# andrewadare/SLAM.jl

Measured on AMD Instinct MI355X. Metric: EKF updates/sec @ 10k landmarks, higher is better.
Workload: dtype f32; 1 GPU; EKF-SLAM observation step (associate+update; no new features arise), N=10000 landmarks (n=20003), nz=64 obs/step, gates 4.0/25.0, cholesky form, state resident in HBM; landmarks=10000, form=cholesky, parallelism=single GPU

## Files before the change

### slam.jl_amd/csrc/common.h

```cpp
#pragma once

#include <hip/hip_runtime.h>
#include <stdint.h>
#include <stdio.h>
#include <string.h>
#include <vector>

#include "../../include/slamhip.h"
#include "../../include/slamhip_diag.h"

#define SLAM_PI 3.14159265358979323846

void slam_set_error(const char* fmt, ...);

#define HIP_TRY(expr)                                                                  \
    do {                                                                               \
        hipError_t _e = (expr);                                                        \
        if (_e != hipSuccess) {                                                        \
            slam_set_error("%s failed: %s (%s:%d)", #expr, hipGetErrorString(_e),     \
                           __FILE__, __LINE__);                                        \
            return (_e == hipErrorOutOfMemory) ? SLAM_E_NOMEM : SLAM_E_HIP;            \
        }                                                                              \
    } while (0)

#define ARG_CHECK(cond, msg)                                                           \
    do {                                                                               \
        if (!(cond)) {                                                                 \
            slam_set_error("bad argument: %s", msg);                                   \
            return SLAM_E_BADARG;                                                      \
        }                                                                              \
    } while (0)

void slam_roctx_push(const char* name);
void slam_roctx_pop(void);
struct SlamRange {
    explicit SlamRange(const char* name) { slam_roctx_push(name); }
    ~SlamRange() { slam_roctx_pop(); }
    SlamRange(const SlamRange&) = delete;
    SlamRange& operator=(const SlamRange&) = delete;
};
#define SLAM_RANGE() SlamRange slam_range_scope_(__func__)

#define SLAM_TILE 128
#define SLAM_KPAD 32

static inline int round_up(int a, int b) { return (a + b - 1) / b * b; }

#ifdef SLAMHIP_EXPERIMENTS
#include <stdlib.h>
static inline int slam_exp_env(const char* name, int dflt) {
    const char* v = getenv(name);
    return v ? atoi(v) : dflt;
}
constexpr int SLAM_XFLAGS_MASK = ~0;
#else
static inline int slam_exp_env(const char*, int dflt) { return dflt; }
constexpr int SLAM_XFLAGS_MASK = 4 | 8 | 16 | 32 | 64 | 128 | 512 | 65536;
#endif

struct TimingPair {
    hipEvent_t a, b;
    int kid;
};

struct slam_ekf {
    int dtype;
    int device;
    int num_cus;
    int maxN;
    int N;
    int ncap;
    int ld;
    int npad;
    size_t esz;
    void* x;
    void* P;
    void* Pside;
    hipStream_t stream;
    double* PHtS;
    hipEvent_t stage_ev;
    int stage_pending;

    int kcap;
    double* PHt;
    double* Kd;
    void* W1;
    void* W2;
    void* Wimg;
    double* Cmat;
    double* Smat;
    double* Mwork;
    double* gvec;
    double* obsbuf;
    int32_t* idfbuf;
    int ocap;
    double* h_obs;
    int32_t* h_idf;
    int32_t* h_assoc;
    int32_t* d_assoc;
    double* h_obs_dev;
    int32_t* h_assoc_dev;
    double* znbuf;
    int32_t* d_count;
    int32_t* h_flag;
    int32_t* h_flag_dev;
    int32_t obs_seq;

    int2* tiles;
    int tiles_T, tiles_len, tiles_cap;
    int tilesB_off, tilesB_len;
    int tilesH_off, tilesH_len;
    unsigned* dd_claim;
    int tiles_xlen[8];
    int diag_off, diag_len, diag_xlen[8];

    double* d_pmax;
    int pmax_valid;

    int gate_mode;
    int gate_last;
    void* grid_meta;
    int32_t* grid_cells;
    void* grid_items;
    int grid_force;
    int grid_upd;
    int grid_live;
    int grid_n_seen;

    double* gate_part;
    int gate_blocks_cap;

    double* d_small;
    double* h_small;
    int32_t* d_status;
    int32_t* h_status;

    int xflags;
    int debug_flags;
    void* dd_prof;
    int factor_blocked;
    int debug_stamps;
    int async_updates;
    int deferred;
    int pending_status;

    int timing;
    std::vector<TimingPair> pairs;
    std::vector<TimingPair> free_pairs;
    double t_ms[SLAM_K_COUNT];
    double t_sq[SLAM_K_COUNT];
    double t_min[SLAM_K_COUNT];
    int64_t t_n[SLAM_K_COUNT];
};

struct KTimer {
    slam_ekf* h;
    TimingPair p;
    bool on;
    hipStream_t s;
    KTimer(slam_ekf* h_, int kid, hipStream_t stream = nullptr);
    ~KTimer();
};

int launch_ellipses(slam_ekf* h, double* d_out);
int launch_block_gather(slam_ekf* h, int r0, int c0, int nr, int nc, int diag, void* d_out);
int launch_pack(slam_ekf* h, const void* d_src, int lds, int n, int cf, int ncols);
int launch_unpack(slam_ekf* h, void* d_dst, int ldd, int n, int cf, int ncols);
int launch_side_rebuild(slam_ekf* h);
int launch_compact(slam_ekf* h, const int32_t* keep_host, int n_new, int f0);
int launch_find_duplicates(slam_ekf* h, double gate, int32_t* pairs_out, int cap, int* count);
int launch_merge_update(slam_ekf* h, const int32_t* keep, const int32_t* gone, int cnt, const double Rc[4]);
int launch_copy_floor(slam_ekf* h, int reps, double out[2]);
int launch_predict(slam_ekf* h, double v, double g, double w, const double Q[4], double dt);
int launch_augment(slam_ekf* h, int nn, const double R[4], const double* zn_dev);
int launch_gate(slam_ekf* h, int nz, const double R[4], double gate1, double gate2, const double* z_host, bool compact);
constexpr int SLAM_GRID_SLOTS = 64;
int gate_kernels_init();
int gate_info(slam_ekf* h, int64_t out[8]);
unsigned long long* grid_drift_slot(slam_ekf* h);
int ensure_pmax(slam_ekf* h);
int launch_nis(slam_ekf* h, const double z1[2], int j, const double R[4]);
int launch_obs_model(slam_ekf* h, int j);
int launch_update(slam_ekf* h, int m, const double R[4], int form, bool device_count);
int ensure_update_workspace(slam_ekf* h, int m);
int ensure_obs_capacity(slam_ekf* h, int nobs);
```

### slam.jl_amd/csrc/ekf_api.hip

```cpp
#include <stdarg.h>
#include <stdio.h>
#include <stdlib.h>
#include <string.h>
#include <vector>

#include "common.h"

int update_kernels_init();

static thread_local char g_err[512] = "";

void slam_set_error(const char* fmt, ...) {
    va_list ap;
    va_start(ap, fmt);
    vsnprintf(g_err, sizeof(g_err), fmt, ap);
    va_end(ap);
}

extern "C" const char* slam_last_error(void) { return g_err; }

#include <dlfcn.h>
#include <mutex>
namespace {
typedef int (*roctx_push_fn)(const char*);
typedef int (*roctx_pop_fn)(void);
roctx_push_fn g_roctx_push = nullptr;
roctx_pop_fn g_roctx_pop = nullptr;
std::once_flag g_roctx_once;
void roctx_resolve() {
    const char* names[] = {"librocprofiler-sdk-roctx.so.1", "librocprofiler-sdk-roctx.so", "libroctx64.so.4", "libroctx64.so"};
    const char* env = getenv("SLAMHIP_ROCTX");
    const bool want = env && atoi(env) != 0;
    if (env && !want) return;
    void* lib = nullptr;
    for (const char* n : names)
        if ((lib = dlopen(n, RTLD_LAZY | RTLD_NOLOAD))) break;
    if (!lib && want)
        for (const char* n : names)
            if ((lib = dlopen(n, RTLD_LAZY | RTLD_GLOBAL))) break;
    if (!lib) return;
    g_roctx_push = (roctx_push_fn)dlsym(lib, "roctxRangePushA");
    g_roctx_pop = (roctx_pop_fn)dlsym(lib, "roctxRangePop");
    if (!g_roctx_push || !g_roctx_pop) g_roctx_push = nullptr, g_roctx_pop = nullptr;
}
}
void slam_roctx_push(const char* name) {
    std::call_once(g_roctx_once, roctx_resolve);
    if (g_roctx_push) (void)g_roctx_push(name);
}
void slam_roctx_pop(void) {
    if (g_roctx_pop) (void)g_roctx_pop();
}

extern "C" int slam_device_count(void) {
    int n = 0;
    if (hipGetDeviceCount(&n) != hipSuccess) {
        (void)hipGetLastError();
        return 0;
    }
    return n;
}

KTimer::KTimer(slam_ekf* h_, int kid, hipStream_t stream)
    : h(h_), on(h_->timing == 1 || ((h_->timing >> (kid + 1)) & 1)), s(stream ? stream : h_->stream) {
    if (!on) return;
    if (!h->free_pairs.empty()) {
        p = h->free_pairs.back();
        h->free_pairs.pop_back();
    } else {
        if (hipEventCreateWithFlags(&p.a, hipEventDisableSystemFence) != hipSuccess ||
            hipEventCreateWithFlags(&p.b, hipEventDisableSystemFence) != hipSuccess) {
            on = false;
            return;
        }
    }
    p.kid = kid;
    (void)hipEventRecord(p.a, s);
}

KTimer::~KTimer() {
    if (!on) return;
    (void)hipEventRecord(p.b, s);
    h->pairs.push_back(p);
}

static int fold_timing(slam_ekf* h) {
    HIP_TRY(hipStreamSynchronize(h->stream));
    for (auto& p : h->pairs) {
        float ms = 0.f;
        if (hipEventElapsedTime(&ms, p.a, p.b) == hipSuccess) {
            h->t_ms[p.kid] += ms;
            h->t_sq[p.kid] += (double)ms * (double)ms;
            if (h->t_min[p.kid] == 0.0 || ms < h->t_min[p.kid]) h->t_min[p.kid] = ms;
            h->t_n[p.kid] += 1;
        }
        h->free_pairs.push_back(p);
    }
    h->pairs.clear();
    return SLAM_OK;
}

template <typename P>
static int dev_alloc_zero(P** p, size_t bytes, hipStream_t s) {
    *p = nullptr;
    if (bytes == 0) bytes = 16;
    HIP_TRY(hipMalloc((void**)p, bytes));
    HIP_TRY(hipMemsetAsync(*p, 0, bytes, s));
    return SLAM_OK;
}

static void dev_free(void* p) {
    if (p) (void)hipFree(p);
}

int ensure_obs_capacity(slam_ekf* h, int nobs) {
    if (nobs <= h->ocap) return SLAM_OK;
    int cap = h->ocap ? h->ocap : 256;
    while (cap < nobs) cap *= 2;
    HIP_TRY(hipStreamSynchronize(h->stream));
    dev_free(h->obsbuf); dev_free(h->idfbuf); dev_free(h->d_assoc); dev_free(h->gate_part); dev_free(h->znbuf);
    if (h->h_obs) (void)hipHostFree(h->h_obs);
    if (h->h_idf) (void)hipHostFree(h->h_idf);
    if (h->h_assoc) (void)hipHostFree(h->h_assoc);
    h->obsbuf = nullptr; h->idfbuf = nullptr; h->d_assoc = nullptr; h->gate_part = nullptr; h->znbuf = nullptr;
    h->h_obs = nullptr; h->h_idf = nullptr; h->h_assoc = nullptr;
    h->ocap = 0;
    int rc;
    if ((rc = dev_alloc_zero(&h->obsbuf, sizeof(double) * 2 * cap, h->stream))) return rc;
    if ((rc = dev_alloc_zero(&h->idfbuf, sizeof(int32_t) * cap, h->stream))) return rc;
    if ((rc = dev_alloc_zero(&h->d_assoc, sizeof(int32_t) * cap, h->stream))) return rc;
    if ((rc = dev_alloc_zero(&h->znbuf, sizeof(double) * 2 * cap, h->stream))) return rc;
    h->gate_blocks_cap = (h->maxN + 63) / 64 + 1;
    if ((rc = dev_alloc_zero(&h->gate_part, sizeof(double) * 3 * 256 * (size_t)h->gate_blocks_cap, h->stream))) return rc;
    HIP_TRY(hipHostMalloc((void**)&h->h_obs, sizeof(double) * 2 * cap, hipHostMallocDefault));
    HIP_TRY(hipHostMalloc((void**)&h->h_idf, sizeof(int32_t) * cap, hipHostMallocDefault));
    HIP_TRY(hipHostMalloc((void**)&h->h_assoc, sizeof(int32_t) * cap, hipHostMallocDefault));
    HIP_TRY(hipHostGetDevicePointer((void**)&h->h_obs_dev, h->h_obs, 0));
    HIP_TRY(hipHostGetDevicePointer((void**)&h->h_assoc_dev, h->h_assoc, 0));
    h->ocap = cap;
    return SLAM_OK;
}

static void free_update_workspace(slam_ekf* h) {
    dev_free(h->PHt); dev_free(h->PHtS); dev_free(h->Kd); dev_free(h->W1); dev_free(h->W2); dev_free(h->Cmat); dev_free(h->Wimg);
    dev_free(h->Smat); dev_free(h->Mwork); dev_free(h->gvec);
    h->W1 = h->W2 = h->Wimg = nullptr;
    h->PHt = h->PHtS = h->Kd = h->Cmat = h->Smat = h->Mwork = h->gvec = nullptr;
    h->kcap = 0;
}

static int zero_panels(slam_ekf* h) {
    if (!h->kcap) return SLAM_OK;
    HIP_TRY(hipMemsetAsync(h->PHt, 0, sizeof(double) * (size_t)h->npad * h->kcap, h->stream));
    HIP_TRY(hipMemsetAsync(h->Kd, 0, sizeof(double) * (size_t)h->npad * h->kcap, h->stream));
    HIP_TRY(hipMemsetAsync(h->W1, 0, h->esz * (size_t)h->npad * 2 * h->kcap, h->stream));
    HIP_TRY(hipMemsetAsync(h->W2, 0, h->esz * (size_t)h->npad * 2 * h->kcap, h->stream));
    return SLAM_OK;
}

int ensure_update_workspace(slam_ekf* h, int m) {
    const int kp = round_up(2 * m, SLAM_KPAD);
    if (kp <= h->kcap) return SLAM_OK;
    int cap = h->kcap ? h->kcap : 32;
    while (cap < kp) cap *= 2;
    HIP_TRY(hipStreamSynchronize(h->stream));
    free_update_workspace(h);
    int rc;
    if ((rc = dev_alloc_zero(&h->PHt, sizeof(double) * (size_t)h->npad * cap, h->stream))) return rc;
    if ((rc = dev_alloc_zero(&h->PHtS, sizeof(double) * (size_t)(3 + cap) * cap, h->stream))) return rc;
    if ((rc = dev_alloc_zero(&h->Kd, sizeof(double) * (size_t)h->npad * cap, h->stream))) return rc;
    if ((rc = dev_alloc_zero(&h->W1, h->esz * (size_t)h->npad * 2 * cap, h->stream))) return rc;
    if ((rc = dev_alloc_zero(&h->W2, h->esz * (size_t)h->npad * 2 * cap, h->stream))) return rc;
    if (h->dtype == SLAM_F32 && (rc = dev_alloc_zero(&h->Wimg, (size_t)(h->npad / 128) * (cap / 16) * 3 * 4096, h->stream))) return rc;
    if ((rc = dev_alloc_zero(&h->Cmat, sizeof(double) * (size_t)cap * cap, h->stream))) return rc;
    if ((rc = dev_alloc_zero(&h->Smat, sizeof(double) * (size_t)cap * cap, h->stream))) return rc;
    if ((rc = dev_alloc_zero(&h->Mwork, sizeof(double) * (size_t)cap * (cap + 1), h->stream))) return rc;
    if ((rc = dev_alloc_zero(&h->gvec, sizeof(double) * (size_t)cap, h->stream))) return rc;
    h->kcap = cap;
    return SLAM_OK;
}

extern "C" int slam_ekf_destroy(slam_ekf_t h) {
    if (!h) return SLAM_OK;
    (void)hipSetDevice(h->device);
    if (h->stream) (void)hipStreamSynchronize(h->stream);
#ifdef SLAMHIP_EXPERIMENTS
    if (h->dd_prof && slam_exp_env("SLAMHIP_STAMPS", 0)) {
        const size_t cnt = (size_t)4096 * 16;
        std::vector<unsigned long long> v(cnt);
        if (hipMemcpy(v.data(), h->dd_prof, cnt * 8, hipMemcpyDeviceToHost) == hipSuccess) {
            double s[16] = {0};
            size_t waves = 0;
            for (size_t w = 0; w < 4096; ++w) {
                if (!v[16 * w]) continue;
                ++waves;
                for (int i = 0; i < 16; ++i) s[i] += (double)v[16 * w + i];
            }
            if (waves) {
                fprintf(stderr, "[slamhip] dma down-date, mean per wave of %zu waves: steps %.1f  clk per step: reads %.0f  mfma-issue %.0f  barrier %.0f  dma-issue %.0f  stores(per tile) %.0f  chunk-wait by step:",
                        waves, s[0] / waves, s[1] / s[0], s[2] / s[0], s[3] / s[0], s[4] / s[0], s[5] / s[0] * 8);
                for (int i = 0; i < 8; ++i) fprintf(stderr, " %.0f", s[6 + i] / s[0] * 8);
                fprintf(stderr, "  | stream: %.0f shader clocks in %.2f us per wave = %.3f GHz in-kernel clock\n", s[14] / waves, s[15] / waves / 100.0,
                        s[15] > 0 ? s[14] / s[15] * 0.1 : 0.0);
            }
        }
        dev_free(h->dd_prof);
        h->dd_prof = nullptr;
    }
#endif
    if (h->dd_prof) {
        const size_t cnt = (size_t)4096 * 4 * 4;
        std::vector<unsigned long long> v(cnt);
        if (hipMemcpy(v.data(), h->dd_prof, cnt * 8, hipMemcpyDeviceToHost) == hipSuccess) {
            double s[4] = {0, 0, 0, 0}, mx = 0;
            size_t waves = 0;
            for (size_t w = 0; w < cnt / 4; ++w) {
                if (!v[4 * w + 3]) continue;
                ++waves;
                for (int i = 0; i < 4; ++i) s[i] += (double)v[4 * w + i];
                if ((double)v[4 * w + 3] > mx) mx = (double)v[4 * w + 3];
            }
            if (waves)
                fprintf(stderr, "[slamhip] down-date per-wave (mean of %zu waves): panel-wait %.0f clk  lifetime %.0f x 10 ns  epilogue %.0f clk  lifetime %.0f clk (max %.0f)\n",
                        waves, s[0] / waves, s[1] / waves, s[2] / waves, s[3] / waves, mx);
        }
        dev_free(h->dd_prof);
    }
    for (auto& p : h->pairs) { (void)hipEventDestroy(p.a); (void)hipEventDestroy(p.b); }
    for (auto& p : h->free_pairs) { (void)hipEventDestroy(p.a); (void)hipEventDestroy(p.b); }
    free_update_workspace(h);
    dev_free(h->x); dev_free(h->P); dev_free(h->Pside); dev_free(h->tiles);
    dev_free(h->obsbuf); dev_free(h->idfbuf); dev_free(h->d_assoc); dev_free(h->gate_part); dev_free(h->znbuf);
    dev_free(h->d_small); dev_free(h->d_status); dev_free(h->d_count); dev_free(h->d_pmax); dev_free(h->dd_claim);
    dev_free(h->grid_meta); dev_free(h->grid_cells); dev_free(h->grid_items);
    if (h->h_flag) (void)hipHostFree(h->h_flag);
    if (h->h_obs) (void)hipHostFree(h->h_obs);
    if (h->h_idf) (void)hipHostFree(h->h_idf);
    if (h->h_assoc) (void)hipHostFree(h->h_assoc);
    if (h->h_small) (void)hipHostFree(h->h_small);
    if (h->h_status) (void)hipHostFree(h->h_status);
    if (h->stage_ev) (void)hipEventDestroy(h->stage_ev);
    if (h->stream) (void)hipStreamDestroy(h->stream);
    delete h;
    return SLAM_OK;
}

static int create_impl(slam_ekf* h) {
    HIP_TRY(hipSetDevice(h->device));
    hipDeviceProp_t prop;
    HIP_TRY(hipGetDeviceProperties(&prop, h->device));
    h->num_cus = prop.multiProcessorCount > 0 ? prop.multiProcessorCount : 256;
    HIP_TRY(hipStreamCreateWithFlags(&h->stream, hipStreamNonBlocking));
    HIP_TRY(hipEventCreateWithFlags(&h->stage_ev, hipEventDisableTiming | hipEventDisableSystemFence));
    int rc;
    if ((rc = update_kernels_init())) return rc;
    if ((rc = gate_kernels_init())) return rc;
    if ((rc = dev_alloc_zero(&h->x, h->esz * (size_t)h->ncap, h->stream))) return rc;
    {
        const int E = h->dtype == SLAM_F32 ? 128 : 64;
        const size_t T = (size_t)h->npad / E;
        if ((rc = dev_alloc_zero(&h->P, h->esz * (T * (T + 1) / 2) * E * E, h->stream))) return rc;
        if ((rc = dev_alloc_zero(&h->Pside, h->esz * 3 * (size_t)(h->npad / 2), h->stream))) return rc;
    }
    if ((rc = dev_alloc_zero(&h->d_small, sizeof(double) * 64, h->stream))) return rc;
    if ((rc = dev_alloc_zero(&h->d_count, sizeof(int32_t) * 4, h->stream))) return rc;
    if ((rc = dev_alloc_zero(&h->d_pmax, sizeof(double), h->stream))) return rc;
    if ((rc = dev_alloc_zero(&h->dd_claim, 8 * 64, h->stream))) return rc;
    HIP_TRY(hipHostMalloc((void**)&h->h_flag, sizeof(int32_t) * 16, hipHostMallocDefault));
    h->h_flag[0] = 0;
    HIP_TRY(hipHostGetDevicePointer((void**)&h->h_flag_dev, h->h_flag, 0));
    if ((h->debug_flags & 8) && (rc = dev_alloc_zero(&h->dd_prof, (size_t)4096 * 4 * 4 * 8, h->stream))) return rc;
#ifdef SLAMHIP_EXPERIMENTS
    if (!h->dd_prof && slam_exp_env("SLAMHIP_STAMPS", 0) && (rc = dev_alloc_zero(&h->dd_prof, (size_t)4096 * 16 * 8, h->stream))) return rc;
#endif
    if ((rc = dev_alloc_zero(&h->d_status, sizeof(int32_t) * 4, h->stream))) return rc;
    HIP_TRY(hipHostMalloc((void**)&h->h_small, sizeof(double) * 64, hipHostMallocDefault));
    HIP_TRY(hipHostMalloc((void**)&h->h_status, sizeof(int32_t) * 4, hipHostMallocDefault));
    if ((rc = ensure_obs_capacity(h, 256))) return rc;
    HIP_TRY(hipStreamSynchronize(h->stream));
    return SLAM_OK;
}

extern "C" int slam_ekf_create(slam_ekf_t* out, int dtype, int max_landmarks, int device) {
    ARG_CHECK(out != nullptr, "handle pointer is null");
    *out = nullptr;
    ARG_CHECK(dtype == SLAM_F32 || dtype == SLAM_F64, "dtype must be SLAM_F32 or SLAM_F64");
    ARG_CHECK(max_landmarks >= 0 && max_landmarks <= 500000, "max_landmarks out of range");
    const int ndev = slam_device_count();
    if (ndev <= 0) {
        slam_set_error("no HIP device available: libslamhip has no CPU fallback");
        return SLAM_E_HIP;
    }
    ARG_CHECK(device >= 0 && device < ndev, "device index out of range");
    slam_ekf* h = new slam_ekf();
    h->dtype = dtype;
    h->device = device;
    h->maxN = max_landmarks;
    h->N = 0;
    h->ncap = 3 + 2 * max_landmarks;
    h->npad = round_up(h->ncap, SLAM_TILE);
    h->ld = h->npad;
    h->esz = dtype == SLAM_F32 ? 4 : 8;
    h->x = h->P = h->Pside = nullptr;
    h->stream = nullptr;
    h->stage_ev = nullptr; h->stage_pending = 0;
    h->PHtS = nullptr;
    h->kcap = 0;
    h->W1 = h->W2 = h->Wimg = nullptr;
    h->PHt = h->PHtS = h->Kd = h->Cmat = h->Smat = h->Mwork = h->gvec = nullptr;
    h->tiles = nullptr; h->tiles_T = h->tiles_len = h->tiles_cap = 0; h->tilesB_off = h->tilesB_len = 0;
    h->obsbuf = nullptr; h->idfbuf = nullptr; h->ocap = 0;
    h->h_obs = nullptr; h->h_idf = nullptr; h->h_assoc = nullptr; h->d_assoc = nullptr;
    h->gate_part = nullptr; h->gate_blocks_cap = 0;
    h->d_small = h->h_small = nullptr;
    h->d_pmax = nullptr; h->pmax_valid = 0; h->dd_claim = nullptr;
    h->gate_mode = SLAM_GATE_AUTO; h->gate_last = 0; h->grid_meta = nullptr; h->grid_cells = nullptr; h->grid_items = nullptr;
    h->grid_force = 1; h->grid_upd = 0; h->grid_live = 0; h->grid_n_seen = 0;
    h->znbuf = nullptr; h->d_count = nullptr; h->h_flag = nullptr; h->h_flag_dev = nullptr; h->obs_seq = 0;
    h->d_status = h->h_status = nullptr;
    h->async_updates = 0; h->deferred = 0; h->pending_status = 0; h->debug_stamps = 0;
    h->debug_flags = 0;
#ifdef SLAMHIP_EXPERIMENTS
    h->debug_flags = getenv("SLAMHIP_DEBUG") ? atoi(getenv("SLAMHIP_DEBUG")) : 0;
#endif
    h->dd_prof = nullptr;
    h->xflags = (getenv("SLAMHIP_X") ? atoi(getenv("SLAMHIP_X")) : 0) & SLAM_XFLAGS_MASK;
    h->factor_blocked = 1;
#ifdef SLAMHIP_EXPERIMENTS
    h->factor_blocked = !(getenv("SLAMHIP_FACTOR") && !strcmp(getenv("SLAMHIP_FACTOR"), "scalar"));
    if (getenv("SLAMHIP_FACTOR") && !strcmp(getenv("SLAMHIP_FACTOR"), "pivot1")) h->factor_blocked = 2;
#endif
    h->timing = 0;
    for (int i = 0; i < SLAM_K_COUNT; ++i) { h->t_ms[i] = 0; h->t_sq[i] = 0; h->t_n[i] = 0; h->t_min[i] = 0; }
    const int rc = create_impl(h);
    if (rc != SLAM_OK) {
        slam_ekf_destroy(h);
        return rc;
    }
    *out = h;
    return SLAM_OK;
}

static int state_band_columns(const slam_ekf* h, int n) {
    const size_t budget = (size_t)256 << 20;
    size_t w = budget / (h->esz * (size_t)n) / SLAM_TILE * SLAM_TILE;
    if (w < SLAM_TILE) w = SLAM_TILE;
    if (w > (size_t)h->npad) w = (size_t)h->npad;
    return (int)w;
}

static int set_state_impl(slam_ekf* h, const void* x, const void* P, int n, int ldP, hipMemcpyKind kind) {
    ARG_CHECK(h != nullptr, "null handle");
    ARG_CHECK(x != nullptr && P != nullptr, "x / P is null");
    ARG_CHECK(n >= 3 && ((n - 3) % 2) == 0, "n must be 3 + 2*N");
    ARG_CHECK(ldP >= n, "ldP < n");
    const int N = (n - 3) / 2;
    if (N > h->maxN) {
        slam_set_error("state has %d landmarks, capacity is %d", N, h->maxN);
        return SLAM_E_CAPACITY;
    }
    HIP_TRY(hipSetDevice(h->device));
    if (N < h->N) {
        const int rc = zero_panels(h);
        if (rc) return rc;
    }
    HIP_TRY(hipMemcpyAsync(h->x, x, h->esz * (size_t)n, kind, h->stream));
    int rc = SLAM_OK;
    hipError_t es = hipSuccess;
    if (kind == hipMemcpyHostToDevice) {
        const int W = state_band_columns(h, n);
        void* d_tmp = nullptr;
        HIP_TRY(hipMalloc(&d_tmp, h->esz * (size_t)n * W));
        for (int c = 0; c < h->npad && rc == SLAM_OK && es == hipSuccess; c += W) {
            const int w = c + W <= h->npad ? W : h->npad - c;
            const int wn = n - c < 0 ? 0 : (n - c < w ? n - c : w);
            if (wn > 0)
                es = hipMemcpy2DAsync(d_tmp, h->esz * (size_t)n, (const char*)P + h->esz * (size_t)c * ldP, h->esz * (size_t)ldP,
                                      h->esz * (size_t)n, (size_t)wn, kind, h->stream);
            if (es == hipSuccess) rc = launch_pack(h, d_tmp, n, n, c, w);
            if (es == hipSuccess && rc == SLAM_OK) es = hipStreamSynchronize(h->stream);
        }
        (void)hipFree(d_tmp);
    } else {
        rc = launch_pack(h, P, ldP, n, 0, h->npad);
        es = hipStreamSynchronize(h->stream);
    }
    if (rc) return rc;
    if (es != hipSuccess) {
        slam_set_error("upload of the state failed: %s", hipGetErrorString(es));
        return SLAM_E_HIP;
    }
    h->N = N;
    h->pmax_valid = 0;
    h->grid_force = 1;
    return SLAM_OK;
}

extern "C" int slam_ekf_set_state(slam_ekf_t h, const void* x, const void* P, int n, int ldP) {
    SLAM_RANGE();
    return set_state_impl(h, x, P, n, ldP, hipMemcpyHostToDevice);
}

extern "C" int slam_ekf_set_state_device(slam_ekf_t h, const void* d_x, const void* d_P, int n, int ldP) {
    SLAM_RANGE();
    return set_state_impl(h, d_x, d_P, n, ldP, hipMemcpyDeviceToDevice);
}

extern "C" int slam_ekf_get_state(slam_ekf_t h, void* x, void* P, int n, int ldP) {
    SLAM_RANGE();
    ARG_CHECK(h != nullptr, "null handle");
    ARG_CHECK(n == 3 + 2 * h->N, "n does not match the state (3 + 2*N)");
    ARG_CHECK(P == nullptr || ldP >= n, "ldP < n");
    HIP_TRY(hipSetDevice(h->device));
    if (x) HIP_TRY(hipMemcpyAsync(x, h->x, h->esz * (size_t)n, hipMemcpyDeviceToHost, h->stream));
    int rc = SLAM_OK;
    hipError_t es = hipSuccess;
    if (P) {
        const int W = state_band_columns(h, n);
        void* d_tmp = nullptr;
        HIP_TRY(hipMalloc(&d_tmp, h->esz * (size_t)n * W));
        for (int c = 0; c < n && rc == SLAM_OK && es == hipSuccess; c += W) {
            const int w = c + W <= n ? W : n - c;
            rc = launch_unpack(h, d_tmp, n, n, c, w);
            if (rc == SLAM_OK)
                es = hipMemcpy2DAsync((char*)P + h->esz * (size_t)c * ldP, h->esz * (size_t)ldP, d_tmp, h->esz * (size_t)n,
                                      h->esz * (size_t)n, (size_t)w, hipMemcpyDeviceToHost, h->stream);
            if (rc == SLAM_OK && es == hipSuccess) es = hipStreamSynchronize(h->stream);
        }
        (void)hipFree(d_tmp);
    }
    if (es == hipSuccess) es = hipStreamSynchronize(h->stream);
    if (rc) return rc;
    if (es != hipSuccess) {
        slam_set_error("download of the state failed: %s", hipGetErrorString(es));
        return SLAM_E_HIP;
    }
    return SLAM_OK;
}

static int get_gathered(slam_ekf* h, int r0, int c0, int nr, int nc, int diag, void* out, int ld_out) {
    HIP_TRY(hipSetDevice(h->device));
    void* d_tmp = nullptr;
    HIP_TRY(hipMalloc(&d_tmp, h->esz * (size_t)nr * nc));
    int rc = launch_block_gather(h, r0, c0, nr, nc, diag, d_tmp);
    if (rc == SLAM_OK) {
        hipError_t e = hipMemcpy2DAsync(out, h->esz * (size_t)ld_out, d_tmp, h->esz * (size_t)nr, h->esz * (size_t)nr, (size_t)nc,
                                        hipMemcpyDeviceToHost, h->stream);
        if (e == hipSuccess) e = hipStreamSynchronize(h->stream);
        if (e != hipSuccess) {
            slam_set_error("HIP error while reading a covariance block: %s", hipGetErrorString(e));
            rc = SLAM_E_HIP;
        }
    }
    (void)hipFree(d_tmp);
    return rc;
}

extern "C" int slam_ekf_get_block(slam_ekf_t h, int r0, int c0, int nr, int nc, void* out, int ld_out) {
    SLAM_RANGE();
    ARG_CHECK(h != nullptr, "null handle");
    const int n = 3 + 2 * h->N;
    ARG_CHECK(nr >= 0 && nc >= 0, "negative block size");
    if (nr == 0 || nc == 0) return SLAM_OK;
    ARG_CHECK(out != nullptr, "out is null");
    ARG_CHECK(r0 >= 0 && c0 >= 0 && r0 + nr <= n && c0 + nc <= n, "block outside the n x n covariance (Julia: BoundsError)");
    ARG_CHECK(ld_out >= nr, "ld_out < nr");
    ARG_CHECK((size_t)nr * nc <= ((size_t)1 << 28), "block larger than 2^28 elements: read it in pieces");
    return get_gathered(h, r0, c0, nr, nc, 0, out, ld_out);
}

extern "C" int slam_ekf_get_diag(slam_ekf_t h, void* out) {
    ARG_CHECK(h != nullptr && out != nullptr, "null argument");
    const int n = 3 + 2 * h->N;
    return get_gathered(h, 0, 0, n, 1, 1, out, n);
}

extern "C" int slam_ekf_get_landmark_blocks(slam_ekf_t h, void* out) {
    ARG_CHECK(h != nullptr && out != nullptr, "null argument");
    if (h->N == 0) return SLAM_OK;
    HIP_TRY(hipSetDevice(h->device));
    HIP_TRY(hipMemcpy2DAsync(out, h->esz * (size_t)h->N, h->Pside, h->esz * (size_t)(h->npad / 2), h->esz * (size_t)h->N, 3,
                             hipMemcpyDeviceToHost, h->stream));
    HIP_TRY(hipStreamSynchronize(h->stream));
    return SLAM_OK;
}

extern "C" int slam_ekf_get_pose(slam_ekf_t h, double pose[3]) {
    ARG_CHECK(h != nullptr && pose != nullptr, "null argument");
    HIP_TRY(hipSetDevice(h->device));
    HIP_TRY(hipMemcpyAsync(h->h_small, h->x, h->esz * 3, hipMemcpyDeviceToHost, h->stream));
    HIP_TRY(hipStreamSynchronize(h->stream));
    for (int i = 0; i < 3; ++i)
        pose[i] = h->dtype == SLAM_F32 ? (double)((float*)h->h_small)[i] : h->h_small[i];
    return SLAM_OK;
}

extern "C" int slam_ekf_ellipses(slam_ekf_t h, double* features, double vehicle[6]) {
    SLAM_RANGE();
    ARG_CHECK(h != nullptr, "null handle");
    HIP_TRY(hipSetDevice(h->device));
    const size_t cnt = (size_t)h->N + 1;
    double* d_out = nullptr;
    HIP_TRY(hipMalloc((void**)&d_out, sizeof(double) * 5 * cnt));
    std::vector<double> host(5 * cnt);
    int rc = launch_ellipses(h, d_out);
    if (rc == SLAM_OK) {
        const hipError_t e1 = hipMemcpyAsync(host.data(), d_out, sizeof(double) * 5 * cnt, hipMemcpyDeviceToHost, h->stream);
        const hipError_t e2 = e1 == hipSuccess ? hipStreamSynchronize(h->stream) : e1;
        if (e2 != hipSuccess) {
            slam_set_error("HIP error in slam_ekf_ellipses: %s", hipGetErrorString(e2));
            rc = SLAM_E_HIP;
        }
    }
    (void)hipFree(d_out);
    if (rc) return rc;
    if (features)
        for (size_t i = 0; i < 5 * (cnt - 1); ++i) features[i] = host[5 + i];
    if (vehicle) {
        double pose[3];
        if ((rc = slam_ekf_get_pose(h, pose))) return rc;
        vehicle[0] = pose[0]; vehicle[1] = pose[1]; vehicle[2] = pose[2];
        vehicle[3] = host[2]; vehicle[4] = host[3]; vehicle[5] = host[4];
    }
    return SLAM_OK;
}

extern "C" int slam_ekf_num_landmarks(slam_ekf_t h, int* N) {
    ARG_CHECK(h != nullptr && N != nullptr, "null argument");
    *N = h->N;
    return SLAM_OK;
}

extern "C" int slam_ekf_dtype(slam_ekf_t h, int* dtype) {
    ARG_CHECK(h != nullptr && dtype != nullptr, "null argument");
    *dtype = h->dtype;
    return SLAM_OK;
}

extern "C" int slam_ekf_device_ptrs(slam_ekf_t h, void** d_x, void** d_P, int* ld, void** stream) {
    ARG_CHECK(h != nullptr, "null handle");
    if (d_x) *d_x = h->x;
    if (d_P) *d_P = h->P;
    if (ld) *ld = h->ld;
    if (stream) *stream = (void*)h->stream;
    return SLAM_OK;
}

extern "C" int slam_ekf_state_written(slam_ekf_t h) {
    SLAM_RANGE();
    ARG_CHECK(h != nullptr, "null handle");
    HIP_TRY(hipSetDevice(h->device));
    h->pmax_valid = 0;
    h->grid_force = 1;
    return launch_side_rebuild(h);
}

static int remove_marked(slam_ekf* h, const std::vector<char>& gone, int cnt, int32_t* new_index) {
    const int N = h->N;
    const int n_new = 3 + 2 * (N - cnt);
    std::vector<int32_t> keep((size_t)n_new);
    keep[0] = 0; keep[1] = 1; keep[2] = 2;
    int first = 0, next = 0;
    for (int j = 1; j <= N; ++j) {
        if (gone[j]) {
            if (!first) first = j;
            continue;
        }
        keep[3 + 2 * next] = 3 + 2 * (j - 1);
        keep[4 + 2 * next] = 4 + 2 * (j - 1);
        ++next;
    }
    HIP_TRY(hipSetDevice(h->device));
    int rc;
    if ((rc = launch_compact(h, keep.data(), n_new, 3 + 2 * (first - 1)))) return rc;
    h->N = N - cnt;
    if ((rc = zero_panels(h))) return rc;
    h->pmax_valid = 0;
    h->grid_force = 1;
    h->grid_n_seen = h->N;
    if ((rc = launch_side_rebuild(h))) return rc;
    if (new_index)
        for (int j = 1, k = 0; j <= N; ++j) new_index[j - 1] = gone[j] ? 0 : ++k;
    return SLAM_OK;
}

extern "C" int slam_ekf_remove_landmarks(slam_ekf_t h, const int32_t* ids, int cnt, int32_t* new_index) {
    SLAM_RANGE();
    ARG_CHECK(h != nullptr, "null handle");
    ARG_CHECK(cnt >= 0, "cnt < 0");
    ARG_CHECK(cnt == 0 || ids != nullptr, "ids is null");
    const int N = h->N;
    std::vector<char> gone((size_t)N + 1, 0);
    for (int i = 0; i < cnt; ++i) {
        ARG_CHECK(ids[i] >= 1 && ids[i] <= N, "landmark id out of range");
        ARG_CHECK(!gone[ids[i]], "duplicate landmark id");
        gone[ids[i]] = 1;
    }
    if (cnt == 0) {
        if (new_index)
            for (int j = 1; j <= N; ++j) new_index[j - 1] = j;
        return SLAM_OK;
    }
    return remove_marked(h, gone, cnt, new_index);
}

extern "C" int slam_ekf_find_duplicates(slam_ekf_t h, double gate, int32_t* pairs, int cap, int* count) {
    SLAM_RANGE();
    ARG_CHECK(h != nullptr, "null handle");
    ARG_CHECK(count != nullptr, "count is null");
    ARG_CHECK(cap >= 0, "cap < 0");
    ARG_CHECK(cap == 0 || pairs != nullptr, "pairs is null");
    ARG_CHECK(gate > 0.0 && gate <= 1.79769313486231570815e308, "gate must be finite and positive");
    HIP_TRY(hipSetDevice(h->device));
    return launch_find_duplicates(h, gate, pairs, cap, count);
}

extern "C" int slam_ekf_merge_landmarks(slam_ekf_t h, const int32_t* pairs, int cnt, const double Rc[4], int32_t* new_index) {
    SLAM_RANGE();
    ARG_CHECK(h != nullptr, "null handle");
    ARG_CHECK(cnt >= 0 && cnt <= SLAM_MERGE_MAX, "cnt outside 0 .. SLAM_MERGE_MAX");
    ARG_CHECK(cnt == 0 || pairs != nullptr, "pairs is null");
    const int N = h->N;
    std::vector<char> used((size_t)N + 1, 0), gone((size_t)N + 1, 0);
    int32_t keep_id[SLAM_MERGE_MAX], gone_id[SLAM_MERGE_MAX];
    for (int p = 0; p < cnt; ++p) {
        const int32_t a = pairs[2 * p], b = pairs[2 * p + 1];
        ARG_CHECK(a >= 1 && a <= N && b >= 1 && b <= N, "landmark id out of range");
        ARG_CHECK(a != b, "a pair names one landmark twice");
        ARG_CHECK(!used[a] && !used[b], "a landmark appears in more than one pair (merge a chain with one call per link)");
        used[a] = used[b] = 1;
        gone[b] = 1;
        keep_id[p] = a;
        gone_id[p] = b;
    }
    if (Rc) {
        ARG_CHECK(Rc[1] == Rc[2], "Rc is not symmetric");
        ARG_CHECK(Rc[0] >= 0.0 && Rc[3] >= 0.0, "Rc has a negative diagonal");
    }
    if (cnt == 0) {
        if (new_index)
            for (int j = 1; j <= N; ++j) new_index[j - 1] = j;
        return SLAM_OK;
    }
    HIP_TRY(hipSetDevice(h->device));
    int rc;
    if ((rc = ensure_update_workspace(h, SLAM_MERGE_MAX))) return rc;
    if ((rc = launch_merge_update(h, keep_id, gone_id, cnt, Rc))) return rc;
    HIP_TRY(hipMemcpyAsync(h->h_status, h->d_status, sizeof(int32_t) * 4, hipMemcpyDeviceToHost, h->stream));
    HIP_TRY(hipStreamSynchronize(h->stream));
    if (h->h_status[0]) {
        slam_set_error("merge: S is not positive definite (state left unchanged, nothing removed)");
        return SLAM_E_NOTPD;
    }
    if ((rc = remove_marked(h, gone, cnt, new_index))) return rc;
    if (new_index)
        for (int p = 0; p < cnt; ++p) new_index[gone_id[p] - 1] = new_index[keep_id[p] - 1];
    return SLAM_OK;
}

extern "C" int slam_ekf_copy_floor(slam_ekf_t h, int reps, double out[2]) {
    SLAM_RANGE();
    ARG_CHECK(h != nullptr && out != nullptr, "null argument");
    ARG_CHECK(reps >= 1 && reps <= 1000, "reps out of range");
    HIP_TRY(hipSetDevice(h->device));
    return launch_copy_floor(h, reps, out);
}

static int check_R(const double* R) {
    ARG_CHECK(R != nullptr, "R is null");
    return SLAM_OK;
}

static int stage_obs(slam_ekf* h, const double* z, const int32_t* idf, int nobs) {
    int rc = ensure_obs_capacity(h, nobs);
    if (rc) return rc;
    if (h->stage_pending) {
        HIP_TRY(hipEventSynchronize(h->stage_ev));
        h->stage_pending = 0;
    }
    memcpy(h->h_obs, z, sizeof(double) * 2 * (size_t)nobs);
    HIP_TRY(hipMemcpyAsync(h->obsbuf, h->h_obs, sizeof(double) * 2 * (size_t)nobs, hipMemcpyHostToDevice, h->stream));
    if (idf) {
        memcpy(h->h_idf, idf, sizeof(int32_t) * (size_t)nobs);
        HIP_TRY(hipMemcpyAsync(h->idfbuf, h->h_idf, sizeof(int32_t) * (size_t)nobs, hipMemcpyHostToDevice, h->stream));
    }
    HIP_TRY(hipEventRecord(h->stage_ev, h->stream));
    h->stage_pending = 1;
    return SLAM_OK;
}

extern "C" int slam_ekf_predict(slam_ekf_t h, double v, double g, double wheelbase, const double Q[4], double dt) {
    SLAM_RANGE();
    ARG_CHECK(h != nullptr && Q != nullptr, "null argument");
    HIP_TRY(hipSetDevice(h->device));
    return launch_predict(h, v, g, wheelbase, Q, dt);
}

extern "C" int slam_ekf_associate(slam_ekf_t h, const double* z, int nz, const double R[4], double gate1, double gate2,
                                  int32_t* assoc) {
    SLAM_RANGE();
    ARG_CHECK(h != nullptr, "null handle");
    ARG_CHECK(nz >= 0, "nz < 0");
    if (nz == 0) return SLAM_OK;
    ARG_CHECK(z != nullptr && assoc != nullptr, "z / assoc is null");
    int rc = check_R(R);
    if (rc) return rc;
    if (h->N == 0) {
        for (int i = 0; i < nz; ++i) assoc[i] = -1;
        return SLAM_OK;
    }
    HIP_TRY(hipSetDevice(h->device));
    if ((rc = ensure_obs_capacity(h, nz))) return rc;
    if ((rc = launch_gate(h, nz, R, gate1, gate2, z, false))) return rc;
    HIP_TRY(hipMemcpyAsync(h->h_assoc, h->d_assoc, sizeof(int32_t) * (size_t)nz, hipMemcpyDeviceToHost, h->stream));
    HIP_TRY(hipStreamSynchronize(h->stream));
    memcpy(assoc, h->h_assoc, sizeof(int32_t) * (size_t)nz);
    return SLAM_OK;
}

extern "C" int slam_ekf_set_gate_mode(slam_ekf_t h, int mode) {
    ARG_CHECK(h != nullptr, "null handle");
    ARG_CHECK(mode == SLAM_GATE_AUTO || mode == SLAM_GATE_SWEEP || mode == SLAM_GATE_GRID, "unknown gate mode");
    h->gate_mode = mode;
    h->grid_force = 1;
    return SLAM_OK;
}

extern "C" int slam_ekf_gate_info(slam_ekf_t h, int64_t out[8]) {
    ARG_CHECK(h != nullptr && out != nullptr, "null argument");
    HIP_TRY(hipSetDevice(h->device));
    return gate_info(h, out);
}

extern "C" int slam_ekf_nis(slam_ekf_t h, const double z1[2], int j, const double R[4], double out[2]) {
    ARG_CHECK(h != nullptr && z1 != nullptr && out != nullptr, "null argument");
    int rc = check_R(R);
    if (rc) return rc;
    ARG_CHECK(j >= 1 && j <= h->N, "landmark index out of range");
    HIP_TRY(hipSetDevice(h->device));
    if ((rc = launch_nis(h, z1, j, R))) return rc;
    HIP_TRY(hipMemcpyAsync(h->h_small, h->d_small, sizeof(double) * 2, hipMemcpyDeviceToHost, h->stream));
    HIP_TRY(hipStreamSynchronize(h->stream));
    out[0] = h->h_small[0];
    out[1] = h->h_small[1];
    return SLAM_OK;
}

extern "C" int slam_ekf_predict_observation(slam_ekf_t h, int j, double zp[2], double Hv[6], double Hf[4]) {
    ARG_CHECK(h != nullptr && zp != nullptr && Hv != nullptr && Hf != nullptr, "null argument");
    ARG_CHECK(j >= 1 && j <= h->N, "landmark index out of range");
    HIP_TRY(hipSetDevice(h->device));
    int rc;
    if ((rc = launch_obs_model(h, j))) return rc;
    HIP_TRY(hipMemcpyAsync(h->h_small, h->d_small, sizeof(double) * 12, hipMemcpyDeviceToHost, h->stream));
    HIP_TRY(hipStreamSynchronize(h->stream));
    zp[0] = h->h_small[0]; zp[1] = h->h_small[1];
    for (int i = 0; i < 6; ++i) Hv[i] = h->h_small[2 + i];
    for (int i = 0; i < 4; ++i) Hf[i] = h->h_small[8 + i];
    return SLAM_OK;
}

static int read_status(slam_ekf* h, int sticky) {
    HIP_TRY(hipMemcpyAsync(h->h_status, h->d_status, sizeof(int32_t) * 4, hipMemcpyDeviceToHost, h->stream));
    HIP_TRY(hipStreamSynchronize(h->stream));
    const int bad = sticky ? h->h_status[1] : h->h_status[0];
    if (h->h_status[1]) HIP_TRY(hipMemsetAsync(h->d_status + 1, 0, sizeof(int32_t), h->stream));
    h->pending_status = 0;
    if (bad == 2) {
        slam_set_error("update: the factorisation did not publish within 2 s; covariance unchanged, the mean may be partly updated");
        return SLAM_E_HIP;
    }
    if (bad) {
        slam_set_error("innovation covariance S is not positive definite (state left unchanged)");
        return SLAM_E_NOTPD;
    }
    return SLAM_OK;
}

extern "C" int slam_ekf_update(slam_ekf_t h, const double* zf, const int32_t* idf, int m, const double R[4], int form) {
    SLAM_RANGE();
    ARG_CHECK(h != nullptr, "null handle");
    ARG_CHECK(m >= 0, "m < 0");
    ARG_CHECK(form == SLAM_FORM_CHOLESKY || form == SLAM_FORM_JOSEPH, "unknown update form");
    if (m == 0) return SLAM_OK;
    ARG_CHECK(zf != nullptr && idf != nullptr, "zf / idf is null");
    int rc = check_R(R);
    if (rc) return rc;
    for (int i = 0; i < m; ++i) ARG_CHECK(idf[i] >= 1 && idf[i] <= h->N, "idf entry out of range (Julia: BoundsError)");
    HIP_TRY(hipSetDevice(h->device));
    if ((rc = ensure_update_workspace(h, m))) return rc;
    if ((rc = stage_obs(h, zf, idf, m))) return rc;
    if ((rc = launch_update(h, m, R, form, false))) return rc;
    if (h->async_updates) {
        h->pending_status = 1;
        return SLAM_OK;
    }
    return read_status(h, 0);
}

extern "C" int slam_ekf_augment(slam_ekf_t h, const double* zn, int nn, const double R[4]) {
    SLAM_RANGE();
    ARG_CHECK(h != nullptr, "null handle");
    ARG_CHECK(nn >= 0, "nn < 0");
    if (nn == 0) return SLAM_OK;
    ARG_CHECK(zn != nullptr, "zn is null");
    int rc = check_R(R);
    if (rc) return rc;
    if (h->N + nn > h->maxN) {
        slam_set_error("augment: %d + %d landmarks exceed capacity %d", h->N, nn, h->maxN);
        return SLAM_E_CAPACITY;
    }
    HIP_TRY(hipSetDevice(h->device));
    if ((rc = stage_obs(h, zn, nullptr, nn))) return rc;
    if ((rc = launch_augment(h, nn, R, h->obsbuf))) return rc;
    h->N += nn;
    return SLAM_OK;
}

extern "C" int slam_ekf_observe(slam_ekf_t h, const double* z, int nz, const double R[4], double gate1, double gate2, int form,
                                int32_t* assoc) {
    SLAM_RANGE();
    ARG_CHECK(h != nullptr, "null handle");
    ARG_CHECK(nz >= 0, "nz < 0");
    ARG_CHECK(form == SLAM_FORM_CHOLESKY || form == SLAM_FORM_JOSEPH, "unknown update form");
    if (nz == 0) return SLAM_OK;
    ARG_CHECK(z != nullptr && assoc != nullptr, "z / assoc is null");
    int rc = check_R(R);
    if (rc) return rc;
    HIP_TRY(hipSetDevice(h->device));
    if (h->N == 0) {
        for (int i = 0; i < nz; ++i) assoc[i] = -1;
        return slam_ekf_augment(h, z, nz, R);
    }
    if ((rc = ensure_update_workspace(h, nz))) return rc;
    if ((rc = ensure_obs_capacity(h, nz))) return rc;
    h->obs_seq = h->obs_seq == 0x7fffffff ? 1 : h->obs_seq + 1;
    if ((rc = launch_gate(h, nz, R, gate1, gate2, z, true))) return rc;
    if ((rc = launch_update(h, nz, R, form, true))) return rc;
    {
        volatile int32_t* flag = h->h_flag;
        unsigned long long spins = 0;
        while (*flag != h->obs_seq) {
            __builtin_ia32_pause();
            if ((++spins & 0xfffffull) == 0) {
                const hipError_t q = hipStreamQuery(h->stream);
                if (q != hipErrorNotReady && *flag != h->obs_seq) {
                    if (q == hipSuccess) slam_set_error("observe: the gating finished without publishing its decisions");
                    else slam_set_error("HIP error while waiting for the gating: %s", hipGetErrorString(q));
                    return SLAM_E_HIP;
                }
            }
        }
        __atomic_thread_fence(__ATOMIC_ACQUIRE);
    }
    int nn = 0;
    for (int i = 0; i < nz; ++i) {
        assoc[i] = h->h_assoc[i];
        nn += assoc[i] < 0;
    }
    int cap_rc = SLAM_OK;
    if (nn) {
        if (h->N + nn > h->maxN) cap_rc = SLAM_E_CAPACITY;
        else {
            if ((rc = launch_augment(h, nn, R, h->znbuf))) return rc;
            h->N += nn;
        }
    }
    if (h->async_updates) h->pending_status = 1;
    else if ((rc = read_status(h, 0))) return rc;
    if (cap_rc) {
        slam_set_error("observe: %d + %d landmarks exceed capacity %d (the update was applied, no feature added)", h->N, nn,
                       h->maxN);
        return cap_rc;
    }
    return SLAM_OK;
}

#ifdef SLAMHIP_EXPERIMENTS
extern "C" int slam_exp_observe_enqueue(slam_ekf_t h, const double* z, int nz, const double R[4], double gate1, double gate2) {
    ARG_CHECK(h != nullptr && z != nullptr && nz > 0 && h->N > 0, "bad argument");
    int rc = check_R(R);
    if (rc) return rc;
    HIP_TRY(hipSetDevice(h->device));
    if ((rc = ensure_update_workspace(h, nz))) return rc;
    if ((rc = ensure_obs_capacity(h, nz))) return rc;
    h->obs_seq = h->obs_seq == 0x7fffffff ? 1 : h->obs_seq + 1;
    if ((rc = launch_gate(h, nz, R, gate1, gate2, z, true))) return rc;
    return launch_update(h, nz, R, SLAM_FORM_CHOLESKY, true);
}

extern "C" int slam_exp_workspace(slam_ekf_t h, int what, void* out, size_t bytes, size_t* size) {
    ARG_CHECK(h != nullptr && h->kcap > 0, "no workspace yet");
    HIP_TRY(hipSetDevice(h->device));
    const void* src = nullptr;
    size_t sz = 0;
    if (what == 0) { src = h->W1; sz = h->esz * (size_t)h->npad * 2 * h->kcap; }
    else if (what == 1) { src = h->Wimg; sz = h->Wimg ? (size_t)(h->npad / 128) * (h->kcap / 16) * 3 * 4096 : 0; }
    else if (what == 2) { src = h->Cmat; sz = sizeof(double) * (size_t)h->kcap * h->kcap; }
    else if (what == 3) { src = h->gvec; sz = sizeof(double) * (size_t)h->kcap; }
    ARG_CHECK(src != nullptr, "no such buffer");
    if (size) *size = sz;
    if (out && bytes) {
        HIP_TRY(hipStreamSynchronize(h->stream));
        HIP_TRY(hipMemcpy(out, src, bytes < sz ? bytes : sz, hipMemcpyDeviceToHost));
    }
    return SLAM_OK;
}
#endif

extern "C" int slam_ekf_set_async(slam_ekf_t h, int async_updates) {
    ARG_CHECK(h != nullptr, "null handle");
    h->async_updates = async_updates ? 1 : 0;
    return SLAM_OK;
}

extern "C" int slam_ekf_sync(slam_ekf_t h) {
    SLAM_RANGE();
    ARG_CHECK(h != nullptr, "null handle");
    HIP_TRY(hipSetDevice(h->device));
    if (h->pending_status) return read_status(h, 1);
    HIP_TRY(hipStreamSynchronize(h->stream));
    return SLAM_OK;
}

extern "C" int slam_ekf_debug_stamps(slam_ekf_t h, int enable, uint64_t* out16) {
    ARG_CHECK(h != nullptr, "null handle");
    h->debug_stamps = enable ? 1 : 0;
    if (out16) {
        HIP_TRY(hipSetDevice(h->device));
        HIP_TRY(hipMemcpyAsync(h->h_small, h->d_small + 40, sizeof(uint64_t) * 16, hipMemcpyDeviceToHost, h->stream));
        HIP_TRY(hipStreamSynchronize(h->stream));
        memcpy(out16, h->h_small, sizeof(uint64_t) * 16);
    }
    return SLAM_OK;
}

extern "C" int slam_ekf_timing(slam_ekf_t h, int enable) {
    ARG_CHECK(h != nullptr, "null handle");
    h->timing = enable < 0 ? 0 : enable;
    return SLAM_OK;
}

extern "C" int slam_ekf_timing_read(slam_ekf_t h, int kid, double* total_ms, int64_t* launches) {
    ARG_CHECK(h != nullptr, "null handle");
    ARG_CHECK(kid >= 0 && kid < SLAM_K_COUNT, "kernel id out of range");
    HIP_TRY(hipSetDevice(h->device));
    const int rc = fold_timing(h);
    if (rc) return rc;
    if (total_ms) *total_ms = h->t_ms[kid];
    if (launches) *launches = h->t_n[kid];
    return SLAM_OK;
}

extern "C" int slam_ekf_timing_min(slam_ekf_t h, int kid, double* min_ms) {
    ARG_CHECK(h != nullptr && min_ms != nullptr, "null argument");
    ARG_CHECK(kid >= 0 && kid < SLAM_K_COUNT, "kernel id out of range");
    HIP_TRY(hipSetDevice(h->device));
    const int rc = fold_timing(h);
    if (rc) return rc;
    *min_ms = h->t_min[kid];
    return SLAM_OK;
}

extern "C" int slam_ekf_timing_stats(slam_ekf_t h, int kid, double out[4]) {
    ARG_CHECK(h != nullptr && out != nullptr, "null argument");
    ARG_CHECK(kid >= 0 && kid < SLAM_K_COUNT, "kernel id out of range");
    HIP_TRY(hipSetDevice(h->device));
    const int rc = fold_timing(h);
    if (rc) return rc;
    const double nn = (double)h->t_n[kid];
    const double mean = nn > 0 ? h->t_ms[kid] / nn : 0.0;
    const double var = nn > 1 ? (h->t_sq[kid] - nn * mean * mean) / (nn - 1.0) : 0.0;
    out[0] = nn; out[1] = mean; out[2] = var > 0 ? sqrt(var) : 0.0; out[3] = h->t_min[kid];
    return SLAM_OK;
}

extern "C" int slam_ekf_timing_reset(slam_ekf_t h) {
    ARG_CHECK(h != nullptr, "null handle");
    HIP_TRY(hipSetDevice(h->device));
    const int rc = fold_timing(h);
    if (rc) return rc;
    for (int i = 0; i < SLAM_K_COUNT; ++i) { h->t_ms[i] = 0; h->t_sq[i] = 0; h->t_n[i] = 0; h->t_min[i] = 0; }
    return SLAM_OK;
}
```

### slam.jl_amd/csrc/ekf_gate.hip

```cpp
#include "common.h"
#include "device_math.h"

namespace {

constexpr int GATE_BLOCK = 64;
constexpr int GATE_WAVES = 1;
constexpr int OBS_WAVES = 8;

struct PairConst {
    double zp0, zp1;
    double s00, s01, s10, s11;
    double det, logdet;
    double qa, qb, qc;
};

__device__ inline PairConst pair_const(const ObsModel& om, const double* pvv, const double pfv[2][3],
                                       const double pff[4], const double R[4]) {
    PairConst pc;
    pc.zp0 = om.zp[0];
    pc.zp1 = om.zp[1];
    double A[2][3];
    double B[2][2];
    double Cc[2][3];
    double D[2][2];
#pragma unroll
    for (int r = 0; r < 2; ++r) {
#pragma unroll
        for (int c = 0; c < 3; ++c) {
            A[r][c] = om.Hv[r * 3 + 0] * pvv[0 * 3 + c] + om.Hv[r * 3 + 1] * pvv[1 * 3 + c] +
                      om.Hv[r * 3 + 2] * pvv[2 * 3 + c];
            Cc[r][c] = om.Hf[r * 2 + 0] * pfv[0][c] + om.Hf[r * 2 + 1] * pfv[1][c];
        }
#pragma unroll
        for (int a = 0; a < 2; ++a) {
            B[r][a] = om.Hv[r * 3 + 0] * pfv[a][0] + om.Hv[r * 3 + 1] * pfv[a][1] + om.Hv[r * 3 + 2] * pfv[a][2];
            D[r][a] = om.Hf[r * 2 + 0] * pff[0 * 2 + a] + om.Hf[r * 2 + 1] * pff[1 * 2 + a];
        }
    }
    double S[2][2];
#pragma unroll
    for (int r = 0; r < 2; ++r)
#pragma unroll
        for (int q = 0; q < 2; ++q) {
            double s = A[r][0] * om.Hv[q * 3 + 0] + A[r][1] * om.Hv[q * 3 + 1] + A[r][2] * om.Hv[q * 3 + 2];
            s += B[r][0] * om.Hf[q * 2 + 0] + B[r][1] * om.Hf[q * 2 + 1];
            s += Cc[r][0] * om.Hv[q * 3 + 0] + Cc[r][1] * om.Hv[q * 3 + 1] + Cc[r][2] * om.Hv[q * 3 + 2];
            s += D[r][0] * om.Hf[q * 2 + 0] + D[r][1] * om.Hf[q * 2 + 1];
            S[r][q] = s + R[q * 2 + r];
        }
    pc.s00 = S[0][0]; pc.s01 = S[0][1]; pc.s10 = S[1][0]; pc.s11 = S[1][1];
    pc.det = pc.s00 * pc.s11 - pc.s01 * pc.s10;
    pc.logdet = log(pc.det);
    const double rdet = 1.0 / pc.det;
    pc.qa = pc.s11 * rdet;
    pc.qb = -(pc.s01 + pc.s10) * rdet;
    pc.qc = pc.s00 * rdet;
    return pc;
}

__device__ inline void pair_eval(const PairConst& pc, double z0, double z1, double& nis, double& nd) {
    const double v0 = z0 - pc.zp0;
    const double v1 = mpi_to_pi_d(z1 - pc.zp1);
    nis = pc.qa * v0 * v0 + pc.qb * v0 * v1 + pc.qc * v1 * v1;
    nd = nis + pc.logdet;
}

template <typename T>
__device__ inline PairConst landmark_const(const T* __restrict__ x, const T* __restrict__ P, int ld, int tlog, int j0,
                                           const double pose[3], const double* pvv, const double R[4],
                                           const T* __restrict__ side = nullptr, int side_n = 0) {
    const int f = 3 + 2 * j0;
    const double lx = (double)x[f], ly = (double)x[f + 1];
    const ObsModel om = obs_model(pose[0], pose[1], pose[2], lx, ly);
    double pfv[2][3];
#pragma unroll
    for (int c = 0; c < 3; ++c) {
        pfv[0][c] = (double)P[p_off(ld, tlog, f, c)];
        pfv[1][c] = (double)P[p_off(ld, tlog, f + 1, c)];
    }
    double pff[4];
    if (side) {
        pff[0] = (double)side[j0];
        pff[2] = (double)side[(size_t)side_n + j0];
        pff[3] = (double)side[(size_t)2 * side_n + j0];
    } else {
        pff[0] = (double)P[p_off(ld, tlog, f, f)];
        pff[2] = (double)P[p_off(ld, tlog, f + 1, f)];
        pff[3] = (double)P[p_off(ld, tlog, f + 1, f + 1)];
    }
    pff[1] = pff[2];
    return pair_const(om, pvv, pfv, pff, R);
}

struct PreGate {
    double b0, b1;
};

__device__ inline PreGate pre_gate(double dx, double dy, const double* pvv, double pmax, const double R[4], double gate2) {
    PreGate g;
    const double d2 = dx * dx + dy * dy, d = sqrt(d2);
    const double sx = sqrt(pvv[0]), sy = sqrt(pvv[4]), sp = sqrt(pvv[8]), sm = sqrt(pmax);
    const double ax = fabs(dx), ay = fabs(dy);
    const double a0 = (ax * sx + ay * sy + (ax + ay) * sm) / d;
    const double a1 = (ay * sx + ax * sy + (ax + ay) * sm) / d2 + sp;
    const double slack = 1.0 + 1e-6;
    g.b0 = gate2 * (a0 * a0 + R[0]) * slack;
    g.b1 = gate2 * (a1 * a1 + R[3]) * slack;
    if (!(g.b0 > 0.0) || !(g.b0 < __builtin_inf())) g.b0 = __builtin_inf();
    if (!(g.b1 > 0.0) || !(g.b1 < __builtin_inf())) g.b1 = __builtin_inf();
    return g;
}

template <bool ZAGENT = false>
__device__ __forceinline__ void compact_wave(const int32_t* assoc, int nz, const double* zsrc,
                                             double* zbuf, int32_t* __restrict__ idf,
                                             double* __restrict__ zn, int32_t* __restrict__ count,
                                             int32_t* __restrict__ assoc_host, int lane, int32_t* __restrict__ flag_host,
                                             int32_t seq) {
    int m = 0, nn = 0;
    for (int base = 0; base < nz; base += 64) {
        const int i = base + lane;
        const int a = i < nz ? __hip_atomic_load(assoc + i, __ATOMIC_RELAXED, __HIP_MEMORY_SCOPE_AGENT) : 0;
        double z0 = 0.0, z1 = 0.0;
        if (i < nz) {
            if (ZAGENT) {
                z0 = __hip_atomic_load(zsrc + 2 * i, __ATOMIC_RELAXED, __HIP_MEMORY_SCOPE_AGENT);
                z1 = __hip_atomic_load(zsrc + 2 * i + 1, __ATOMIC_RELAXED, __HIP_MEMORY_SCOPE_AGENT);
            } else {
                z0 = zsrc[2 * i];
                z1 = zsrc[2 * i + 1];
            }
        }
        if (i < nz) __hip_atomic_store(assoc_host + i, a, __ATOMIC_RELAXED, __HIP_MEMORY_SCOPE_SYSTEM);
        const unsigned long long mm = __ballot(a > 0), mn = __ballot(a < 0);
        const unsigned long long below = (1ull << lane) - 1ull;
        __builtin_amdgcn_s_waitcnt(0);
        __builtin_amdgcn_wave_barrier();
        if (a > 0) {
            const int pos = m + __popcll(mm & below);
            idf[pos] = a;
            zbuf[2 * pos] = z0;
            zbuf[2 * pos + 1] = z1;
        } else if (a < 0) {
            const int pos = nn + __popcll(mn & below);
            zn[2 * pos] = z0;
            zn[2 * pos + 1] = z1;
        }
        m += __popcll(mm);
        nn += __popcll(mn);
    }
    if (lane == 0) {
        count[0] = m;
        count[1] = nn;
    }
    asm volatile("s_waitcnt vmcnt(0)" ::: "memory");
    __builtin_amdgcn_wave_barrier();
    if (lane == 0) __hip_atomic_store(flag_host, seq, __ATOMIC_RELAXED, __HIP_MEMORY_SCOPE_SYSTEM);
}

constexpr int GATE_CHUNK = 128;
__device__ __forceinline__ const double* zdev_base(const double*, const double* zbuf) { return zbuf; }
struct GateObs {
    double z[2 * GATE_CHUNK];
};

template <typename T>
__global__ __launch_bounds__(GATE_BLOCK * OBS_WAVES) void gate_kernel(GateObs zarg, const T* __restrict__ x, const T* __restrict__ P,
                                                           int ld, int N, double* __restrict__ zdev, int nz, double R0,
                                                           double R1, double R2, double R3, double gate1, double gate2,
                                                           double* __restrict__ part, const double* __restrict__ pmax_ptr,
                                                           int pregate, int tlog, const T* __restrict__ side, int side_n,
                                                           int part_cap, int32_t* assoc, int32_t* assoc_all, int compact_total,
                                                           double* zbuf, int32_t* __restrict__ idf, double* __restrict__ zn,
                                                           int32_t* __restrict__ count, int32_t* __restrict__ assoc_host, int32_t* arrive,
                                                           int32_t* __restrict__ flag_host, int32_t seq) {
    extern __shared__ double smem[];
    double* zs = smem;
    double* red = smem + 2 * nz;
    const int tid = threadIdx.x;
    const int lane = tid & 63;
    const int wave = tid >> 6;
    constexpr int NT = GATE_BLOCK * OBS_WAVES;
    typedef const __attribute__((address_space(4))) GateObs* KargPtr;
    const KargPtr ka = (KargPtr)__builtin_amdgcn_kernarg_segment_ptr();
    for (int i = tid; i < 2 * nz; i += NT) {
        const double v = ka->z[i];
        zs[i] = v;
        if (blockIdx.x == 0) __hip_atomic_store(zdev + i, v, __ATOMIC_RELAXED, __HIP_MEMORY_SCOPE_AGENT);
    }
    double* const list = part;
    int32_t* const cnt = reinterpret_cast<int32_t*>(part + (size_t)2 * GATE_CHUNK * part_cap);
    int32_t* const nearw = cnt + GATE_CHUNK;

    const double R[4] = {R0, R1, R2, R3};
    double pose[3] = {(double)x[0], (double)x[1], (double)x[2]};
    double pvv[9];
#pragma unroll
    for (int r = 0; r < 3; ++r)
#pragma unroll
        for (int c = 0; c < 3; ++c) pvv[r * 3 + c] = (double)P[p_off(ld, tlog, r, c)];

    const int j0 = blockIdx.x * GATE_BLOCK + lane;
    bool valid = j0 < N;
    const double INF = __builtin_inf();
    if (pregate) {
        __syncthreads();
        bool need = false;
        if (valid) {
            const int f = 3 + 2 * j0;
            const double dx = (double)x[f] - pose[0], dy = (double)x[f + 1] - pose[1];
            const PreGate g = pre_gate(dx, dy, pvv, *pmax_ptr, R, gate2);
            const double zp0 = sqrt(dx * dx + dy * dy), zp1 = atan2(dy, dx) - pose[2];
            for (int i = wave; i < nz; i += OBS_WAVES) {
                const double v0 = zs[2 * i] - zp0, v1 = mpi_to_pi_d(zs[2 * i + 1] - zp1);
                if (!(v0 * v0 > g.b0) && !(v1 * v1 > g.b1)) need = true;
            }
        }
        valid = need;
    }
    PairConst pc;
    if (valid) pc = landmark_const(x, P, ld, tlog, j0, pose, pvv, R, side, side_n);
    __syncthreads();

    for (int i = wave; i < nz; i += OBS_WAVES) {
        double nis = INF, nd = INF;
        if (valid) pair_eval(pc, zs[2 * i], zs[2 * i + 1], nis, nd);
        const bool cand = valid && (nis < gate1) && (nd < INF);
        const bool near = valid && (nis <= gate2);
        const unsigned long long cand_mask = __ballot(cand);
        const unsigned long long near_mask = __ballot(near);
        if ((cand_mask | near_mask) != 0ull) {
            double nd_c = INF;
            int j_c = 0x7fffffff;
            if (cand_mask != 0ull) {
                if (cand) { nd_c = nd; j_c = j0 + 1; }
#pragma unroll
                for (int off = 32; off >= 1; off >>= 1) {
                    const double o_nd = __shfl_xor(nd_c, off);
                    const int o_j = __shfl_xor(j_c, off);
                    if (o_nd < nd_c || (o_nd == nd_c && o_j < j_c)) { nd_c = o_nd; j_c = o_j; }
                }
            }
            if (lane == 0) {
                (void)__hip_atomic_fetch_or(nearw + i, 1, __ATOMIC_RELAXED, __HIP_MEMORY_SCOPE_AGENT);
                if (cand_mask != 0ull) {
                    const int e = __hip_atomic_fetch_add(cnt + i, 1, __ATOMIC_RELAXED, __HIP_MEMORY_SCOPE_AGENT);
                    double* o = list + ((size_t)i * part_cap + e) * 2;
                    __hip_atomic_store(o, nd_c, __ATOMIC_RELAXED, __HIP_MEMORY_SCOPE_AGENT);
                    __hip_atomic_store(o + 1, (double)j_c, __ATOMIC_RELAXED, __HIP_MEMORY_SCOPE_AGENT);
                }
            }
        }
    }
    asm volatile("s_waitcnt vmcnt(0)" ::: "memory");
    __syncthreads();
    int* const s_last = reinterpret_cast<int*>(red);
    if (tid == 0) *s_last = __hip_atomic_fetch_add(arrive, 1, __ATOMIC_RELAXED, __HIP_MEMORY_SCOPE_AGENT) == (int)gridDim.x - 1 ? 1 : 0;
    __syncthreads();
    if (!*s_last) return;
    for (int i = tid; i < nz; i += NT) {
        const int c = __hip_atomic_load(cnt + i, __ATOMIC_RELAXED, __HIP_MEMORY_SCOPE_AGENT);
        const int nr = __hip_atomic_load(nearw + i, __ATOMIC_RELAXED, __HIP_MEMORY_SCOPE_AGENT);
        double nd_c = INF, j_c = (double)0x7fffffff;
        for (int e = 0; e < c; ++e) {
            const double* o = list + ((size_t)i * part_cap + e) * 2;
            const double r0 = __hip_atomic_load(o, __ATOMIC_RELAXED, __HIP_MEMORY_SCOPE_AGENT);
            const double r1 = __hip_atomic_load(o + 1, __ATOMIC_RELAXED, __HIP_MEMORY_SCOPE_AGENT);
            if (r0 < nd_c || (r0 == nd_c && r1 < j_c)) { nd_c = r0; j_c = r1; }
        }
        int32_t a;
        if (nd_c < INF) a = (int32_t)j_c;
        else if (!nr) a = -1;
        else a = 0;
        __hip_atomic_store(assoc + i, a, __ATOMIC_RELAXED, __HIP_MEMORY_SCOPE_AGENT);
        __hip_atomic_store(cnt + i, 0, __ATOMIC_RELAXED, __HIP_MEMORY_SCOPE_AGENT);
        __hip_atomic_store(nearw + i, 0, __ATOMIC_RELAXED, __HIP_MEMORY_SCOPE_AGENT);
    }
    if (tid == 0) __hip_atomic_store(arrive, 0, __ATOMIC_RELAXED, __HIP_MEMORY_SCOPE_AGENT);
    if (compact_total > 0) {
        asm volatile("s_waitcnt vmcnt(0)" ::: "memory");
        __syncthreads();
        if (wave == 0) compact_wave<true>(assoc_all, compact_total, zdev_base(zdev, zbuf), zbuf, idf, zn, count, assoc_host, lane, flag_host, seq);
    }
}

constexpr int GRID_MAX_G = 128;
constexpr int GRID_SLOTS = SLAM_GRID_SLOTS;
constexpr int GRID_SUBS = 16;
constexpr int GRID_FOLD_UPDATES = 16;
constexpr int GRID_TAIL_MAX = 512;
constexpr int GRID_AUTO_N = 16384;
constexpr int GRID_BUILD_THREADS = 1024;
constexpr int GRID_QUERY_THREADS = 256;

struct GridItem {
    double bx, by;
    int j0, pad;
};

struct GridMeta {
    double x0, y0, invx, invy;
    double cellmin;
    double drift;
    int G, n_built, valid, pad;
    unsigned long long rebuilds, queries, boxed, evals;
    unsigned long long slot[GRID_SUBS][GRID_SLOTS];
};

__device__ __forceinline__ int grid_coord(double p, double p0, double inv, int G) {
    const double t = floor((p - p0) * inv);
    if (t >= (double)(G - 1)) return G - 1;
    return t > 0.0 ? (int)t : 0;
}

template <typename T>
__global__ __launch_bounds__(GRID_BUILD_THREADS) void grid_prepare_kernel(const T* __restrict__ x, int N, GridMeta* __restrict__ meta,
                                                                          int32_t* __restrict__ cell_start,
                                                                          GridItem* __restrict__ items, int nslots, int force) {
    extern __shared__ int g_hist[];
    __shared__ double s_red[4][GRID_BUILD_THREADS / 64];
    __shared__ int s_scan[GRID_BUILD_THREADS / 64];
    __shared__ int s_do;
    const int tid = threadIdx.x, lane = tid & 63, wave = tid >> 6;
    constexpr int NW = GRID_BUILD_THREADS / 64;
    const double INF = __builtin_inf();
    if (wave == 0) {
        double d = 0.0;
        if (lane < nslots) {
            unsigned long long m = 0ull;
            for (int sub = 0; sub < GRID_SUBS; ++sub) {
                const unsigned long long v = meta->slot[sub][lane];
                m = v > m ? v : m;
                meta->slot[sub][lane] = 0ull;
            }
            d = __longlong_as_double((long long)m);
        }
#pragma unroll
        for (int off = 32; off >= 1; off >>= 1) d += __shfl_xor(d, off);
        if (lane == 0) {
            d = (meta->drift + d) * (1.0 + 1e-12);
            const int tail_max = min(GRID_TAIL_MAX, 32 + meta->n_built / 4);
            const bool rebuild = force || !meta->valid || !(d <= 0.25 * meta->cellmin) || N < meta->n_built ||
                                 N - meta->n_built >= tail_max;
            meta->drift = d;
            s_do = rebuild ? 1 : 0;
        }
    }
    __syncthreads();
    if (!s_do) return;

    double xmin = INF, xmax = -INF, ymin = INF, ymax = -INF;
    for (int j = tid; j < N; j += GRID_BUILD_THREADS) {
        const double lx = (double)x[3 + 2 * j], ly = (double)x[4 + 2 * j];
        if (lx < xmin) xmin = lx;
        if (lx > xmax) xmax = lx;
        if (ly < ymin) ymin = ly;
        if (ly > ymax) ymax = ly;
    }
#pragma unroll
    for (int off = 32; off >= 1; off >>= 1) {
        xmin = fmin(xmin, __shfl_xor(xmin, off));
        xmax = fmax(xmax, __shfl_xor(xmax, off));
        ymin = fmin(ymin, __shfl_xor(ymin, off));
        ymax = fmax(ymax, __shfl_xor(ymax, off));
    }
    if (lane == 0) { s_red[0][wave] = xmin; s_red[1][wave] = xmax; s_red[2][wave] = ymin; s_red[3][wave] = ymax; }
    __syncthreads();
    xmin = s_red[0][0]; xmax = s_red[1][0]; ymin = s_red[2][0]; ymax = s_red[3][0];
    for (int w = 1; w < NW; ++w) {
        xmin = fmin(xmin, s_red[0][w]); xmax = fmax(xmax, s_red[1][w]);
        ymin = fmin(ymin, s_red[2][w]); ymax = fmax(ymax, s_red[3][w]);
    }
    if (!(xmin <= xmax) || !(xmax < INF) || !(xmin > -INF)) { xmin = 0.0; xmax = 0.0; }
    if (!(ymin <= ymax) || !(ymax < INF) || !(ymin > -INF)) { ymin = 0.0; ymax = 0.0; }
    int G = (int)sqrt((double)N / 4.0);
    G = G < 4 ? 4 : (G > GRID_MAX_G ? GRID_MAX_G : G);
    const double scale = fmax(fmax(fabs(xmin), fabs(xmax)), fmax(fabs(ymin), fabs(ymax)));
    const double tiny = fmax(1e-9, 1e-12 * scale);
    double cwx = (xmax - xmin) / G, cwy = (ymax - ymin) / G;
    if (!(cwx > tiny)) cwx = fmax(1.0, tiny);
    if (!(cwy > tiny)) cwy = fmax(1.0, tiny);
    const double invx = 1.0 / cwx, invy = 1.0 / cwy;
    const int cells = G * G;
    for (int c = tid; c < cells; c += GRID_BUILD_THREADS) g_hist[c] = 0;
    __syncthreads();
    for (int j = tid; j < N; j += GRID_BUILD_THREADS) {
        const int cx = grid_coord((double)x[3 + 2 * j], xmin, invx, G), cy = grid_coord((double)x[4 + 2 * j], ymin, invy, G);
        atomicAdd(&g_hist[cy * G + cx], 1);
    }
    __syncthreads();
    const int per = (cells + GRID_BUILD_THREADS - 1) / GRID_BUILD_THREADS;
    const int c0 = tid * per;
    int sum = 0;
    for (int u = 0; u < per; ++u)
        if (c0 + u < cells) sum += g_hist[c0 + u];
    int incl = sum;
#pragma unroll
    for (int off = 1; off < 64; off <<= 1) {
        const int o = __shfl_up(incl, off);
        if (lane >= off) incl += o;
    }
    if (lane == 63) s_scan[wave] = incl;
    __syncthreads();
    int base = 0;
    for (int w = 0; w < wave; ++w) base += s_scan[w];
    int run = base + incl - sum;
    for (int u = 0; u < per; ++u)
        if (c0 + u < cells) {
            const int cnt = g_hist[c0 + u];
            cell_start[c0 + u] = run;
            g_hist[c0 + u] = run;
            run += cnt;
        }
    if (tid == 0) cell_start[cells] = N;
    __syncthreads();
    for (int j = tid; j < N; j += GRID_BUILD_THREADS) {
        const double lx = (double)x[3 + 2 * j], ly = (double)x[4 + 2 * j];
        const int cx = grid_coord(lx, xmin, invx, G), cy = grid_coord(ly, ymin, invy, G);
        GridItem it;
        it.bx = lx; it.by = ly; it.j0 = j; it.pad = 0;
        items[atomicAdd(&g_hist[cy * G + cx], 1)] = it;
    }
    if (tid == 0) {
        meta->x0 = xmin; meta->y0 = ymin; meta->invx = invx; meta->invy = invy;
        meta->cellmin = fmin(cwx, cwy);
        meta->drift = 0.0;
        meta->G = G; meta->n_built = N; meta->valid = 1;
        meta->rebuilds += 1ull;
    }
}

__device__ __forceinline__ bool arc_has(double a, double b, double t) {
    const double k = ceil((a - t) / (2.0 * SLAM_PI_D));
    return t + 2.0 * SLAM_PI_D * k <= b;
}

template <typename T>
__global__ __launch_bounds__(GRID_QUERY_THREADS) void gate_grid_kernel(
    GateObs zarg, const T* __restrict__ x, const T* __restrict__ P, int ld, int N, double* zdev, int nz, double R0, double R1, double R2,
    double R3, double gate1, double gate2, const double* __restrict__ pmax_ptr, int tlog, const T* __restrict__ side, int side_n,
    GridMeta* meta, int nslots, const int32_t* __restrict__ cell_start, const GridItem* __restrict__ items,
    int32_t* assoc, int32_t* assoc_all, int compact_total, double* zall, int32_t* __restrict__ idf, double* __restrict__ zn,
    int32_t* __restrict__ count, int32_t* __restrict__ assoc_host, int32_t* arrive, int32_t* __restrict__ flag_host, int32_t seq) {
    __shared__ double s_nd[GRID_QUERY_THREADS / 64];
    __shared__ int s_j[GRID_QUERY_THREADS / 64], s_near[GRID_QUERY_THREADS / 64];
    __shared__ unsigned s_cnt[2][GRID_QUERY_THREADS / 64];
    const int tid = threadIdx.x, lane = tid & 63, wave = tid >> 6;
    constexpr int NW = GRID_QUERY_THREADS / 64;
    const int i = blockIdx.x;
    typedef const __attribute__((address_space(4))) GateObs* KargPtr;
    const KargPtr ka = (KargPtr)__builtin_amdgcn_kernarg_segment_ptr();
    const double z0 = ka->z[2 * i], z1 = ka->z[2 * i + 1];
    unsigned long long dm[4];
#pragma unroll
    for (int it = 0; it < 4; ++it) {
        const int sl = 4 * it + (lane >> 4);
        dm[it] = sl < nslots ? meta->slot[lane & 15][sl] : 0ull;
    }
    const double R[4] = {R0, R1, R2, R3};
    const double pose[3] = {(double)x[0], (double)x[1], (double)x[2]};
    double pvv[9];
#pragma unroll
    for (int r = 0; r < 3; ++r)
#pragma unroll
        for (int c = 0; c < 3; ++c) pvv[r * 3 + c] = (double)P[p_off(ld, tlog, r, c)];
    const double pmax = *pmax_ptr;
    const int G = meta->G, n_built = meta->n_built < N ? meta->n_built : N;
    const double gx0 = meta->x0, gy0 = meta->y0, invx = meta->invx, invy = meta->invy, drift0 = meta->drift;
    if (tid == 0) {
        __hip_atomic_store(zdev + 2 * i, z0, __ATOMIC_RELAXED, __HIP_MEMORY_SCOPE_AGENT);
        __hip_atomic_store(zdev + 2 * i + 1, z1, __ATOMIC_RELAXED, __HIP_MEMORY_SCOPE_AGENT);
    }
    double dsum = 0.0;
#pragma unroll
    for (int it = 0; it < 4; ++it) {
#pragma unroll
        for (int off = 1; off <= 8; off <<= 1) {
            const unsigned long long o = __shfl_xor(dm[it], off);
            dm[it] = o > dm[it] ? o : dm[it];
        }
        dsum += __longlong_as_double((long long)dm[it]);
    }
    dsum += __shfl_xor(dsum, 16);
    dsum += __shfl_xor(dsum, 32);
    const double drift = (drift0 + dsum) * (1.0 + 1e-12);
    const double INF = __builtin_inf();

    int cx0 = 0, cx1 = G - 1, cy0 = 0, cy1 = G - 1;
    double d_lo = -INF, d_hi = INF;
    {
        const double A0 = sqrt(fmax(pvv[0], 0.0) + fmax(pvv[4], 0.0)) + sqrt(2.0 * fmax(pmax, 0.0));
        const double sp = sqrt(fmax(pvv[8], 0.0));
        const double rho = sqrt(gate2 * (A0 * A0 + R0)) * (1.0 + 1e-6) + 1e-9;
        const double dmax = z0 + rho;
        double dmin = z0 - rho;
        if (dmin < 0.0) dmin = 0.0;
        if (dmax < INF && dmax == dmax && drift == drift && drift < INF) {
            if (dmax < 0.0) { cx0 = 1; cx1 = 0; d_hi = -INF; }
            else {
                double cmin = -1.0, cmax = 1.0, smin = -1.0, smax = 1.0;
                if (dmin > 0.0) {
                    const double a1 = A0 / dmin + sp;
                    const double beta = sqrt(gate2 * (a1 * a1 + R3)) * (1.0 + 1e-6) + 1e-9;
                    const double th = z1 + pose[2];
                    if (beta < SLAM_PI_D && th == th && fabs(th) < 1e6) {
                        const double a = th - beta, b = th + beta;
                        const double ca = cos(a), cb = cos(b), sa = sin(a), sb = sin(b);
                        cmax = arc_has(a, b, 0.0) ? 1.0 : fmax(ca, cb);
                        cmin = arc_has(a, b, SLAM_PI_D) ? -1.0 : fmin(ca, cb);
                        smax = arc_has(a, b, 0.5 * SLAM_PI_D) ? 1.0 : fmax(sa, sb);
                        smin = arc_has(a, b, -0.5 * SLAM_PI_D) ? -1.0 : fmin(sa, sb);
                    }
                }
                const double eps = 1e-9 * (dmax + fabs(pose[0]) + fabs(pose[1]) + 1.0);
                const double pad = drift + eps;
                const double xlo = fmin(cmin * dmax, cmin * dmin), xhi = fmax(cmax * dmax, cmax * dmin);
                const double ylo = fmin(smin * dmax, smin * dmin), yhi = fmax(smax * dmax, smax * dmin);
                cx0 = grid_coord(pose[0] + xlo - pad, gx0, invx, G);
                cx1 = grid_coord(pose[0] + xhi + pad, gx0, invx, G);
                cy0 = grid_coord(pose[1] + ylo - pad, gy0, invy, G);
                cy1 = grid_coord(pose[1] + yhi + pad, gy0, invy, G);
                d_lo = dmin - 1.4142135623730951 * drift - eps;
                d_hi = dmax + 1.4142135623730951 * drift + eps;
            }
        }
    }

    double best_nd = INF;
    int best_j = 0x7fffffff;
    bool near_any = false;
    unsigned n_box = 0, n_eval = 0;
    auto evaluate = [&](int j0) {
        ++n_eval;
        const PairConst pc = landmark_const(x, P, ld, tlog, j0, pose, pvv, R, side, side_n);
        double nis, nd;
        pair_eval(pc, z0, z1, nis, nd);
        if (nis <= gate2) near_any = true;
        if (nis < gate1 && nd < INF && (nd < best_nd || (nd == best_nd && j0 + 1 < best_j))) {
            best_nd = nd;
            best_j = j0 + 1;
        }
    };
    if (cx0 <= cx1)
        for (int cy = cy0 + wave; cy <= cy1; cy += NW) {
            const int k0 = cell_start[cy * G + cx0], k1 = cell_start[cy * G + cx1 + 1];
            for (int k = k0 + lane; k < k1; k += 64) {
                const GridItem it = items[k];
                ++n_box;
                const double dx = it.bx - pose[0], dy = it.by - pose[1];
                const double db = sqrt(dx * dx + dy * dy);
                if (db < d_lo || db > d_hi) continue;
                if (it.j0 < N) evaluate(it.j0);
            }
        }
    for (int j0 = n_built + tid; j0 < N; j0 += GRID_QUERY_THREADS) {
        ++n_box;
        evaluate(j0);
    }

#pragma unroll
    for (int off = 32; off >= 1; off >>= 1) {
        const double o_nd = __shfl_xor(best_nd, off);
        const int o_j = __shfl_xor(best_j, off);
        if (o_nd < best_nd || (o_nd == best_nd && o_j < best_j)) { best_nd = o_nd; best_j = o_j; }
        n_box += __shfl_xor(n_box, off);
        n_eval += __shfl_xor(n_eval, off);
    }
    const bool wave_near = __ballot(near_any) != 0ull;
    if (lane == 0) { s_nd[wave] = best_nd; s_j[wave] = best_j; s_near[wave] = wave_near ? 1 : 0; s_cnt[0][wave] = n_box; s_cnt[1][wave] = n_eval; }
    __syncthreads();
    if (wave != 0) return;
    int last = 0;
    if (lane == 0) {
        bool near = false;
        unsigned long long nb = 0, ne = 0;
        for (int w = 0; w < NW; ++w) {
            if (s_nd[w] < best_nd || (s_nd[w] == best_nd && s_j[w] < best_j)) { best_nd = s_nd[w]; best_j = s_j[w]; }
            near = near || s_near[w] != 0;
            nb += s_cnt[0][w]; ne += s_cnt[1][w];
        }
        int32_t a;
        if (best_nd < INF) a = best_j;
        else if (!near) a = -1;
        else a = 0;
        __hip_atomic_store(assoc + i, a, __ATOMIC_RELAXED, __HIP_MEMORY_SCOPE_AGENT);
        if (compact_total > 0) {
            asm volatile("s_waitcnt vmcnt(0)" ::: "memory");
            last = __hip_atomic_fetch_add(arrive, 1, __ATOMIC_RELAXED, __HIP_MEMORY_SCOPE_AGENT) == (int)gridDim.x - 1;
        }
        atomicAdd(&meta->boxed, nb);
        atomicAdd(&meta->evals, ne);
        if (i == 0) atomicAdd(&meta->queries, 1ull);
    }
    if (compact_total > 0 && __shfl(last, 0)) {
        compact_wave<true>(assoc_all, compact_total, zall, zall, idf, zn, count, assoc_host, lane, flag_host, seq);
        if (lane == 0) __hip_atomic_store(arrive, 0, __ATOMIC_RELAXED, __HIP_MEMORY_SCOPE_AGENT);
    }
}

template <typename T>
__global__ void single_pair_kernel(const T* __restrict__ x, const T* __restrict__ P, int ld, int j0, double z0, double z1,
                                   double R0, double R1, double R2, double R3, int mode, double* __restrict__ out, int tlog) {
    if (threadIdx.x != 0 || blockIdx.x != 0) return;
    const double R[4] = {R0, R1, R2, R3};
    double pose[3] = {(double)x[0], (double)x[1], (double)x[2]};
    if (mode == 1) {
        const int f = 3 + 2 * j0;
        const ObsModel om = obs_model(pose[0], pose[1], pose[2], (double)x[f], (double)x[f + 1]);
        out[0] = om.zp[0]; out[1] = om.zp[1];
        for (int c = 0; c < 3; ++c) { out[2 + 2 * c] = om.Hv[c]; out[2 + 2 * c + 1] = om.Hv[3 + c]; }
        for (int c = 0; c < 2; ++c) { out[8 + 2 * c] = om.Hf[c]; out[8 + 2 * c + 1] = om.Hf[2 + c]; }
        return;
    }
    double pvv[9];
    for (int r = 0; r < 3; ++r)
        for (int c = 0; c < 3; ++c) pvv[r * 3 + c] = (double)P[p_off(ld, tlog, r, c)];
    const PairConst pc = landmark_const(x, P, ld, tlog, j0, pose, pvv, R);
    double nis, nd;
    pair_eval(pc, z0, z1, nis, nd);
    out[0] = nis;
    out[1] = nd;
}

}

template <typename T>
__global__ __launch_bounds__(256) void diag_max_kernel(const T* __restrict__ P, int ld, int n, unsigned long long* __restrict__ pmax, int tlog) {
    const int i = 3 + blockIdx.x * blockDim.x + threadIdx.x;
    double v = 0.0;
    if (i < n) {
        v = (double)P[p_off(ld, tlog, i, i)];
        if (!(v >= 0.0)) v = __builtin_inf();
    }
#pragma unroll
    for (int off = 32; off >= 1; off >>= 1) v = fmax(v, __shfl_xor(v, off));
    if ((threadIdx.x & 63) == 0 && v > 0.0) atomicMax(pmax, (unsigned long long)__double_as_longlong(v));
}

int ensure_pmax(slam_ekf* h) {
    if (h->pmax_valid) return SLAM_OK;
    const int n = 3 + 2 * h->N;
    HIP_TRY(hipMemsetAsync(h->d_pmax, 0, sizeof(double), h->stream));
    if (h->N > 0) {
        const int blocks = (2 * h->N + 255) / 256;
        if (h->dtype == SLAM_F32)
            hipLaunchKernelGGL(diag_max_kernel<float>, dim3(blocks), dim3(256), 0, h->stream, (const float*)h->P, h->ld, n,
                               (unsigned long long*)h->d_pmax, 7);
        else
            hipLaunchKernelGGL(diag_max_kernel<double>, dim3(blocks), dim3(256), 0, h->stream, (const double*)h->P, h->ld, n,
                               (unsigned long long*)h->d_pmax, 6);
        HIP_TRY(hipGetLastError());
    }
    h->pmax_valid = 1;
    return SLAM_OK;
}

static int grid_alloc_zero(void** p, size_t bytes, hipStream_t s) {
    *p = nullptr;
    HIP_TRY(hipMalloc(p, bytes));
    HIP_TRY(hipMemsetAsync(*p, 0, bytes, s));
    return SLAM_OK;
}

static int ensure_grid(slam_ekf* h) {
    if (h->grid_meta) return SLAM_OK;
    int rc;
    if ((rc = grid_alloc_zero(&h->grid_meta, sizeof(GridMeta), h->stream))) return rc;
    if ((rc = grid_alloc_zero((void**)&h->grid_cells, sizeof(int32_t) * (GRID_MAX_G * GRID_MAX_G + 1), h->stream))) return rc;
    if ((rc = grid_alloc_zero(&h->grid_items, sizeof(GridItem) * (size_t)(h->maxN > 0 ? h->maxN : 1), h->stream))) return rc;
    h->grid_force = 1;
    h->grid_upd = 0;
    return SLAM_OK;
}

unsigned long long* grid_drift_slot(slam_ekf* h) {
    if (!h->grid_live) return nullptr;
    if (h->grid_upd >= GRID_SLOTS) {
        h->grid_force = 1;
        return nullptr;
    }
    return &((GridMeta*)h->grid_meta)->slot[0][h->grid_upd++];
}

static int launch_gate_grid(slam_ekf* h, int nz, const double R[4], double gate1, double gate2, const double* z_host, bool compact) {
    int rc;
    if ((rc = ensure_pmax(h))) return rc;
    if ((rc = ensure_grid(h))) return rc;
    GridMeta* meta = (GridMeta*)h->grid_meta;
    GridItem* items = (GridItem*)h->grid_items;
    const int tlog = h->dtype == SLAM_F32 ? 7 : 6;
    KTimer t(h, SLAM_K_GATE);
    const int tail_max = GRID_TAIL_MAX < 32 + h->grid_n_seen / 4 ? GRID_TAIL_MAX : 32 + h->grid_n_seen / 4;
    if (h->grid_force || !h->grid_live || h->grid_upd >= GRID_FOLD_UPDATES || h->N - h->grid_n_seen >= tail_max || h->N < h->grid_n_seen) {
        const size_t lds = sizeof(int) * GRID_MAX_G * GRID_MAX_G;
        if (h->dtype == SLAM_F32)
            hipLaunchKernelGGL(grid_prepare_kernel<float>, dim3(1), dim3(GRID_BUILD_THREADS), lds, h->stream, (const float*)h->x, h->N,
                               meta, h->grid_cells, items, h->grid_upd, h->grid_force);
        else
            hipLaunchKernelGGL(grid_prepare_kernel<double>, dim3(1), dim3(GRID_BUILD_THREADS), lds, h->stream, (const double*)h->x, h->N,
                               meta, h->grid_cells, items, h->grid_upd, h->grid_force);
        HIP_TRY(hipGetLastError());
        h->grid_upd = 0;
        h->grid_force = 0;
        h->grid_live = 1;
        h->grid_n_seen = h->N;
    }
    constexpr int CHUNK = GATE_CHUNK;
    for (int o = 0; o < nz; o += CHUNK) {
        const int cz = nz - o < CHUNK ? nz - o : CHUNK;
        GateObs zarg;
        memcpy(zarg.z, z_host + 2 * (size_t)o, sizeof(double) * 2 * (size_t)cz);
        double* zc = h->obsbuf + 2 * (size_t)o;
        const bool last = o + CHUNK >= nz;
        const int ctot = (compact && last) ? nz : 0;
        if (h->dtype == SLAM_F32)
            hipLaunchKernelGGL(gate_grid_kernel<float>, dim3(cz), dim3(GRID_QUERY_THREADS), 0, h->stream, zarg, (const float*)h->x,
                               (const float*)h->P, h->ld, h->N, zc, cz, R[0], R[1], R[2], R[3], gate1, gate2, (const double*)h->d_pmax,
                               tlog, (const float*)h->Pside, h->npad / 2, meta, h->grid_upd, (const int32_t*)h->grid_cells,
                               (const GridItem*)items, h->d_assoc + o, h->d_assoc, ctot, h->obsbuf, h->idfbuf, h->znbuf, h->d_count,
                               h->h_assoc_dev, h->d_count + 2, h->h_flag_dev, h->obs_seq);
        else
            hipLaunchKernelGGL(gate_grid_kernel<double>, dim3(cz), dim3(GRID_QUERY_THREADS), 0, h->stream, zarg, (const double*)h->x,
                               (const double*)h->P, h->ld, h->N, zc, cz, R[0], R[1], R[2], R[3], gate1, gate2, (const double*)h->d_pmax,
                               tlog, (const double*)h->Pside, h->npad / 2, meta, h->grid_upd, (const int32_t*)h->grid_cells,
                               (const GridItem*)items, h->d_assoc + o, h->d_assoc, ctot, h->obsbuf, h->idfbuf, h->znbuf, h->d_count,
                               h->h_assoc_dev, h->d_count + 2, h->h_flag_dev, h->obs_seq);
        HIP_TRY(hipGetLastError());
    }
    h->gate_last = SLAM_GATE_GRID;
    return SLAM_OK;
}

int gate_kernels_init() {
    const int lds = (int)sizeof(int) * GRID_MAX_G * GRID_MAX_G + 4096;
    HIP_TRY(hipFuncSetAttribute(reinterpret_cast<const void*>(&grid_prepare_kernel<float>), hipFuncAttributeMaxDynamicSharedMemorySize, lds));
    HIP_TRY(hipFuncSetAttribute(reinterpret_cast<const void*>(&grid_prepare_kernel<double>), hipFuncAttributeMaxDynamicSharedMemorySize, lds));
    return SLAM_OK;
}

int gate_info(slam_ekf* h, int64_t out[8]) {
    for (int i = 0; i < 8; ++i) out[i] = 0;
    out[0] = h->gate_last;
    if (!h->grid_meta) return SLAM_OK;
    GridMeta m;
    HIP_TRY(hipMemcpyAsync(&m, h->grid_meta, sizeof(GridMeta), hipMemcpyDeviceToHost, h->stream));
    HIP_TRY(hipStreamSynchronize(h->stream));
    out[1] = m.G;
    out[2] = m.n_built;
    out[3] = h->N - m.n_built;
    out[4] = (int64_t)m.rebuilds;
    out[5] = (int64_t)m.queries;
    out[6] = (int64_t)m.boxed;
    out[7] = (int64_t)m.evals;
    return SLAM_OK;
}

int launch_gate(slam_ekf* h, int nz, const double R[4], double gate1, double gate2, const double* z_host, bool compact) {
    const int nblocks = (h->N + GATE_BLOCK - 1) / GATE_BLOCK;
    if (nblocks > h->gate_blocks_cap) {
        slam_set_error("internal: gate partial buffer too small");
        return SLAM_E_HIP;
    }
    const bool r_pd = R[0] > 0.0 && R[3] > 0.0 && R[0] * R[3] - 0.25 * (R[1] + R[2]) * (R[1] + R[2]) > 0.0 && R[1] == R[2];
    const bool big = h->N >= 32768 || (h->xflags & 64);
    const int pregate = (big && r_pd && gate2 >= gate1 && gate2 < __builtin_inf() && !(h->xflags & 32)) ? 1 : 0;
    if (pregate) {
        const int rcp = ensure_pmax(h);
        if (rcp) return rcp;
    }
    const bool grid_ok = r_pd && gate2 >= gate1 && gate2 < __builtin_inf();
    if (grid_ok && (h->gate_mode == SLAM_GATE_GRID || (h->gate_mode == SLAM_GATE_AUTO && h->N >= GRID_AUTO_N)))
        return launch_gate_grid(h, nz, R, gate1, gate2, z_host, compact);
    h->gate_last = SLAM_GATE_SWEEP;
    if (h->grid_live) {
        h->grid_live = 0;
        h->grid_force = 1;
    }
    constexpr int CHUNK = GATE_CHUNK;
    for (int o = 0; o < nz; o += CHUNK) {
        const int cz = nz - o < CHUNK ? nz - o : CHUNK;
        const size_t shmem = (size_t)(2 * cz + 3 * GATE_WAVES * cz) * sizeof(double);
        GateObs zarg;
        memcpy(zarg.z, z_host + 2 * (size_t)o, sizeof(double) * 2 * (size_t)cz);
        double* zc = h->obsbuf + 2 * (size_t)o;
        {
            KTimer t(h, SLAM_K_GATE);
            const bool last = o + CHUNK >= nz;
            const int ctot = (compact && last) ? nz : 0;
            if (h->dtype == SLAM_F32)
                hipLaunchKernelGGL(gate_kernel<float>, dim3(nblocks), dim3(GATE_BLOCK * OBS_WAVES), shmem, h->stream, zarg,
                                   (const float*)h->x, (const float*)h->P, h->ld, h->N, zc, cz, R[0], R[1], R[2], R[3],
                                   gate1, gate2, h->gate_part, (const double*)h->d_pmax, pregate, 7, (const float*)h->Pside, h->npad / 2,
                                   h->gate_blocks_cap, h->d_assoc + o, h->d_assoc, ctot, h->obsbuf, h->idfbuf, h->znbuf, h->d_count,
                                   h->h_assoc_dev, h->d_count + 2, h->h_flag_dev, h->obs_seq);
            else
                hipLaunchKernelGGL(gate_kernel<double>, dim3(nblocks), dim3(GATE_BLOCK * OBS_WAVES), shmem, h->stream, zarg,
                                   (const double*)h->x, (const double*)h->P, h->ld, h->N, zc, cz, R[0], R[1], R[2], R[3],
                                   gate1, gate2, h->gate_part, (const double*)h->d_pmax, pregate, 6, (const double*)h->Pside, h->npad / 2,
                                   h->gate_blocks_cap, h->d_assoc + o, h->d_assoc, ctot, h->obsbuf, h->idfbuf, h->znbuf, h->d_count,
                                   h->h_assoc_dev, h->d_count + 2, h->h_flag_dev, h->obs_seq);
        }
        HIP_TRY(hipGetLastError());
    }
    return SLAM_OK;
}

static int launch_single(slam_ekf* h, int j0, double z0, double z1, const double R[4], int mode) {
    if (h->dtype == SLAM_F32)
        hipLaunchKernelGGL(single_pair_kernel<float>, dim3(1), dim3(64), 0, h->stream, (const float*)h->x,
                           (const float*)h->P, h->ld, j0, z0, z1, R[0], R[1], R[2], R[3], mode, h->d_small, 7);
    else
        hipLaunchKernelGGL(single_pair_kernel<double>, dim3(1), dim3(64), 0, h->stream, (const double*)h->x,
                           (const double*)h->P, h->ld, j0, z0, z1, R[0], R[1], R[2], R[3], mode, h->d_small, 6);
    HIP_TRY(hipGetLastError());
    return SLAM_OK;
}

int launch_nis(slam_ekf* h, const double z1[2], int j, const double R[4]) {
    return launch_single(h, j - 1, z1[0], z1[1], R, 0);
}

int launch_obs_model(slam_ekf* h, int j) {
    const double R[4] = {0, 0, 0, 0};
    return launch_single(h, j - 1, 0.0, 0.0, R, 1);
}
```

### slam.jl_amd/csrc/ekf_update.hip

```cpp
#include "common.h"
#include "device_math.h"

int launch_downdate(slam_ekf* h, int kp_total, const void* X, const void* Y, int pitch, const int32_t* dcount, int joseph, int k16,
                    const void* img);

namespace {

#define SLAM_DEVICE_COUNT(dcount, m, k, kp)          \
    if (dcount) {                                    \
        m = dcount[0];                               \
        k = 2 * m;                                   \
        kp = (k + SLAM_KPAD - 1) / SLAM_KPAD * SLAM_KPAD; \
    }

constexpr int PHT_OBS = 16;
__device__ __forceinline__ double pht_entry(double h0, double h1, double h2, double h3, double h4, double p0, double p1, double p2,
                                            double q0, double q1) {
    return __builtin_fma(h4, q1, __builtin_fma(h3, q0, __builtin_fma(h2, p2, __builtin_fma(h1, p1, h0 * p0))));
}
constexpr int HB_STRIDE = 10, HB_MAXOBS = 64;

template <typename T>
__device__ __forceinline__ void pht_body(const T* __restrict__ x, const T* __restrict__ P, int ld, int n,
                                         const int32_t* __restrict__ idf, int m, int k, int kp, double* __restrict__ PHt,
                                         int pitch, int tile_log2, const int32_t* __restrict__ dcount, int row0, int by,
                                         const double* __restrict__ hblk = nullptr) {
    __shared__ double sh[PHT_OBS][10];
    __shared__ int sf[PHT_OBS];
    SLAM_DEVICE_COUNT(dcount, m, k, kp)
    const int tid = threadIdx.x;
    const int i0 = by * PHT_OBS;
    if (2 * i0 >= kp) return;
    const int mc = (m - i0 < PHT_OBS) ? m - i0 : PHT_OBS;
    if (tid < mc && hblk) {
#pragma unroll
        for (int q = 0; q < 10; ++q) sh[tid][q] = hblk[HB_STRIDE * (i0 + tid) + q];
        sf[tid] = reinterpret_cast<const int*>(hblk + HB_STRIDE * HB_MAXOBS)[i0 + tid];
    } else if (tid < mc) {
        const double xv = (double)x[0], yv = (double)x[1], phi = (double)x[2];
        const int f = 3 + 2 * (idf[i0 + tid] - 1);
        const ObsModel om = obs_model(xv, yv, phi, (double)x[f], (double)x[f + 1]);
#pragma unroll
        for (int q = 0; q < 6; ++q) sh[tid][q] = om.Hv[q];
#pragma unroll
        for (int q = 0; q < 4; ++q) sh[tid][6 + q] = om.Hf[q];
        sf[tid] = f;
    }
    __syncthreads();
    const int r = row0 + tid;
    if (r >= n) return;
    double* out = PHt + (size_t)r * pitch + 2 * i0;
    if (mc > 0) {
        const double p0 = (double)P[p_off(ld, tile_log2, r, 0)];
        const double p1 = (double)P[p_off(ld, tile_log2, r, 1)];
        const double p2 = (double)P[p_off(ld, tile_log2, r, 2)];
        T q0[PHT_OBS], q1[PHT_OBS];
#pragma unroll
        for (int i = 0; i < PHT_OBS; ++i) {
            const int f = sf[i < mc ? i : 0];
            q0[i] = sym_at(P, ld, tile_log2, r, f);
            q1[i] = sym_at(P, ld, tile_log2, r, f + 1);
        }
#pragma unroll
        for (int i = 0; i < PHT_OBS; ++i) {
            if (i < mc) {
                const double* hb = sh[i];
                out[2 * i] = pht_entry(hb[0], hb[1], hb[2], hb[6], hb[7], p0, p1, p2, (double)q0[i], (double)q1[i]);
                out[2 * i + 1] = pht_entry(hb[3], hb[4], hb[5], hb[8], hb[9], p0, p1, p2, (double)q0[i], (double)q1[i]);
            }
        }
    }
    const int c_begin = (2 * i0 > k) ? 2 * i0 : k;
    const int c_end = (2 * (i0 + PHT_OBS) < kp) ? 2 * (i0 + PHT_OBS) : kp;
    for (int c = c_begin; c < c_end; ++c) PHt[(size_t)r * pitch + c] = 0.0;
}

template <typename T>
__global__ __launch_bounds__(128) void pht_compact_kernel(const T* __restrict__ x, const T* __restrict__ P, int ld, int n,
                                                           const int32_t* __restrict__ idf, int m, int k, int kp,
                                                           double* __restrict__ PHtS, int pitch, int tile_log2,
                                                           const int32_t* __restrict__ dcount) {
    SLAM_DEVICE_COUNT(dcount, m, k, kp)
    const int slot = blockIdx.x;
    if (slot >= 3 + 2 * m) return;
    const int r = slot < 3 ? slot : 3 + 2 * (idf[(slot - 3) >> 1] - 1) + ((slot - 3) & 1);
    const double xv = (double)x[0], yv = (double)x[1], phi = (double)x[2];
    const double p0 = (double)sym_at(P, ld, tile_log2, r, 0), p1 = (double)sym_at(P, ld, tile_log2, r, 1),
                 p2 = (double)sym_at(P, ld, tile_log2, r, 2);
    double* out = PHtS + (size_t)slot * pitch;
    for (int i = threadIdx.x; i < m; i += blockDim.x) {
        const int f = 3 + 2 * (idf[i] - 1);
        const double q0 = (double)sym_at(P, ld, tile_log2, r, f), q1 = (double)sym_at(P, ld, tile_log2, r, f + 1);
        const ObsModel om = obs_model(xv, yv, phi, (double)x[f], (double)x[f + 1]);
        out[2 * i] = pht_entry(om.Hv[0], om.Hv[1], om.Hv[2], om.Hf[0], om.Hf[1], p0, p1, p2, q0, q1);
        out[2 * i + 1] = pht_entry(om.Hv[3], om.Hv[4], om.Hv[5], om.Hf[2], om.Hf[3], p0, p1, p2, q0, q1);
    }
    for (int c = k + threadIdx.x; c < kp; c += blockDim.x) out[c] = 0.0;
}

template <typename T>
__global__ __launch_bounds__(128) void s_build_kernel(const T* __restrict__ x, const T* __restrict__ P, int ld,
                                                       const int32_t* __restrict__ idf, int m, int k, int kp,
                                                       double* __restrict__ Sg, int pitch, int tile_log2,
                                                       const int32_t* __restrict__ dcount, double R0, double R1, double R2, double R3,
                                                       double* __restrict__ hblk, unsigned* __restrict__ ready) {
    if (ready && blockIdx.x == 0 && threadIdx.x == 0) ready[0] = 0u;
    SLAM_DEVICE_COUNT(dcount, m, k, kp)
    const int i = blockIdx.x;
    if (2 * i >= kp) return;
    double* row0 = Sg + (size_t)(2 * i) * pitch;
    double* row1 = row0 + pitch;
    if (i >= m) {
        for (int b = threadIdx.x; b < kp; b += blockDim.x) {
            row0[b] = (b == 2 * i) ? 1.0 : 0.0;
            row1[b] = (b == 2 * i + 1) ? 1.0 : 0.0;
        }
        return;
    }
    const double xv = (double)x[0], yv = (double)x[1], phi = (double)x[2];
    const int fi = 3 + 2 * (idf[i] - 1);
    const ObsModel oi = obs_model(xv, yv, phi, (double)x[fi], (double)x[fi + 1]);
    if (hblk && threadIdx.x == 0) {
#pragma unroll
        for (int q = 0; q < 6; ++q) hblk[HB_STRIDE * i + q] = oi.Hv[q];
#pragma unroll
        for (int q = 0; q < 4; ++q) hblk[HB_STRIDE * i + 6 + q] = oi.Hf[q];
        reinterpret_cast<int*>(hblk + HB_STRIDE * HB_MAXOBS)[i] = fi;
    }
    const int rows[5] = {0, 1, 2, fi, fi + 1};
    for (int b = threadIdx.x; b < kp; b += blockDim.x) {
        if (b >= k) {
            row0[b] = 0.0;
            row1[b] = 0.0;
            continue;
        }
        const int j = b >> 1, bb = b & 1;
        const int fj = 3 + 2 * (idf[j] - 1);
        const ObsModel oj = obs_model(xv, yv, phi, (double)x[fj], (double)x[fj + 1]);
        double pr[5][5];
#pragma unroll
        for (int t = 0; t < 5; ++t) {
            pr[t][0] = (double)sym_at(P, ld, tile_log2, rows[t], 0);
            pr[t][1] = (double)sym_at(P, ld, tile_log2, rows[t], 1);
            pr[t][2] = (double)sym_at(P, ld, tile_log2, rows[t], 2);
            pr[t][3] = (double)sym_at(P, ld, tile_log2, rows[t], fj);
            pr[t][4] = (double)sym_at(P, ld, tile_log2, rows[t], fj + 1);
        }
        double ph[5];
#pragma unroll
        for (int t = 0; t < 5; ++t)
            ph[t] = bb == 0 ? pht_entry(oj.Hv[0], oj.Hv[1], oj.Hv[2], oj.Hf[0], oj.Hf[1], pr[t][0], pr[t][1], pr[t][2], pr[t][3], pr[t][4])
                            : pht_entry(oj.Hv[3], oj.Hv[4], oj.Hv[5], oj.Hf[2], oj.Hf[3], pr[t][0], pr[t][1], pr[t][2], pr[t][3], pr[t][4]);
#pragma unroll
        for (int ra = 0; ra < 2; ++ra) {
            double sv = pht_entry(oi.Hv[3 * ra + 0], oi.Hv[3 * ra + 1], oi.Hv[3 * ra + 2], oi.Hf[2 * ra + 0], oi.Hf[2 * ra + 1], ph[0], ph[1], ph[2],
                                  ph[3], ph[4]);
            if (j == i) sv += ra ? (bb ? R3 : R1) : (bb ? R2 : R0);
            double pt[5];
#pragma unroll
            for (int t = 0; t < 5; ++t)
                pt[t] = pht_entry(oi.Hv[3 * ra + 0], oi.Hv[3 * ra + 1], oi.Hv[3 * ra + 2], oi.Hf[2 * ra + 0], oi.Hf[2 * ra + 1], pr[0][t], pr[1][t],
                                  pr[2][t], pr[3][t], pr[4][t]);
            double st = pht_entry(bb ? oj.Hv[3] : oj.Hv[0], bb ? oj.Hv[4] : oj.Hv[1], bb ? oj.Hv[5] : oj.Hv[2], bb ? oj.Hf[2] : oj.Hf[0],
                                  bb ? oj.Hf[3] : oj.Hf[1], pt[0], pt[1], pt[2], pt[3], pt[4]);
            if (j == i) st += bb ? (ra ? R3 : R1) : (ra ? R2 : R0);
            (ra ? row1 : row0)[b] = (b == 2 * i + ra) ? sv : (sv + st) * 0.5;
        }
    }
}

constexpr int FACTOR_THREADS = 512;

template <int NB>
__device__ __forceinline__ bool eliminate_in_registers(double* M, int mp, int k, int kp, double* rowbuf, double* colbuf) {
    const int tid = threadIdx.x;
    const bool worker = tid < 256;
    const int tx = tid & 15, ty = (tid >> 4) & 15;
    double a[NB][NB];
    if (worker) {
#pragma unroll
        for (int u = 0; u < NB; ++u)
#pragma unroll
            for (int v = 0; v < NB; ++v) {
                const int i = ty + 16 * u, c = tx + 16 * v;
                a[u][v] = (M[(size_t)i * mp + c] + M[(size_t)c * mp + i]) * 0.5;
            }
    }
    bool bad = false;
#pragma unroll
    for (int ub = 0; ub < NB; ++ub) {
        for (int jj = 0; jj < 16; ++jj) {
            const int j = 16 * ub + jj;
            if (j >= k || bad) break;
            double* rb = rowbuf + (j & 1) * kp;
            double* cb = colbuf + (j & 1) * kp;
            if (worker && ty == jj) {
#pragma unroll
                for (int v = 0; v < NB; ++v) rb[tx + 16 * v] = a[ub][v];
            }
            if (worker && tx == jj) {
#pragma unroll
                for (int u = 0; u < NB; ++u) cb[ty + 16 * u] = a[u][ub];
            }
            __syncthreads();
            const double piv = rb[j];
            if (!(piv > 0.0) || piv == __builtin_inf()) { bad = true; break; }
            if (worker) {
                double rp = __builtin_amdgcn_rcp(piv);
                rp = __builtin_fma(rp, __builtin_fma(-piv, rp, 1.0), rp);
                rp = __builtin_fma(rp, __builtin_fma(-piv, rp, 1.0), rp);
                double rowv[NB], colv[NB];
#pragma unroll
                for (int v = 0; v < NB; ++v) rowv[v] = rb[tx + 16 * v];
#pragma unroll
                for (int u = 0; u < NB; ++u) colv[u] = cb[ty + 16 * u];
                const bool fix = tx == jj;
#pragma unroll
                for (int u = ub; u < NB; ++u) {
                    const bool act = (u > ub) || (ty > jj);
                    const double mu = act ? colv[u] * rp : 0.0;
#pragma unroll
                    for (int v = 0; v < NB; ++v) a[u][v] = __builtin_fma(-mu, rowv[v], a[u][v]);
                    a[u][ub] = (act && fix) ? -mu : a[u][ub];
                }
            }
        }
    }
    __syncthreads();
    if (worker) {
#pragma unroll
        for (int u = 0; u < NB; ++u)
#pragma unroll
            for (int v = 0; v < NB; ++v) M[(size_t)(ty + 16 * u) * mp + tx + 16 * v] = a[u][v];
    }
    __syncthreads();
    return !bad;
}

typedef double f64x4 __attribute__((ext_vector_type(4)));

__device__ __forceinline__ double pivot_rcp(double piv) {
    double rp = __builtin_amdgcn_rcp(piv);
    rp = __builtin_fma(rp, __builtin_fma(-piv, rp, 1.0), rp);
    rp = __builtin_fma(rp, __builtin_fma(-piv, rp, 1.0), rp);
    return rp;
}

__device__ __forceinline__ double readlane_f64(double v, int srclane) {
    const long long b = __builtin_bit_cast(long long, v);
    const int lo = __builtin_amdgcn_readlane((int)(b & 0xffffffffll), srclane);
    const int hi = __builtin_amdgcn_readlane((int)(b >> 32), srclane);
    return __builtin_bit_cast(double, ((long long)hi << 32) | (unsigned int)lo);
}

__device__ __forceinline__ double bpermute_f64(double v, int srclane) {
    const long long b = __builtin_bit_cast(long long, v);
    const int lo = __builtin_amdgcn_ds_bpermute(4 * srclane, (int)(b & 0xffffffffll));
    const int hi = __builtin_amdgcn_ds_bpermute(4 * srclane, (int)(b >> 32));
    return __builtin_bit_cast(double, ((long long)hi << 32) | (unsigned int)lo);
}

__device__ __forceinline__ bool factor_diag_block4(double* M, int mp, int J, double* dvec, double* dinv) {
    const int lane = threadIdx.x & 63;
    const int c = lane & 15, q = lane >> 4;
    double* blk = M + (16 * J) * mp + 16 * J;
    f64x4 acc;
#pragma unroll
    for (int r = 0; r < 4; ++r) acc[r] = blk[(4 * r + q) * mp + c];
    bool bad = false;
#pragma unroll
    for (int s = 0; s < 4; ++s) {
        const int j0 = 4 * s;
        double rp[4];
#pragma unroll
        for (int t = 0; t < 4; ++t) {
            const int j = j0 + t;
            const double piv = readlane_f64(acc[s], j + 16 * t);
            bad = bad || !(piv > 0.0) || piv == __builtin_inf();
            rp[t] = pivot_rcp(piv);
            if (t < 3) {
                const double rowv = bpermute_f64(acc[s], c + 16 * t);
                const double muv = bpermute_f64(acc[s], (j0 + q) + 16 * t);
                const double mu = muv * rp[t];
                if (q > t) acc[s] = (c == j) ? -mu : acc[s] - mu * rowv;
            }
        }
        if (s < 3) {
            const double rpq = q == 0 ? rp[0] : (q == 1 ? rp[1] : (q == 2 ? rp[2] : rp[3]));
            const double aval = (c > j0 + 3) ? -(acc[s] * rpq) : 0.0;
            const double bval = (c == j0 + q) ? 1.0 : ((c > j0 + q && c <= j0 + 3) ? 0.0 : acc[s]);
#pragma unroll
            for (int r = 0; r < 4; ++r)
                if (r > s) acc[r] = (c >= j0 && c <= j0 + 3) ? 0.0 : acc[r];
            acc = __builtin_amdgcn_mfma_f64_16x16x4f64(aval, bval, acc, 0, 0, 0);
        }
    }
#pragma unroll
    for (int r = 0; r < 4; ++r) {
        const int row = 4 * r + q;
        blk[row * mp + c] = (c < row) ? acc[r] : (c == row ? 1.0 : 0.0);
        if (c == row) {
            dvec[16 * J + row] = acc[r];
            dinv[16 * J + row] = pivot_rcp(acc[r]);
        }
    }
    return !bad;
}

__device__ __forceinline__ bool factor_diag_block(double* M, int mp, int J, double* dvec, double* dinv) {
    const int lane = threadIdx.x & 63;
    const int c = lane & 15, q = lane >> 4;
    double* blk = M + (16 * J) * mp + 16 * J;
    f64x4 acc;
#pragma unroll
    for (int r = 0; r < 4; ++r) acc[r] = blk[(4 * r + q) * mp + c];
    bool bad = false;
#pragma unroll
    for (int j = 0; j < 16; ++j) {
        const int rj = j >> 2, qj = j & 3;
        const double rowv = bpermute_f64(acc[rj], c + 16 * qj);
        const double piv = readlane_f64(acc[rj], j + 16 * qj);
        bad = bad || !(piv > 0.0) || piv == __builtin_inf();
        const double rp = pivot_rcp(piv);
        const double aval = (q == 0 && c > j) ? -(rowv * rp) : 0.0;
        const double bval = (q == 0) ? (c == j ? 1.0 : rowv) : 0.0;
#pragma unroll
        for (int r = 0; r < 4; ++r)
            if (4 * r + 3 > j) acc[r] = (c == j && 4 * r + q > j) ? 0.0 : acc[r];
        acc = __builtin_amdgcn_mfma_f64_16x16x4f64(aval, bval, acc, 0, 0, 0);
    }
#pragma unroll
    for (int r = 0; r < 4; ++r) {
        const int row = 4 * r + q;
        blk[row * mp + c] = (c < row) ? acc[r] : (c == row ? 1.0 : 0.0);
        if (c == row) {
            dvec[16 * J + row] = acc[r];
            dinv[16 * J + row] = pivot_rcp(acc[r]);
        }
    }
    return !bad;
}

struct ProgC {
    double* C;
    int pitch, k;
    unsigned* ready;
    int mode;
    unsigned long long* stamps;
};
constexpr unsigned PC_DONE = 15u, PC_FAIL = 31u;
constexpr unsigned long long FW1_TIMEOUT = 200000000ull;
typedef unsigned pc_u32x4 __attribute__((ext_vector_type(4)));
typedef unsigned u32x2_pc __attribute__((ext_vector_type(2)));
__device__ __forceinline__ void emit_c_part(const double* M, int mp, int Jc, const double* dvec, const ProgC& pc, int wave, int lane,
                                            int nwaves) {
    const int blk = wave - 1;
    const bool diag = blk == Jc || (wave == 0 && Jc + 1 >= nwaves);
    if (!diag && !(blk >= 0 && blk < Jc)) return;
    const auto rsc = __builtin_amdgcn_make_buffer_rsrc(pc.C, (short)0, 0x7fffffff, 0x00020000);
    const int b0 = 16 * Jc + 2 * (lane & 7);
    const double m0 = b0 < pc.k ? 1.0 / sqrt(dvec[b0]) : 0.0, m1 = b0 + 1 < pc.k ? 1.0 / sqrt(dvec[b0 + 1]) : 0.0;
    const int rblk = diag ? Jc : blk;
    double v[2][2];
#pragma unroll
    for (int u = 0; u < 2; ++u) {
        const int a = 16 * rblk + (lane >> 3) + 8 * u;
        if (!diag) {
            v[u][0] = M[a * mp + b0];
            v[u][1] = M[a * mp + b0 + 1];
        } else {
            v[u][0] = a < b0 ? M[b0 * mp + a] : (a == b0 ? 1.0 : 0.0);
            v[u][1] = a < b0 + 1 ? M[(b0 + 1) * mp + a] : (a == b0 + 1 ? 1.0 : 0.0);
        }
    }
#pragma unroll
    for (int u = 0; u < 2; ++u) {
        const int a = 16 * rblk + (lane >> 3) + 8 * u;
        double c0, c1;
        if (!diag) {
            c0 = v[u][0] * m0;
            c1 = v[u][1] * m1;
        } else {
            c0 = a == b0 ? m0 : v[u][0] * m0;
            c1 = a == b0 + 1 ? m1 : v[u][1] * m1;
        }
        if (a >= pc.k || b0 >= pc.k) c0 = 0.0;
        if (a >= pc.k || b0 + 1 >= pc.k) c1 = 0.0;
        pc_u32x4 w4;
        const unsigned long long u0 = (unsigned long long)__double_as_longlong(c0), u1 = (unsigned long long)__double_as_longlong(c1);
        w4.x = (unsigned)u0; w4.y = (unsigned)(u0 >> 32); w4.z = (unsigned)u1; w4.w = (unsigned)(u1 >> 32);
        __builtin_amdgcn_raw_buffer_store_b128(w4, rsc, (unsigned)(((size_t)a * pc.pitch + b0) * 8), 0u, 16);
    }
}

__device__ __forceinline__ bool eliminate_blocked(double* M, int mp, int k, int kp, double* dvec, double* dinv, double* flag,
                                                  bool four = true, const ProgC pc = ProgC{nullptr, 0, 0, nullptr, 0, nullptr}) {
    const int tid = threadIdx.x, nt = blockDim.x;
    const int lane = tid & 63, wave = tid >> 6, nwaves = nt >> 6;
    const int li = lane & 15, kk = lane >> 4;
    const int nbk = (k + 15) >> 4;
    const int tc = tid & 31, tr = tid >> 5, trs = nt >> 5;
    for (int j = tid; j < kp; j += nt) { dvec[j] = 1.0; dinv[j] = 1.0; }
    if (tid == 0) flag[0] = 0.0;
    __syncthreads();
    auto trailing = [&](int Jp, int e0, int stride, int e_end) {
        for (int first = e0; first < e_end; first += 4 * stride) {
            f64x4 acc[4];
            double av[4][4], bv[4][4];
            int bi[4], bk[4];
#pragma unroll
            for (int q = 0; q < 4; ++q) {
                const int e = first + q * stride;
                int I = 0;
                while ((I + 1) * (I + 2) / 2 <= e) ++I;
                const int K = e - I * (I + 1) / 2;
                bi[q] = e < e_end ? Jp + 1 + I : -1;
                bk[q] = Jp + 1 + K;
                if (bi[q] < 0) continue;
#pragma unroll
                for (int r = 0; r < 4; ++r) acc[q][r] = M[(16 * bi[q] + 4 * r + kk) * mp + 16 * bk[q] + li];
#pragma unroll
                for (int s = 0; s < 4; ++s) {
                    const int kx = 4 * s + kk;
                    av[q][s] = -M[(16 * bi[q] + li) * mp + 16 * Jp + kx] * dvec[16 * Jp + kx];
                    bv[q][s] = M[(16 * bk[q] + li) * mp + 16 * Jp + kx];
                }
            }
#pragma unroll
            for (int q = 0; q < 4; ++q) {
                if (bi[q] < 0) continue;
#pragma unroll
                for (int s = 0; s < 4; ++s) acc[q] = __builtin_amdgcn_mfma_f64_16x16x4f64(av[q][s], bv[q][s], acc[q], 0, 0, 0);
#pragma unroll
                for (int r = 0; r < 4; ++r) M[(16 * bi[q] + 4 * r + kk) * mp + 16 * bk[q] + li] = acc[q][r];
            }
        }
    };
#define ESTAMP(i)                                                                                             \
    do {                                                                                                      \
        if ((pc.mode & 16) && pc.stamps && J == 3 && tid == 0) pc.stamps[8 + (i)] = wall_clock64();           \
    } while (0)
    if ((pc.mode & 16) && pc.stamps && tid == 0) pc.stamps[14] = wall_clock64();
    for (int J = 0; J < nbk; ++J) {
        ESTAMP(0);
        if (pc.ready && J > 0 && !(pc.mode & 2)) {
            if (!(pc.mode & 1)) asm volatile("s_waitcnt vmcnt(0)" ::: "memory");
            if (wave > 0) emit_c_part(M, mp, J - 1, dvec, pc, wave, lane, nwaves);
        }
        f64x4 T = {0.0, 0.0, 0.0, 0.0};
        const int C = wave - 1;
        const int tp = nbk - J;
        if (wave == 0) {
            if (J > 0) trailing(J - 1, 0, 1, 1);
            ESTAMP(1);
            const bool okb = four ? factor_diag_block4(M, mp, J, dvec, dinv) : factor_diag_block(M, mp, J, dvec, dinv);
            if (!okb && lane == 0) flag[0] = 1.0;
            ESTAMP(2);
        } else {
            if (J > 0) trailing(J - 1, wave, nwaves - 1, tp * (tp + 1) / 2);
            if (C < J) {
                for (int K = C; K < J; ++K) {
#pragma unroll
                    for (int s = 0; s < 4; ++s) {
                        const int kx = 4 * s + kk;
                        const double av = M[(16 * J + li) * mp + 16 * K + kx];
                        const double bv = (K == C) ? M[(16 * C + kx) * mp + 16 * C + li]
                                                   : M[(16 * C + li) * mp + 16 * K + kx];
                        T = __builtin_amdgcn_mfma_f64_16x16x4f64(av, bv, T, 0, 0, 0);
                    }
                }
            }
        }
        __syncthreads();
        ESTAMP(3);
        if (pc.ready && !(pc.mode & 3) && J >= 2 && tid == nt - 1 && flag[0] == 0.0) __hip_atomic_store(pc.ready, (unsigned)(J - 1), __ATOMIC_RELAXED, __HIP_MEMORY_SCOPE_AGENT);
        if (wave >= 1 && C < J) {
            f64x4 acc = {0.0, 0.0, 0.0, 0.0};
#pragma unroll
            for (int s = 0; s < 4; ++s)
                acc = __builtin_amdgcn_mfma_f64_16x16x4f64(M[(16 * J + li) * mp + 16 * J + 4 * s + kk], T[s], acc, 0, 0, 0);
#pragma unroll
            for (int r = 0; r < 4; ++r) M[(16 * C + li) * mp + 16 * J + 4 * r + kk] = -acc[r];
        } else if (wave > J && wave < nbk) {
            const int I = wave;
            f64x4 acc = {0.0, 0.0, 0.0, 0.0};
#pragma unroll
            for (int s = 0; s < 4; ++s) {
                const int kx = 4 * s + kk;
                acc = __builtin_amdgcn_mfma_f64_16x16x4f64(M[(16 * I + li) * mp + 16 * J + kx],
                                                           M[(16 * J + li) * mp + 16 * J + kx], acc, 0, 0, 0);
            }
            const double di = dinv[16 * J + li];
#pragma unroll
            for (int r = 0; r < 4; ++r) M[(16 * I + 4 * r + kk) * mp + 16 * J + li] = acc[r] * di;
        }
        ESTAMP(4);
        __syncthreads();
        ESTAMP(5);
    }
#undef ESTAMP
    if ((pc.mode & 16) && pc.stamps && tid == 0) pc.stamps[15] = wall_clock64();
    if (pc.ready) {
        if (flag[0] == 0.0) {
            if (pc.mode & 2)
                for (int Jc = 0; Jc < nbk - 1; ++Jc) emit_c_part(M, mp, Jc, dvec, pc, wave, lane, nwaves);
            emit_c_part(M, mp, nbk - 1, dvec, pc, wave, lane, nwaves);
        }
        for (int j = tid; j < kp; j += nt) M[(size_t)j * mp + j] = dvec[j];
        asm volatile("s_waitcnt vmcnt(0)" ::: "memory");
        __syncthreads();
        const bool good = flag[0] == 0.0;
        if (good && tid == 0) __hip_atomic_store(pc.ready, (unsigned)nbk, __ATOMIC_RELAXED, __HIP_MEMORY_SCOPE_AGENT);
        return good;
    }
    for (int b = tr; b < kp; b += trs) {
        double v[4];
#pragma unroll
        for (int u = 0; u < 4; ++u) {
            const int a = tc + 32 * u;
            const bool low = a < kp && (b >> 4) > (a >> 4);
            v[u] = (low && (b >> 4) < nbk) ? M[(size_t)a * mp + b] : 0.0;
        }
#pragma unroll
        for (int u = 0; u < 4; ++u) {
            const int a = tc + 32 * u;
            if (a < kp && (b >> 4) > (a >> 4)) M[(size_t)b * mp + a] = v[u];
        }
    }
    for (int j = tid; j < kp; j += nt) M[(size_t)j * mp + j] = dvec[j];
    __syncthreads();
    return flag[0] == 0.0;
}

__device__ inline bool eliminate_in_memory(double* M, int mp, int k, double* mvec) {
    const int tid = threadIdx.x, nt = blockDim.x;
    for (int j = 0; j < k; ++j) {
        const double piv = M[(size_t)j * mp + j];
        if (!(piv > 0.0) || piv == __builtin_inf()) return false;
        const double rp = 1.0 / piv;
        for (int i = j + 1 + tid; i < k; i += nt) mvec[i] = M[(size_t)i * mp + j] * rp;
        __syncthreads();
        const int rows = k - j - 1;
        for (int idx = tid; idx < rows * k; idx += nt) {
            const int ii = idx / k;
            const int c = idx - ii * k;
            const int i = j + 1 + ii;
            const double mi = mvec[i];
            if (c == j) M[(size_t)i * mp + j] = -mi;
            else M[(size_t)i * mp + c] -= mi * M[(size_t)j * mp + c];
        }
        __syncthreads();
    }
    return true;
}

template <typename T, bool INLDS>
__device__ __forceinline__ void factor_body(
    const T* __restrict__ x, const double* __restrict__ PHt, int pht_pitch, const double* __restrict__ z,
    const int32_t* __restrict__ idf, int m, int k, int kp, double R0, double R1, double R2, double R3,
    double* __restrict__ Cout, int c_pitch, double* __restrict__ gvec, double* __restrict__ Sout, int want_sinv,
    double* __restrict__ Mglobal, int32_t* __restrict__ status, unsigned long long* __restrict__ stamps,
    const int32_t* __restrict__ dcount, int blocked, unsigned* __restrict__ ready = nullptr, int mode = 0) {
#define STAMP(i)                                                  \
    do {                                                          \
        if (stamps && threadIdx.x == 0) stamps[i] = wall_clock64(); \
    } while (0)
    extern __shared__ double lds[];
    STAMP(0);
    SLAM_DEVICE_COUNT(dcount, m, k, kp)
    if (m == 0) {
        if (threadIdx.x == 0) status[0] = 0;
        return;
    }
    const int tid = threadIdx.x;
    const int nt = blockDim.x;
    const int mp = kp + 1;
    double* M;
    double* aux;
    if constexpr (INLDS) {
        M = lds;
        aux = lds + (size_t)kp * mp;
    } else {
        M = Mglobal;
        aux = lds;
    }
    double* mvec = aux;
    double* vvec = aux + kp;
    double* yvec = aux + 2 * kp;
    double* rowbuf = aux + 3 * kp;
    double* colbuf = aux + 5 * kp;
    double* hb = aux + 7 * kp;
    int* sf = reinterpret_cast<int*>(hb + (size_t)10 * m);

    if (tid == 0) status[0] = 0;
    const double xv = (double)x[0], yv = (double)x[1], phi = (double)x[2];
    for (int i = tid; i < m; i += nt) {
        const int f = 3 + 2 * (idf[i] - 1);
        const ObsModel om = obs_model(xv, yv, phi, (double)x[f], (double)x[f + 1]);
        for (int q = 0; q < 6; ++q) hb[10 * i + q] = om.Hv[q];
        for (int q = 0; q < 4; ++q) hb[10 * i + 6 + q] = om.Hf[q];
        sf[i] = f;
        vvec[2 * i] = z[2 * i] - om.zp[0];
        vvec[2 * i + 1] = mpi_to_pi_d(z[2 * i + 1] - om.zp[1]);
    }
    for (int a = k + tid; a < kp; a += nt) vvec[a] = 0.0;
    __syncthreads();
    STAMP(1);

    if constexpr (INLDS) {
        const int a0 = tid >> 5, bcol = tid & 31;
        for (int u0 = 0; u0 < kp; u0 += 8 * (nt >> 5)) {
            double v[8][4];
#pragma unroll
            for (int u = 0; u < 8; ++u)
#pragma unroll
                for (int w = 0; w < 4; ++w) {
                    const int a = u0 + a0 + u * (nt >> 5), b = bcol + 32 * w;
                    v[u][w] = (a < kp && b < kp) ? PHt[(size_t)a * pht_pitch + b] : 0.0;
                }
#pragma unroll
            for (int u = 0; u < 8; ++u)
#pragma unroll
                for (int w = 0; w < 4; ++w) {
                    const int a = u0 + a0 + u * (nt >> 5), b = bcol + 32 * w;
                    if (a < kp && b < kp) M[(size_t)a * mp + b] = v[u][w];
                }
        }
    } else {
    for (int a = tid >> 5; a < kp; a += nt >> 5)
        for (int b = tid & 31; b < kp; b += 32) {
        double s;
        if (a < k && b < k) {
            const int i = a >> 1, ra = a & 1;
            const double* h = hb + 10 * i;
            s = h[3 * ra + 0] * PHt[(size_t)0 * pht_pitch + b] + h[3 * ra + 1] * PHt[(size_t)1 * pht_pitch + b] +
                h[3 * ra + 2] * PHt[(size_t)2 * pht_pitch + b] + h[6 + 2 * ra + 0] * PHt[(size_t)(3 + 2 * i) * pht_pitch + b] +
                h[6 + 2 * ra + 1] * PHt[(size_t)(4 + 2 * i) * pht_pitch + b];
            if ((b >> 1) == i) s += ra ? ((b & 1) ? R3 : R1) : ((b & 1) ? R2 : R0);
        } else {
            s = (a == b) ? 1.0 : 0.0;
        }
        M[(size_t)a * mp + b] = s;
    }
    }
    __syncthreads();
    STAMP(2);
    if constexpr (!INLDS) {
        for (int idx = tid; idx < k * k; idx += nt) {
            const int a = idx / k, b = idx - a * k;
            if (a < b) {
                const double s = (M[(size_t)a * mp + b] + M[(size_t)b * mp + a]) * 0.5;
                M[(size_t)a * mp + b] = s;
                M[(size_t)b * mp + a] = s;
            }
        }
        __syncthreads();
    }
    if (Sout) {
        for (int a = tid >> 5; a < kp; a += nt >> 5)
            for (int b = tid & 31; b < kp; b += 32) {
            Sout[(size_t)a * c_pitch + b] =
                (a < k && b < k) ? (M[(size_t)a * mp + b] + M[(size_t)b * mp + a]) * 0.5 : 0.0;
        }
        __syncthreads();
    }
    STAMP(3);
    bool ok;
    if constexpr (!INLDS) ok = eliminate_in_memory(M, mp, k, mvec);
    else if (blocked) {
        const ProgC pcs{Cout, c_pitch, k, ready, mode, stamps};
        ok = eliminate_blocked(M, mp, k, kp, rowbuf, rowbuf + kp, colbuf, blocked != 2, pcs);
    }
    else if (kp == 32) ok = eliminate_in_registers<2>(M, mp, k, kp, rowbuf, colbuf);
    else if (kp == 64) ok = eliminate_in_registers<4>(M, mp, k, kp, rowbuf, colbuf);
    else if (kp == 96) ok = eliminate_in_registers<6>(M, mp, k, kp, rowbuf, colbuf);
    else ok = eliminate_in_registers<8>(M, mp, k, kp, rowbuf, colbuf);
    if (!ok) {
        if (tid == 0) {
            status[0] = 1; status[1] = 1;
            if (ready) __hip_atomic_store(ready, PC_FAIL, __ATOMIC_RELAXED, __HIP_MEMORY_SCOPE_AGENT);
        }
        return;
    }
    STAMP(4);
    for (int b = tid; b < kp; b += nt) mvec[b] = (b < k) ? 1.0 / sqrt(M[(size_t)b * mp + b]) : 0.0;
    __syncthreads();
    const bool up = ready != nullptr;
    for (int b0 = 0; b0 < kp; b0 += nt / 8) {
        const int b = b0 + (tid >> 3), part = tid & 7;
        double s = 0.0;
        if (b < k)
            for (int a = part; a < b; a += 8) s += ((up && (a >> 4) < (b >> 4)) ? M[(size_t)a * mp + b] : M[(size_t)b * mp + a]) * vvec[a];
        s += __shfl_xor(s, 1);
        s += __shfl_xor(s, 2);
        s += __shfl_xor(s, 4);
        if (part == 0 && b < kp) yvec[b] = (b < k) ? (s + vvec[b]) * mvec[b] : 0.0;
    }
    __syncthreads();
    for (int a0 = 0; a0 < kp; a0 += nt / 8) {
        const int a = a0 + (tid >> 3), part = tid & 7;
        double s = 0.0;
        if (a < k)
            for (int b = a + 1 + part; b < k; b += 8) s += ((up && (a >> 4) < (b >> 4)) ? M[(size_t)a * mp + b] : M[(size_t)b * mp + a]) * mvec[b] * yvec[b];
        s += __shfl_xor(s, 1);
        s += __shfl_xor(s, 2);
        s += __shfl_xor(s, 4);
        if (part == 0 && a < kp) {
            const double gv = (a < k) ? s + yvec[a] * mvec[a] : 0.0;
            if (ready) __hip_atomic_store(gvec + a, gv, __ATOMIC_RELAXED, __HIP_MEMORY_SCOPE_AGENT);
            else gvec[a] = gv;
        }
    }
    STAMP(5);
    if (ready) {
        asm volatile("s_waitcnt vmcnt(0)" ::: "memory");
        __syncthreads();
        if (tid == 0) __hip_atomic_store(ready, PC_DONE, __ATOMIC_RELAXED, __HIP_MEMORY_SCOPE_AGENT);
    } else if (!want_sinv) {
        if (kp < 96) {
            for (int a = tid >> 5; a < kp; a += nt >> 5)
                for (int b = tid & 31; b < kp; b += 32) {
                    double c = 0.0;
                    if (a < k && b < k) {
                        if (a == b) c = mvec[b];
                        else if (a < b) c = M[(size_t)b * mp + a] * mvec[b];
                    }
                    Cout[(size_t)a * c_pitch + b] = c;
                }
        } else
        for (int bb = 0; bb < kp; bb += 128)
        for (int a0 = tid >> 5; a0 < kp; a0 += 4 * (nt >> 5)) {
            double v[4][4], mv[4];
#pragma unroll
            for (int w = 0; w < 4; ++w) {
                const int b = bb + (tid & 31) + 32 * w;
                mv[w] = b < kp ? mvec[b] : 0.0;
#pragma unroll
                for (int u = 0; u < 4; ++u) {
                    const int a = a0 + u * (nt >> 5);
                    v[u][w] = (a < b && b < k) ? M[(size_t)b * mp + a] : 0.0;
                }
            }
#pragma unroll
            for (int u = 0; u < 4; ++u) {
                const int a = a0 + u * (nt >> 5);
#pragma unroll
                for (int w = 0; w < 4; ++w) {
                    const int b = bb + (tid & 31) + 32 * w;
                    double c = 0.0;
                    if (a < k && b < k) c = a == b ? mv[w] : (a < b ? v[u][w] * mv[w] : 0.0);
                    if (a < kp && b < kp) Cout[(size_t)a * c_pitch + b] = c;
                }
            }
        }
    } else {
        for (int a = tid >> 5; a < kp; a += nt >> 5)
            for (int b = tid & 31; b < kp; b += 32) {
            double s = 0.0;
            if (a < k && b < k) {
                const int c0 = a > b ? a : b;
                for (int c = c0; c < k; ++c) {
                    const double ca = (c == a) ? 1.0 : M[(size_t)c * mp + a];
                    const double cb = (c == b) ? 1.0 : M[(size_t)c * mp + b];
                    s += ca * cb * mvec[c] * mvec[c];
                }
            }
            Cout[(size_t)a * c_pitch + b] = s;
        }
    }
    STAMP(6);
#undef STAMP
}

template <typename T, bool INLDS>
__global__ __launch_bounds__(FACTOR_THREADS) void factor_kernel(
    const T* __restrict__ x, const double* __restrict__ PHtS, int pht_pitch, const double* __restrict__ z,
    const int32_t* __restrict__ idf, int m, int k, int kp, double R0, double R1, double R2, double R3,
    double* __restrict__ Cout, int c_pitch, double* __restrict__ gvec, double* __restrict__ Sout, int want_sinv,
    double* __restrict__ Mglobal, int32_t* __restrict__ status, unsigned long long* __restrict__ stamps,
    const int32_t* __restrict__ dcount, int blocked, const T* __restrict__ P, int ld, int n, double* __restrict__ PHt,
    int tile_log2, int nbx, const double* __restrict__ hblk) {
    if (blockIdx.x == 0) {
        factor_body<T, INLDS>(x, PHtS, pht_pitch, z, idf, m, k, kp, R0, R1, R2, R3, Cout, c_pitch, gvec, Sout, want_sinv, Mglobal,
                              status, stamps, dcount, blocked);
    } else {
        const int b = blockIdx.x - 1;
        pht_body<T>(x, P, ld, n, idf, m, k, kp, PHt, pht_pitch, tile_log2, dcount, (b % nbx) * FACTOR_THREADS, b / nbx, hblk);
    }
}

constexpr int PG_ROWS = 64;
constexpr int PG_COLS = 64;
constexpr int PG_KC = 32;

template <typename TO>
__global__ __launch_bounds__(256) void panel_gemm_kernel(const double* __restrict__ IN, int in_pitch,
                                                          const double* __restrict__ MAT, int mat_pitch, int kp, int upper,
                                                          double alpha, const double* __restrict__ ADD, int add_pitch,
                                                          double beta, TO* __restrict__ OUT1, int out1_pitch, int out1_col,
                                                          TO* __restrict__ OUT2, int out2_pitch, int out2_col,
                                                          double* __restrict__ OUTD, int outd_pitch,
                                                          const int32_t* __restrict__ status,
                                                          const int32_t* __restrict__ dcount) {
    if (status[0] != 0) return;
    if (dcount) {
        const int kp_host = kp;
        int m = 0, k = 0;
        SLAM_DEVICE_COUNT(dcount, m, k, kp)
        if (out1_col == kp_host) out1_col = kp;
        if (out2_col == kp_host) out2_col = kp;
        if ((int)(blockIdx.y * PG_COLS) >= kp) return;
    }
    __shared__ double sIn[PG_ROWS][PG_KC + 1];
    __shared__ __attribute__((aligned(16))) double sMat[PG_KC][PG_COLS];
    const int tid = threadIdx.x;
    const int tr = tid & 31;
    const int tc = tid >> 5;
    const int row0 = blockIdx.x * PG_ROWS;
    const int b0 = blockIdx.y * PG_COLS;
    const int bw = (kp - b0 < PG_COLS) ? kp - b0 : PG_COLS;
    double acc[2][8];
#pragma unroll
    for (int u = 0; u < 2; ++u)
#pragma unroll
        for (int q = 0; q < 8; ++q) acc[u][q] = 0.0;
    const int a_end = upper ? (b0 + bw) : kp;
    double gi[8], gm[8];
    const int irow = tid >> 5, icol = tid & 31;
    const int mrow = tid >> 6, mcol = tid & 63;
    const double* isrc = IN + (size_t)(row0 + irow) * in_pitch + icol;
    const double* msrc = MAT + (size_t)mrow * mat_pitch + b0 + mcol;
    const bool mvalid = mcol < bw;
#pragma unroll
    for (int s = 0; s < 8; ++s) {
        gi[s] = isrc[(size_t)(8 * s) * in_pitch];
        gm[s] = mvalid ? msrc[(size_t)(4 * s) * mat_pitch] : 0.0;
    }
    for (int a0 = 0; a0 < a_end; a0 += PG_KC) {
#pragma unroll
        for (int s = 0; s < 8; ++s) {
            sIn[irow + 8 * s][icol] = gi[s];
            sMat[mrow + 4 * s][mcol] = gm[s];
        }
        __syncthreads();
        if (a0 + PG_KC < a_end) {
#pragma unroll
            for (int s = 0; s < 8; ++s) {
                gi[s] = isrc[(size_t)(8 * s) * in_pitch + a0 + PG_KC];
                gm[s] = mvalid ? msrc[(size_t)(a0 + PG_KC + 4 * s) * mat_pitch] : 0.0;
            }
        }
#pragma unroll 8
        for (int a = 0; a < PG_KC; ++a) {
            const double p0 = sIn[tr][a], p1 = sIn[tr + 32][a];
#pragma unroll
            for (int q = 0; q < 8; ++q) {
                const double mv = sMat[a][tc * 8 + q];
                acc[0][q] = __builtin_fma(p0, mv, acc[0][q]);
                acc[1][q] = __builtin_fma(p1, mv, acc[1][q]);
            }
        }
        __syncthreads();
    }
#pragma unroll
    for (int u = 0; u < 2; ++u) {
        const size_t row = (size_t)(row0 + tr + 32 * u);
#pragma unroll
        for (int q = 0; q < 8; ++q) {
            const int b = b0 + tc * 8 + q;
            if (b >= kp) continue;
            double v = alpha * acc[u][q];
            if (ADD) v += beta * ADD[row * add_pitch + b];
            OUT1[row * out1_pitch + out1_col + b] = (TO)v;
            if (OUT2) OUT2[row * out2_pitch + out2_col + b] = (TO)v;
            if (OUTD) OUTD[row * outd_pitch + b] = v;
        }
    }
}

typedef double f64x2 __attribute__((ext_vector_type(2)));
constexpr int W1_THREADS = 512;

__device__ __forceinline__ void split_bf16(float v, unsigned short& h, unsigned short& m, unsigned short& l) {
    typedef __bf16 bf1;
    asm volatile("" : "+v"(v));
    const bf1 bh = (bf1)v;
    const float r1 = v - (float)bh;
    const bf1 bm = (bf1)r1;
    const float r2 = r1 - (float)bm;
    const bf1 bl = (bf1)r2;
    h = __builtin_bit_cast(unsigned short, bh);
    m = __builtin_bit_cast(unsigned short, bm);
    l = __builtin_bit_cast(unsigned short, bl);
}

__device__ __forceinline__ double fmax_nan(double a, double b) { return (a != a || a > b) ? a : b; }

template <typename TO, int NCB>
__device__ __forceinline__ void w1_mfma_body(const double* __restrict__ PHt, int pitchA, const double* __restrict__ Cmat,
                                             int pitchC, double* sC, TO* __restrict__ W1, int pitchW, TO* __restrict__ x,
                                             int n, const double* __restrict__ g, char* __restrict__ img, int img_nch,
                                             unsigned long long* __restrict__ drift, int dbg) {
    constexpr int kp = 16 * NCB;
    const int lane = threadIdx.x & 63, wave = threadIdx.x >> 6;
    const int i = lane & 15, kk = lane >> 4;
    const int r0 = (blockIdx.x * (W1_THREADS / 64) + wave) * 16;
    f64x2 a[NCB * 2];
    const double* arow = PHt + (size_t)(r0 + i) * pitchA + 2 * kk;
#pragma unroll
    for (int s = 0; s < NCB * 2; ++s) a[s] = *reinterpret_cast<const f64x2*>(arow + 8 * s);
    constexpr int PER = kp * kp / W1_THREADS;
    constexpr int BATCH = PER < 16 ? PER : 16;
#pragma unroll
    for (int base = 0; base < PER; base += BATCH) {
        double v[BATCH];
#pragma unroll
        for (int u = 0; u < BATCH; ++u) {
            const int idx = (base + u) * W1_THREADS + threadIdx.x;
            const int ar = idx / kp, c = idx % kp;
            v[u] = (base + u < PER && ar <= c) ? Cmat[(size_t)ar * pitchC + c] : 0.0;
        }
#pragma unroll
        for (int u = 0; u < BATCH; ++u)
            if (base + u < PER) sC[(base + u) * W1_THREADS + threadIdx.x] = v[u];
    }
    f64x4 acc[NCB];
#pragma unroll
    for (int cb = 0; cb < NCB; ++cb) acc[cb] = f64x4{0.0, 0.0, 0.0, 0.0};
    __syncthreads();
#pragma unroll
    for (int s = 0; s < NCB * 2; ++s) {
#pragma unroll
        for (int t = 0; t < 2; ++t) {
            const double* brow = sC + (size_t)(8 * s + 2 * kk + t) * kp + i;
#pragma unroll
            for (int cb = s / 2; cb < NCB; ++cb)
                acc[cb] = __builtin_amdgcn_mfma_f64_16x16x4f64(a[s][t], brow[16 * cb], acc[cb], 0, 0, 0);
        }
    }
    if (!(dbg & 2)) {
#pragma unroll
    for (int cb = 0; cb < NCB; ++cb)
#pragma unroll
        for (int r = 0; r < 4; ++r)
            W1[(size_t)(r0 + 4 * r + kk) * pitchW + 16 * cb + i] = (TO)acc[cb][r];
    }
    if (img && !(dbg & 1)) {
#pragma unroll
        for (int cb = 0; cb < NCB; ++cb)
#pragma unroll
            for (int r = 0; r < 4; ++r) {
                const int rr = (r0 & 127) + 4 * r + kk;
                unsigned short hh, mm, ll;
                split_bf16((float)acc[cb][r], hh, mm, ll);
                char* d = img + ((size_t)(blockIdx.x * img_nch + cb) * 3) * 4096 + rr * 32 + ((((i >> 3) ^ (rr >> 3)) & 1) * 16) + (i & 7) * 2;
                *reinterpret_cast<unsigned short*>(d) = hh;
                *reinterpret_cast<unsigned short*>(d + 4096) = mm;
                *reinterpret_cast<unsigned short*>(d + 8192) = ll;
            }
    }
    double sx = 0.0;
#pragma unroll
    for (int s = 0; s < NCB * 2; ++s) {
        const f64x2 gg = *reinterpret_cast<const f64x2*>(g + 8 * s + 2 * kk);
        sx = __builtin_fma(a[s][0], gg[0], sx);
        sx = __builtin_fma(a[s][1], gg[1], sx);
    }
    sx += __shfl_xor(sx, 16);
    sx += __shfl_xor(sx, 32);
    double moved = 0.0;
    if (kk == 0 && r0 + i < n) {
        const double xo = (double)x[r0 + i];
        const TO xn = (TO)(xo + sx);
        x[r0 + i] = xn;
        if (r0 + i >= 3) moved = fabs((double)xn - xo);
    }
    if (drift) {
        __shared__ double s_moved[W1_THREADS / 64];
        moved = fmax_nan(moved, __shfl_xor(moved, 1));
        moved = fmax_nan(moved, __shfl_xor(moved, 2));
        moved = fmax_nan(moved, __shfl_xor(moved, 4));
        moved = fmax_nan(moved, __shfl_xor(moved, 8));
        if (lane == 0) s_moved[wave] = moved;
        __syncthreads();
        if (threadIdx.x == 0) {
#pragma unroll
            for (int w = 1; w < W1_THREADS / 64; ++w) moved = fmax_nan(moved, s_moved[w]);
            if (!(moved == 0.0)) atomicMax(drift + (blockIdx.x & 15) * SLAM_GRID_SLOTS, (unsigned long long)__double_as_longlong(moved));
        }
    }
}

template <typename TO>
__global__ __launch_bounds__(W1_THREADS) void w1_mfma_kernel(const double* __restrict__ PHt, int pitchA,
                                                             const double* __restrict__ Cmat, int pitchC, int kp,
                                                             TO* __restrict__ W1, int pitchW, TO* __restrict__ x, int n,
                                                             const double* __restrict__ g,
                                                             const int32_t* __restrict__ status,
                                                             const int32_t* __restrict__ dcount, char* __restrict__ img,
                                                             int img_nch, unsigned* __restrict__ dd_claim,
                                                             unsigned long long* __restrict__ drift, int dbg) {
    if (dd_claim && blockIdx.x == 0 && threadIdx.x < 128) dd_claim[threadIdx.x] = 0u;
    if (status[0] != 0) return;
    if (dcount) {
        int m = 0, k = 0;
        SLAM_DEVICE_COUNT(dcount, m, k, kp)
        if (m == 0) return;
    }
    extern __shared__ double sC[];
    if (kp == 32) w1_mfma_body<TO, 2>(PHt, pitchA, Cmat, pitchC, sC, W1, pitchW, x, n, g, img, img_nch, drift, dbg);
    else if (kp == 64) w1_mfma_body<TO, 4>(PHt, pitchA, Cmat, pitchC, sC, W1, pitchW, x, n, g, img, img_nch, drift, dbg);
    else if (kp == 96) w1_mfma_body<TO, 6>(PHt, pitchA, Cmat, pitchC, sC, W1, pitchW, x, n, g, img, img_nch, drift, dbg);
    else w1_mfma_body<TO, 8>(PHt, pitchA, Cmat, pitchC, sC, W1, pitchW, x, n, g, img, img_nch, drift, dbg);
}


template <typename T>
__device__ __forceinline__ T ld_agent(const T* p) { return __hip_atomic_load(p, __ATOMIC_RELAXED, __HIP_MEMORY_SCOPE_AGENT); }

template <typename TO, int NCB>
__device__ __forceinline__ void w1_stream_body(const TO* __restrict__ P, int ld, int tile_log2, int n, int npad, int m, int k,
                                               const double* __restrict__ hblk, const double* __restrict__ Cmat, int pitchC,
                                               double* lds, TO* __restrict__ W1, int pitchW, TO* __restrict__ x,
                                               const double* __restrict__ g, char* __restrict__ img, int img_nch,
                                               unsigned long long* __restrict__ drift, const unsigned* __restrict__ ready,
                                               unsigned long long* __restrict__ stamps, int wpw, int mode, int32_t* __restrict__ status) {
#define CSTAMP(i)                                                                        \
    do {                                                                                 \
        if (stamps && !(mode & 16) && blockIdx.x == 1 && threadIdx.x == 0) stamps[8 + (i)] = wall_clock64(); \
    } while (0)
    CSTAMP(0);
    double* sh = lds;
    const int* sfs = reinterpret_cast<const int*>(sh + HB_STRIDE * HB_MAXOBS);
    const int tid = threadIdx.x, lane = tid & 63, wave = tid >> 6;
    const int i = lane & 15, kk = lane >> 4;
    const int rb = blockIdx.x - 1;
    const int r0 = (rb * wpw + wave) * 16;
    const bool act = wave < wpw && r0 < npad;
    for (int t = tid; t < HB_STRIDE * HB_MAXOBS + HB_MAXOBS / 2; t += FACTOR_THREADS) sh[t] = hblk[t];
    __syncthreads();
    double moved = 0.0;
    if (act) {
        f64x2 a[NCB * 2];
        {
            const int r = r0 + i;
            const bool live = r < n;
            const int rr = live ? r : 0;
            const double p0 = (double)P[p_off(ld, tile_log2, rr, 0)];
            const double p1 = (double)P[p_off(ld, tile_log2, rr, 1)];
            const double p2 = (double)P[p_off(ld, tile_log2, rr, 2)];
            TO q0[NCB * 2], q1[NCB * 2];
#pragma unroll
            for (int s = 0; s < NCB * 2; ++s) {
                const int ob = 4 * s + kk;
                const int f = sfs[ob < m ? ob : 0];
                q0[s] = sym_at(P, ld, tile_log2, rr, f);
                q1[s] = sym_at(P, ld, tile_log2, rr, f + 1);
            }
#pragma unroll
            for (int s = 0; s < NCB * 2; ++s) {
                const int ob = 4 * s + kk;
                const double* hb = sh + HB_STRIDE * (ob < m ? ob : 0);
                const double v0 = pht_entry(hb[0], hb[1], hb[2], hb[6], hb[7], p0, p1, p2, (double)q0[s], (double)q1[s]);
                const double v1 = pht_entry(hb[3], hb[4], hb[5], hb[8], hb[9], p0, p1, p2, (double)q0[s], (double)q1[s]);
                double a0 = (live && ob < m) ? v0 : 0.0, a1 = (live && ob < m) ? v1 : 0.0;
                asm volatile("" : "+v"(a0), "+v"(a1));
                a[s][0] = a0;
                a[s][1] = a1;
            }
        }
        CSTAMP(1);
        const int nbk = (k + 15) >> 4;
        const auto rsc = __builtin_amdgcn_make_buffer_rsrc(const_cast<double*>(Cmat), (short)0, 0x7fffffff, 0x00020000);
        auto wait_for = [&](unsigned need) __attribute__((always_inline)) {
            unsigned v = 0;
            if (lane == 0) {
                const unsigned long long t0 = wall_clock64();
                while ((v = ld_agent(ready)) < need) {
                    __builtin_amdgcn_s_sleep(16);
                    if (wall_clock64() - t0 > FW1_TIMEOUT) {
                        status[0] = 2; status[1] = 2;
                        v = PC_FAIL;
                        break;
                    }
                }
            }
            return (unsigned)__builtin_amdgcn_readfirstlane((int)v);
        };
        auto put = [&](int cb, const f64x4& v) __attribute__((always_inline)) {
            if (mode & 4) return;
#pragma unroll
            for (int r = 0; r < 4; ++r) W1[(size_t)(r0 + 4 * r + kk) * pitchW + 16 * cb + i] = (TO)v[r];
            if (img) {
#pragma unroll
                for (int r = 0; r < 4; ++r) {
                    const int rr = (r0 & 127) + 4 * r + kk;
                    unsigned short hh, mm, ll;
                    split_bf16((float)v[r], hh, mm, ll);
                    char* d = img + ((size_t)((r0 >> 7) * img_nch + cb) * 3) * 4096 + rr * 32 + ((((i >> 3) ^ (rr >> 3)) & 1) * 16) + (i & 7) * 2;
                    *reinterpret_cast<unsigned short*>(d) = hh;
                    *reinterpret_cast<unsigned short*>(d + 4096) = mm;
                    *reinterpret_cast<unsigned short*>(d + 8192) = ll;
                }
            }
        };
        unsigned rdy = 0;
        bool failed = false;
        f64x4 acc[NCB];
#pragma unroll
        for (int cb = 0; cb < NCB; ++cb) {
            acc[cb] = f64x4{0.0, 0.0, 0.0, 0.0};
            if (cb < nbk && !failed) {
                if (rdy < (unsigned)(cb + 1)) rdy = wait_for((unsigned)(cb + 1));
                failed = rdy == PC_FAIL;
                if (cb == 0) CSTAMP(2);
                if (cb == nbk - 1) CSTAMP(3);
                if (!failed) {
                    double bv[2 * NCB][2];
#pragma unroll
                    for (int s = 0; s < 2 * cb + 2; ++s)
#pragma unroll
                        for (int t = 0; t < 2; ++t) {
                            const u32x2_pc w2 = __builtin_amdgcn_raw_buffer_load_b64(rsc, (unsigned)(((size_t)(8 * s + 2 * kk + t) * pitchC + 16 * cb + i) * 8), 0u, 0);
                            bv[s][t] = __longlong_as_double((long long)((unsigned long long)w2.x | ((unsigned long long)w2.y << 32)));
                        }
                    if (!(mode & 8)) {
#pragma unroll
                        for (int s = 0; s < 2 * cb + 2; ++s)
#pragma unroll
                            for (int t = 0; t < 2; ++t) acc[cb] = __builtin_amdgcn_mfma_f64_16x16x4f64(a[s][t], bv[s][t], acc[cb], 0, 0, 0);
                    }
                }
            }
            if (cb > 0 && !failed) put(cb - 1, acc[cb - 1]);
        }
        if (!failed) put(NCB - 1, acc[NCB - 1]);
        CSTAMP(4);
        if (!failed && rdy != PC_DONE) {
            rdy = wait_for(PC_DONE);
            failed = rdy == PC_FAIL;
        }
        CSTAMP(5);
        if (!failed) {
            const auto rsg = __builtin_amdgcn_make_buffer_rsrc(const_cast<double*>(g), (short)0, 0x7fffffff, 0x00020000);
            double sx = 0.0;
            pc_u32x4 gw[NCB * 2];
#pragma unroll
            for (int s = 0; s < NCB * 2; ++s) gw[s] = __builtin_amdgcn_raw_buffer_load_b128(rsg, (unsigned)((8 * s + 2 * kk) * 8), 0u, 0);
#pragma unroll
            for (int s = 0; s < NCB * 2; ++s) {
                const double g0 = __longlong_as_double((long long)((unsigned long long)gw[s].x | ((unsigned long long)gw[s].y << 32)));
                const double g1 = __longlong_as_double((long long)((unsigned long long)gw[s].z | ((unsigned long long)gw[s].w << 32)));
                sx = __builtin_fma(a[s][0], g0, sx);
                sx = __builtin_fma(a[s][1], g1, sx);
            }
            sx += __shfl_xor(sx, 16);
            sx += __shfl_xor(sx, 32);
            if (kk == 0 && r0 + i < n) {
                const double xo = (double)x[r0 + i];
                const TO xn = (TO)(xo + sx);
                x[r0 + i] = xn;
                if (r0 + i >= 3) moved = fabs((double)xn - xo);
            }
        }
    }
    if (drift) {
        __shared__ double s_moved[FACTOR_THREADS / 64];
        moved = fmax_nan(moved, __shfl_xor(moved, 1));
        moved = fmax_nan(moved, __shfl_xor(moved, 2));
        moved = fmax_nan(moved, __shfl_xor(moved, 4));
        moved = fmax_nan(moved, __shfl_xor(moved, 8));
        if (lane == 0) s_moved[wave] = moved;
        __syncthreads();
        if (tid == 0) {
#pragma unroll
            for (int w = 1; w < FACTOR_THREADS / 64; ++w) moved = fmax_nan(moved, s_moved[w]);
            if (!(moved == 0.0)) atomicMax(drift + (rb & 15) * SLAM_GRID_SLOTS, (unsigned long long)__double_as_longlong(moved));
        }
    }
    CSTAMP(6);
#undef CSTAMP
}

template <typename T>
__global__ __launch_bounds__(FACTOR_THREADS) void factor_w1_kernel(
    T* __restrict__ x, const double* __restrict__ Sg, int s_pitch, const double* __restrict__ z,
    const int32_t* __restrict__ idf, int m, int k, int kp, double R0, double R1, double R2, double R3,
    double* __restrict__ Cout, int c_pitch, double* __restrict__ gvec, int32_t* __restrict__ status,
    unsigned long long* __restrict__ stamps, const int32_t* __restrict__ dcount, int blocked, const T* __restrict__ P, int ld,
    int n, int npad, int tile_log2, const double* __restrict__ hblk, T* __restrict__ W1, int pitchW, char* __restrict__ img, int img_nch,
    unsigned* __restrict__ dd_claim, unsigned long long* __restrict__ drift, unsigned* __restrict__ sync, int wpw, int mode) {
    if (blockIdx.x == 0) {
        if (mode & 32) return;
        factor_body<T, true>(x, Sg, s_pitch, z, idf, m, k, kp, R0, R1, R2, R3, Cout, c_pitch, gvec, (double*)nullptr, 0, (double*)nullptr,
                             status, stamps, dcount, blocked, sync, mode);
        return;
    }
    if (dd_claim && blockIdx.x == 1 && threadIdx.x < 128) dd_claim[threadIdx.x] = 0u;
    SLAM_DEVICE_COUNT(dcount, m, k, kp)
    if (m == 0) return;
    extern __shared__ double lds[];
    if (kp == 32) w1_stream_body<T, 2>(P, ld, tile_log2, n, npad, m, k, hblk, Cout, c_pitch, lds, W1, pitchW, x, gvec, img, img_nch, drift, sync, stamps, wpw, mode, status);
    else if (kp == 64) w1_stream_body<T, 4>(P, ld, tile_log2, n, npad, m, k, hblk, Cout, c_pitch, lds, W1, pitchW, x, gvec, img, img_nch, drift, sync, stamps, wpw, mode, status);
    else if (kp == 96) w1_stream_body<T, 6>(P, ld, tile_log2, n, npad, m, k, hblk, Cout, c_pitch, lds, W1, pitchW, x, gvec, img, img_nch, drift, sync, stamps, wpw, mode, status);
    else w1_stream_body<T, 8>(P, ld, tile_log2, n, npad, m, k, hblk, Cout, c_pitch, lds, W1, pitchW, x, gvec, img, img_nch, drift, sync, stamps, wpw, mode, status);
}

template <typename T>
__global__ __launch_bounds__(256) void x_update_kernel(T* __restrict__ x, const double* __restrict__ PHt, int pitch, int n,
                                                        int k, const double* __restrict__ g,
                                                        const int32_t* __restrict__ status,
                                                        const int32_t* __restrict__ dcount,
                                                        unsigned long long* __restrict__ drift) {
    if (status[0] != 0) return;
    if (dcount) k = 2 * dcount[0];
    const int r = blockIdx.x * 32 + (threadIdx.x >> 3);
    const int part = threadIdx.x & 7;
    double s = 0.0;
    if (r < n) {
        const double* row = PHt + (size_t)r * pitch;
        for (int a = part; a < k; a += 8) s += row[a] * g[a];
    }
    s += __shfl_xor(s, 1);
    s += __shfl_xor(s, 2);
    s += __shfl_xor(s, 4);
    double moved = 0.0;
    if (part == 0 && r < n) {
        const double xo = (double)x[r];
        const T xn = (T)(xo + s);
        x[r] = xn;
        if (r >= 3) moved = fabs((double)xn - xo);
    }
    if (drift) {
        __shared__ double s_moved[4];
        moved = fmax_nan(moved, __shfl_xor(moved, 8));
        moved = fmax_nan(moved, __shfl_xor(moved, 16));
        moved = fmax_nan(moved, __shfl_xor(moved, 32));
        if ((threadIdx.x & 63) == 0) s_moved[threadIdx.x >> 6] = moved;
        __syncthreads();
        if (threadIdx.x == 0) {
            for (int w = 1; w < 4; ++w) moved = fmax_nan(moved, s_moved[w]);
            if (!(moved == 0.0)) atomicMax(drift + (blockIdx.x & 15) * SLAM_GRID_SLOTS, (unsigned long long)__double_as_longlong(moved));
        }
    }
}

template <typename T>
int update_typed(slam_ekf* h, int m, const double R[4], int form, const int32_t* dcount) {
    const int n = 3 + 2 * h->N;
    const int k = 2 * m;
    const int kp = round_up(k, SLAM_KPAD);
    const int pitchA = h->kcap;
    const int pitchW = 2 * h->kcap;
    T* x = (T*)h->x;
    T* P = (T*)h->P;
    T* W1 = (T*)h->W1;
    T* W2 = (T*)h->W2;
    const bool joseph = form == SLAM_FORM_JOSEPH;
    unsigned long long* drift = grid_drift_slot(h);

    const int tlog = h->dtype == SLAM_F32 ? 7 : 6;
    const bool fused = !joseph && kp <= 128 && h->factor_blocked == 1 && !(h->xflags & 128);
    double* hblk = h->Smat;
    {
        KTimer t(h, SLAM_K_PHT);
        if (kp <= 128)
            hipLaunchKernelGGL(s_build_kernel<T>, dim3(kp / 2), dim3(128), 0, h->stream, x, P, h->ld, h->idfbuf, m, k, kp, h->PHtS,
                               pitchA, tlog, dcount, R[0], R[1], R[2], R[3], joseph ? (double*)nullptr : hblk,
                               fused ? reinterpret_cast<unsigned*>(h->d_small + 56) : (unsigned*)nullptr);
        else
            hipLaunchKernelGGL(pht_compact_kernel<T>, dim3(3 + 2 * m), dim3(128), 0, h->stream, x, P, h->ld, n, h->idfbuf, m, k, kp,
                               h->PHtS, pitchA, tlog, dcount);
    }
    HIP_TRY(hipGetLastError());
    {
        KTimer t(h, SLAM_K_FACTOR);
        const bool in_lds = kp <= 128;
        const int nbx = (n + FACTOR_THREADS - 1) / FACTOR_THREADS, nby = kp / (2 * PHT_OBS);
        const dim3 fgrid(1 + nbx * nby);
        const size_t aux = (size_t)7 * kp * sizeof(double) + (size_t)m * (10 * sizeof(double) + sizeof(int));
        const size_t shm = aux + (in_lds ? (size_t)kp * (kp + 1) * sizeof(double) : 0);
        unsigned long long* stamps = h->debug_stamps ? (unsigned long long*)(h->d_small + 40) : (unsigned long long*)nullptr;
        if (fused) {
            const bool img = h->dtype == SLAM_F32 && h->Wimg && !(h->xflags & 16);
            const size_t need = (size_t)(HB_STRIDE * HB_MAXOBS + HB_MAXOBS / 2) * sizeof(double);
            const int groups = h->npad / 16, room = h->num_cus >= 16 ? h->num_cus * 7 / 8 : 1;
            int wpw = (groups + room - 1) / room;
            wpw = wpw < 1 ? 1 : (wpw > FACTOR_THREADS / 64 ? FACTOR_THREADS / 64 : wpw);
            wpw = slam_exp_env("SLAMHIP_FW1_WPW", wpw);
            hipLaunchKernelGGL(factor_w1_kernel<T>, dim3(1 + (groups + wpw - 1) / wpw), dim3(FACTOR_THREADS), shm > need ? shm : need, h->stream, x,
                               (const double*)h->PHtS, pitchA, (const double*)h->obsbuf, (const int32_t*)h->idfbuf, m, k, kp, R[0], R[1],
                               R[2], R[3], h->Cmat, pitchA, h->gvec, h->d_status, stamps, dcount, h->factor_blocked, (const T*)P, h->ld, n,
                               h->npad, tlog, (const double*)hblk, W1, pitchW, img ? (char*)h->Wimg : (char*)nullptr, h->kcap / 16,
                               img ? h->dd_claim : (unsigned*)nullptr, drift, reinterpret_cast<unsigned*>(h->d_small + 56), wpw,
                               slam_exp_env("SLAMHIP_FW1", 0));
        } else if (in_lds)
            hipLaunchKernelGGL((factor_kernel<T, true>), fgrid, dim3(FACTOR_THREADS), shm, h->stream, x, h->PHtS, pitchA,
                               h->obsbuf, h->idfbuf, m, k, kp, R[0], R[1], R[2], R[3], h->Cmat, pitchA, h->gvec,
                               joseph ? h->Smat : (double*)nullptr, joseph ? 1 : 0, (double*)nullptr, h->d_status, stamps, dcount, h->factor_blocked,
                               (const T*)P, h->ld, n, h->PHt, tlog, nbx, joseph ? (const double*)nullptr : (const double*)hblk);
        else
            hipLaunchKernelGGL((factor_kernel<T, false>), fgrid, dim3(FACTOR_THREADS), shm, h->stream, x, h->PHtS, pitchA,
                               h->obsbuf, h->idfbuf, m, k, kp, R[0], R[1], R[2], R[3], h->Cmat, pitchA, h->gvec,
                               joseph ? h->Smat : (double*)nullptr, joseph ? 1 : 0, h->Mwork, h->d_status, stamps, dcount, 0,
                               (const T*)P, h->ld, n, h->PHt, tlog, nbx, (const double*)nullptr);
    }
    HIP_TRY(hipGetLastError());
    const dim3 pg_grid(h->npad / PG_ROWS, (kp + PG_COLS - 1) / PG_COLS);
    int kp_total;
    bool use_img = false;
    use_img = !joseph && kp <= 128 && h->dtype == SLAM_F32 && h->Wimg && !(h->xflags & 16);
    if (fused) {
        kp_total = round_up(k, 16);
    } else {
        KTimer t(h, SLAM_K_W1);
        if (!joseph && kp <= 128) {
            hipLaunchKernelGGL(w1_mfma_kernel<T>, dim3(h->npad / 128), dim3(W1_THREADS), (size_t)kp * kp * sizeof(double),
                               h->stream, (const double*)h->PHt, pitchA, (const double*)h->Cmat, pitchA, kp, W1, pitchW, x, n,
                               (const double*)h->gvec, h->d_status, dcount, use_img ? (char*)h->Wimg : (char*)nullptr, h->kcap / 16,
                               use_img ? h->dd_claim : (unsigned*)nullptr, drift, slam_exp_env("SLAMHIP_W1DBG", 0));
            kp_total = round_up(k, 16);
        } else if (!joseph) {
            hipLaunchKernelGGL(panel_gemm_kernel<T>, pg_grid, dim3(256), 0, h->stream, h->PHt, pitchA, h->Cmat, pitchA, kp, 1,
                               1.0, (const double*)nullptr, 0, 0.0, W1, pitchW, 0, (T*)nullptr, 0, 0, (double*)nullptr, 0,
                               h->d_status, dcount);
            kp_total = round_up(k, 16);
        } else {
            hipLaunchKernelGGL(panel_gemm_kernel<T>, pg_grid, dim3(256), 0, h->stream, h->PHt, pitchA, h->Cmat, pitchA, kp, 0,
                               1.0, (const double*)nullptr, 0, 0.0, W1, pitchW, 0, W2, pitchW, kp, h->Kd, pitchA,
                               h->d_status, dcount);
            hipLaunchKernelGGL(panel_gemm_kernel<T>, pg_grid, dim3(256), 0, h->stream, (const double*)h->Kd, pitchA,
                               (const double*)h->Smat, pitchA, kp, 0, -0.5, (const double*)h->PHt, pitchA, 1.0, W1, pitchW,
                               kp, W2, pitchW, 0, (double*)nullptr, 0, h->d_status, dcount);
            kp_total = 2 * kp;
        }
        if (joseph || kp > 128)
            hipLaunchKernelGGL(x_update_kernel<T>, dim3((n + 31) / 32), dim3(256), 0, h->stream, x, h->PHt, pitchA, n, k,
                               h->gvec, h->d_status, dcount, drift);
    }
    HIP_TRY(hipGetLastError());
    return launch_downdate(h, kp_total, W1, joseph ? (const void*)W2 : (const void*)W1, pitchW, dcount, joseph ? 1 : 0, round_up(k, 16),
                           use_img ? h->Wimg : nullptr);
}

}

int launch_update(slam_ekf* h, int m, const double R[4], int form, bool device_count) {
    if (form == SLAM_FORM_JOSEPH) h->pmax_valid = 0;
    const int32_t* dcount = device_count ? h->d_count : (const int32_t*)nullptr;
    return h->dtype == SLAM_F32 ? update_typed<float>(h, m, R, form, dcount) : update_typed<double>(h, m, R, form, dcount);
}

int update_kernels_init() {
    const int big = 160 * 1024;
    HIP_TRY(hipFuncSetAttribute(reinterpret_cast<const void*>(&w1_mfma_kernel<float>),
                                hipFuncAttributeMaxDynamicSharedMemorySize, big - 1024));
    HIP_TRY(hipFuncSetAttribute(reinterpret_cast<const void*>(&w1_mfma_kernel<double>),
                                hipFuncAttributeMaxDynamicSharedMemorySize, big - 1024));
    const int fbig = big - 4096;
    HIP_TRY(hipFuncSetAttribute(reinterpret_cast<const void*>(&factor_kernel<float, true>),
                                hipFuncAttributeMaxDynamicSharedMemorySize, fbig));
    HIP_TRY(hipFuncSetAttribute(reinterpret_cast<const void*>(&factor_kernel<double, true>),
                                hipFuncAttributeMaxDynamicSharedMemorySize, fbig));
    HIP_TRY(hipFuncSetAttribute(reinterpret_cast<const void*>(&factor_w1_kernel<float>), hipFuncAttributeMaxDynamicSharedMemorySize, fbig));
    HIP_TRY(hipFuncSetAttribute(reinterpret_cast<const void*>(&factor_w1_kernel<double>), hipFuncAttributeMaxDynamicSharedMemorySize, fbig));
    return SLAM_OK;
}
```

Before: 143,100 obs-updates/s (one observation assimilated = one update).

## Fuse innovation-covariance build into gate kernel via extra spin-waiting blocks

Appends builder blocks to the gate kernel grid. Each one spin-waits on a sequence-tagged ready word published by the compaction wave, then builds its two rows of S and the H blocks, so the separate s_build kernel launch is dropped in Cholesky form. The factor kernel also prefetches S tiles into registers before the blocked elimination and writes the trailing tiles into LDS late, overlapping the load with the first panel step. The cost is intra-kernel spin-waiting that depends on co-residency of the builder and sweep blocks, guarded by a timeout and a fail status, plus a new xflag to disable the path.

New measurement: 144,000 obs-updates/s (one observation assimilated = one update) (median of 6 runs). Within noise of the previous version (+0.7%).

```diff
diff --git a/slam.jl_amd/csrc/common.h b/slam.jl_amd/csrc/common.h
--- a/slam.jl_amd/csrc/common.h
+++ b/slam.jl_amd/csrc/common.h
@@ -55,7 +55,7 @@
 constexpr int SLAM_XFLAGS_MASK = ~0;
 #else
 static inline int slam_exp_env(const char*, int dflt) { return dflt; }
-constexpr int SLAM_XFLAGS_MASK = 4 | 8 | 16 | 32 | 64 | 128 | 512 | 65536;
+constexpr int SLAM_XFLAGS_MASK = 4 | 8 | 16 | 32 | 64 | 128 | 512 | 65536 | 131072;
 #endif
 
 struct TimingPair {
@@ -105,6 +105,7 @@
     int32_t* h_flag;
     int32_t* h_flag_dev;
     int32_t obs_seq;
+    int s_built;
 
     int2* tiles;
     int tiles_T, tiles_len, tiles_cap;
@@ -173,7 +174,7 @@
 int launch_copy_floor(slam_ekf* h, int reps, double out[2]);
 int launch_predict(slam_ekf* h, double v, double g, double w, const double Q[4], double dt);
 int launch_augment(slam_ekf* h, int nn, const double R[4], const double* zn_dev);
-int launch_gate(slam_ekf* h, int nz, const double R[4], double gate1, double gate2, const double* z_host, bool compact);
+int launch_gate(slam_ekf* h, int nz, const double R[4], double gate1, double gate2, const double* z_host, bool compact, bool build_s = false);
 constexpr int SLAM_GRID_SLOTS = 64;
 int gate_kernels_init();
 int gate_info(slam_ekf* h, int64_t out[8]);
@@ -184,3 +185,88 @@
 int launch_update(slam_ekf* h, int m, const double R[4], int form, bool device_count);
 int ensure_update_workspace(slam_ekf* h, int m);
 int ensure_obs_capacity(slam_ekf* h, int nobs);
+
+#include "device_math.h"
+
+__device__ __forceinline__ double pht_entry(double h0, double h1, double h2, double h3, double h4, double p0, double p1, double p2,
+                                            double q0, double q1) {
+    return __builtin_fma(h4, q1, __builtin_fma(h3, q0, __builtin_fma(h2, p2, __builtin_fma(h1, p1, h0 * p0))));
+}
+constexpr int HB_STRIDE = 10, HB_MAXOBS = 64;
+constexpr unsigned PC_DONE = 15u, PC_FAIL = 31u;
+constexpr unsigned long long FW1_TIMEOUT = 200000000ull;
+
+template <typename T>
+__device__ __forceinline__ void s_build_rows(const T* __restrict__ x, const T* __restrict__ P, int ld, const int32_t* idf, int i, int m,
+                                             int k, int kp, double* __restrict__ Sg, int pitch, int tile_log2, double R0, double R1,
+                                             double R2, double R3, double* __restrict__ hblk) {
+    if (2 * i >= kp) return;
+    double* row0 = Sg + (size_t)(2 * i) * pitch;
+    double* row1 = row0 + pitch;
+    const int b = threadIdx.x;
+    if (b >= kp) return;
+    if (i >= m) {
+        row0[b] = (b == 2 * i) ? 1.0 : 0.0;
+        row1[b] = (b == 2 * i + 1) ? 1.0 : 0.0;
+        return;
+    }
+    const int j = b < k ? b >> 1 : i, bb = b & 1;
+    const int idi = __hip_atomic_load(idf + i, __ATOMIC_RELAXED, __HIP_MEMORY_SCOPE_AGENT);
+    const int idj = __hip_atomic_load(idf + j, __ATOMIC_RELAXED, __HIP_MEMORY_SCOPE_AGENT);
+    const double xv = (double)x[0], yv = (double)x[1], phi = (double)x[2];
+    const int fi = 3 + 2 * (idi - 1), fj = 3 + 2 * (idj - 1);
+    const double lxi = (double)x[fi], lyi = (double)x[fi + 1], lxj = (double)x[fj], lyj = (double)x[fj + 1];
+    const ObsModel oi = obs_model(xv, yv, phi, lxi, lyi);
+    if (hblk && threadIdx.x == 0) {
+#pragma unroll
+        for (int q = 0; q < 6; ++q) hblk[HB_STRIDE * i + q] = oi.Hv[q];
+#pragma unroll
+        for (int q = 0; q < 4; ++q) hblk[HB_STRIDE * i + 6 + q] = oi.Hf[q];
+        reinterpret_cast<int*>(hblk + HB_STRIDE * HB_MAXOBS)[i] = fi;
+    }
+    const int rows[5] = {0, 1, 2, fi, fi + 1};
+    if (b >= k) {
+        row0[b] = 0.0;
+        row1[b] = 0.0;
+        return;
+    }
+    const ObsModel oj = obs_model(xv, yv, phi, lxj, lyj);
+    double pr[5][5];
+#pragma unroll
+    for (int t = 0; t < 5; ++t) {
+        pr[t][0] = (double)sym_at(P, ld, tile_log2, rows[t], 0);
+        pr[t][1] = (double)sym_at(P, ld, tile_log2, rows[t], 1);
+        pr[t][2] = (double)sym_at(P, ld, tile_log2, rows[t], 2);
+        pr[t][3] = (double)sym_at(P, ld, tile_log2, rows[t], fj);
+        pr[t][4] = (double)sym_at(P, ld, tile_log2, rows[t], fj + 1);
+    }
+    double ph[5];
+#pragma unroll
+    for (int t = 0; t < 5; ++t)
+        ph[t] = bb == 0 ? pht_entry(oj.Hv[0], oj.Hv[1], oj.Hv[2], oj.Hf[0], oj.Hf[1], pr[t][0], pr[t][1], pr[t][2], pr[t][3], pr[t][4])
+                        : pht_entry(oj.Hv[3], oj.Hv[4], oj.Hv[5], oj.Hf[2], oj.Hf[3], pr[t][0], pr[t][1], pr[t][2], pr[t][3], pr[t][4]);
+#pragma unroll
+    for (int ra = 0; ra < 2; ++ra) {
+        double sv = pht_entry(oi.Hv[3 * ra + 0], oi.Hv[3 * ra + 1], oi.Hv[3 * ra + 2], oi.Hf[2 * ra + 0], oi.Hf[2 * ra + 1], ph[0], ph[1], ph[2],
+                              ph[3], ph[4]);
+        if (j == i) sv += ra ? (bb ? R3 : R1) : (bb ? R2 : R0);
+        double pt[5];
+#pragma unroll
+        for (int t = 0; t < 5; ++t)
+            pt[t] = pht_entry(oi.Hv[3 * ra + 0], oi.Hv[3 * ra + 1], oi.Hv[3 * ra + 2], oi.Hf[2 * ra + 0], oi.Hf[2 * ra + 1], pr[0][t], pr[1][t],
+                              pr[2][t], pr[3][t], pr[4][t]);
+        double st = pht_entry(bb ? oj.Hv[3] : oj.Hv[0], bb ? oj.Hv[4] : oj.Hv[1], bb ? oj.Hv[5] : oj.Hv[2], bb ? oj.Hf[2] : oj.Hf[0],
+                              bb ? oj.Hf[3] : oj.Hf[1], pt[0], pt[1], pt[2], pt[3], pt[4]);
+        if (j == i) st += bb ? (ra ? R3 : R1) : (ra ? R2 : R0);
+        (ra ? row1 : row0)[b] = (b == 2 * i + ra) ? sv : (sv + st) * 0.5;
+    }
+}
+
+struct SBuildArgs {
+    double* Sg;
+    double* hblk;
+    unsigned* ready;
+    unsigned long long* sready;
+    int32_t* status;
+    int pitch, nbuild;
+};
diff --git a/slam.jl_amd/csrc/ekf_api.hip b/slam.jl_amd/csrc/ekf_api.hip
--- a/slam.jl_amd/csrc/ekf_api.hip
+++ b/slam.jl_amd/csrc/ekf_api.hip
@@ -316,7 +316,7 @@
     h->d_pmax = nullptr; h->pmax_valid = 0; h->dd_claim = nullptr;
     h->gate_mode = SLAM_GATE_AUTO; h->gate_last = 0; h->grid_meta = nullptr; h->grid_cells = nullptr; h->grid_items = nullptr;
     h->grid_force = 1; h->grid_upd = 0; h->grid_live = 0; h->grid_n_seen = 0;
-    h->znbuf = nullptr; h->d_count = nullptr; h->h_flag = nullptr; h->h_flag_dev = nullptr; h->obs_seq = 0;
+    h->znbuf = nullptr; h->d_count = nullptr; h->h_flag = nullptr; h->h_flag_dev = nullptr; h->obs_seq = 0; h->s_built = 0;
     h->d_status = h->h_status = nullptr;
     h->async_updates = 0; h->deferred = 0; h->pending_status = 0; h->debug_stamps = 0;
     h->debug_flags = 0;
@@ -835,7 +835,7 @@
     if ((rc = ensure_update_workspace(h, nz))) return rc;
     if ((rc = ensure_obs_capacity(h, nz))) return rc;
     h->obs_seq = h->obs_seq == 0x7fffffff ? 1 : h->obs_seq + 1;
-    if ((rc = launch_gate(h, nz, R, gate1, gate2, z, true))) return rc;
+    if ((rc = launch_gate(h, nz, R, gate1, gate2, z, true, form == SLAM_FORM_CHOLESKY && !(h->xflags & 131072)))) return rc;
     if ((rc = launch_update(h, nz, R, form, true))) return rc;
     {
         volatile int32_t* flag = h->h_flag;
diff --git a/slam.jl_amd/csrc/ekf_gate.hip b/slam.jl_amd/csrc/ekf_gate.hip
--- a/slam.jl_amd/csrc/ekf_gate.hip
+++ b/slam.jl_amd/csrc/ekf_gate.hip
@@ -116,7 +116,7 @@
                                              double* zbuf, int32_t* __restrict__ idf,
                                              double* __restrict__ zn, int32_t* __restrict__ count,
                                              int32_t* __restrict__ assoc_host, int lane, int32_t* __restrict__ flag_host,
-                                             int32_t seq) {
+                                             int32_t seq, unsigned long long* sready = nullptr) {
     int m = 0, nn = 0;
     for (int base = 0; base < nz; base += 64) {
         const int i = base + lane;
@@ -138,7 +138,7 @@
         __builtin_amdgcn_wave_barrier();
         if (a > 0) {
             const int pos = m + __popcll(mm & below);
-            idf[pos] = a;
+            __hip_atomic_store(idf + pos, a, __ATOMIC_RELAXED, __HIP_MEMORY_SCOPE_AGENT);
             zbuf[2 * pos] = z0;
             zbuf[2 * pos + 1] = z1;
         } else if (a < 0) {
@@ -155,6 +155,8 @@
     }
     asm volatile("s_waitcnt vmcnt(0)" ::: "memory");
     __builtin_amdgcn_wave_barrier();
+    if (lane == 0 && sready)
+        __hip_atomic_store(sready, ((unsigned long long)(unsigned)seq << 32) | (unsigned)m, __ATOMIC_RELAXED, __HIP_MEMORY_SCOPE_AGENT);
     if (lane == 0) __hip_atomic_store(flag_host, seq, __ATOMIC_RELAXED, __HIP_MEMORY_SCOPE_SYSTEM);
 }
 
@@ -163,6 +165,38 @@
 struct GateObs {
     double z[2 * GATE_CHUNK];
 };
+
+template <typename T>
+__device__ __forceinline__ void s_builder(const T* __restrict__ x, const T* __restrict__ P, int ld, int tlog, const int32_t* idf,
+                                          double R0, double R1, double R2, double R3, int32_t seq, const SBuildArgs& sb, int i) {
+    if (threadIdx.x >= 128) return;
+    int ok = 0, m = 0;
+    if ((threadIdx.x & 63) == 0) {
+        const unsigned long long t0 = wall_clock64();
+        ok = 1;
+        unsigned long long v;
+        while ((unsigned)((v = __hip_atomic_load(sb.sready, __ATOMIC_RELAXED, __HIP_MEMORY_SCOPE_AGENT)) >> 32) != (unsigned)seq) {
+            __builtin_amdgcn_s_sleep(2);
+            if (wall_clock64() - t0 > FW1_TIMEOUT) {
+                ok = 0;
+                break;
+            }
+        }
+        m = (int)(unsigned)v;
+    }
+    ok = __builtin_amdgcn_readfirstlane(ok);
+    m = __builtin_amdgcn_readfirstlane(m);
+    if (!ok) {
+        if (threadIdx.x == 0) {
+            sb.status[0] = 2; sb.status[1] = 2;
+            if (sb.ready) __hip_atomic_store(sb.ready, PC_FAIL, __ATOMIC_RELAXED, __HIP_MEMORY_SCOPE_AGENT);
+        }
+        return;
+    }
+    if (sb.ready && i == 0 && threadIdx.x == 0) sb.ready[0] = 0u;
+    const int k = 2 * m, kp = (k + SLAM_KPAD - 1) / SLAM_KPAD * SLAM_KPAD;
+    s_build_rows<T>(x, P, ld, idf, i, m, k, kp, sb.Sg, sb.pitch, tlog, R0, R1, R2, R3, sb.hblk);
+}
 
 template <typename T>
 __global__ __launch_bounds__(GATE_BLOCK * OBS_WAVES) void gate_kernel(GateObs zarg, const T* __restrict__ x, const T* __restrict__ P,
@@ -173,7 +207,12 @@
                                                            int part_cap, int32_t* assoc, int32_t* assoc_all, int compact_total,
                                                            double* zbuf, int32_t* __restrict__ idf, double* __restrict__ zn,
                                                            int32_t* __restrict__ count, int32_t* __restrict__ assoc_host, int32_t* arrive,
-                                                           int32_t* __restrict__ flag_host, int32_t seq) {
+                                                           int32_t* __restrict__ flag_host, int32_t seq, SBuildArgs sb) {
+    const int nsweep = (int)gridDim.x - sb.nbuild;
+    if ((int)blockIdx.x >= nsweep) {
+        s_builder<T>(x, P, ld, tlog, idf, R0, R1, R2, R3, seq, sb, (int)blockIdx.x - nsweep);
+        return;
+    }
     extern __shared__ double smem[];
     double* zs = smem;
     double* red = smem + 2 * nz;
@@ -255,7 +294,7 @@
     asm volatile("s_waitcnt vmcnt(0)" ::: "memory");
     __syncthreads();
     int* const s_last = reinterpret_cast<int*>(red);
-    if (tid == 0) *s_last = __hip_atomic_fetch_add(arrive, 1, __ATOMIC_RELAXED, __HIP_MEMORY_SCOPE_AGENT) == (int)gridDim.x - 1 ? 1 : 0;
+    if (tid == 0) *s_last = __hip_atomic_fetch_add(arrive, 1, __ATOMIC_RELAXED, __HIP_MEMORY_SCOPE_AGENT) == nsweep - 1 ? 1 : 0;
     __syncthreads();
     if (!*s_last) return;
     for (int i = tid; i < nz; i += NT) {
@@ -280,7 +319,8 @@
     if (compact_total > 0) {
         asm volatile("s_waitcnt vmcnt(0)" ::: "memory");
         __syncthreads();
-        if (wave == 0) compact_wave<true>(assoc_all, compact_total, zdev_base(zdev, zbuf), zbuf, idf, zn, count, assoc_host, lane, flag_host, seq);
+        if (wave == 0) compact_wave<true>(assoc_all, compact_total, zdev_base(zdev, zbuf), zbuf, idf, zn, count, assoc_host, lane, flag_host, seq,
+                                          sb.nbuild > 0 ? sb.sready : (unsigned long long*)nullptr);
     }
 }
 
@@ -755,7 +795,8 @@
     return SLAM_OK;
 }
 
-int launch_gate(slam_ekf* h, int nz, const double R[4], double gate1, double gate2, const double* z_host, bool compact) {
+int launch_gate(slam_ekf* h, int nz, const double R[4], double gate1, double gate2, const double* z_host, bool compact, bool build_s) {
+    h->s_built = 0;
     const int nblocks = (h->N + GATE_BLOCK - 1) / GATE_BLOCK;
     if (nblocks > h->gate_blocks_cap) {
         slam_set_error("internal: gate partial buffer too small");
@@ -787,18 +828,31 @@
             KTimer t(h, SLAM_K_GATE);
             const bool last = o + CHUNK >= nz;
             const int ctot = (compact && last) ? nz : 0;
+            SBuildArgs sb{};
+            const int kp_max = round_up(2 * nz, SLAM_KPAD);
+            if (build_s && ctot > 0 && kp_max <= 128 && h->kcap >= kp_max) {
+                sb.Sg = h->PHtS;
+                sb.hblk = h->Smat;
+                sb.ready = reinterpret_cast<unsigned*>(h->d_small + 56);
+                sb.sready = reinterpret_cast<unsigned long long*>(h->d_small + 57);
+                sb.status = h->d_status;
+                sb.pitch = h->kcap;
+                sb.nbuild = kp_max / 2;
+                h->s_built = 1;
+            }
+            const int grid = nblocks + sb.nbuild;
             if (h->dtype == SLAM_F32)
-                hipLaunchKernelGGL(gate_kernel<float>, dim3(nblocks), dim3(GATE_BLOCK * OBS_WAVES), shmem, h->stream, zarg,
+                hipLaunchKernelGGL(gate_kernel<float>, dim3(grid), dim3(GATE_BLOCK * OBS_WAVES), shmem, h->stream, zarg,
                                    (const float*)h->x, (const float*)h->P, h->ld, h->N, zc, cz, R[0], R[1], R[2], R[3],
                                    gate1, gate2, h->gate_part, (const double*)h->d_pmax, pregate, 7, (const float*)h->Pside, h->npad / 2,
                                    h->gate_blocks_cap, h->d_assoc + o, h->d_assoc, ctot, h->obsbuf, h->idfbuf, h->znbuf, h->d_count,
-                                   h->h_assoc_dev, h->d_count + 2, h->h_flag_dev, h->obs_seq);
+                                   h->h_assoc_dev, h->d_count + 2, h->h_flag_dev, h->obs_seq, sb);
             else
-                hipLaunchKernelGGL(gate_kernel<double>, dim3(nblocks), dim3(GATE_BLOCK * OBS_WAVES), shmem, h->stream, zarg,
+                hipLaunchKernelGGL(gate_kernel<double>, dim3(grid), dim3(GATE_BLOCK * OBS_WAVES), shmem, h->stream, zarg,
                                    (const double*)h->x, (const double*)h->P, h->ld, h->N, zc, cz, R[0], R[1], R[2], R[3],
                                    gate1, gate2, h->gate_part, (const double*)h->d_pmax, pregate, 6, (const double*)h->Pside, h->npad / 2,
                                    h->gate_blocks_cap, h->d_assoc + o, h->d_assoc, ctot, h->obsbuf, h->idfbuf, h->znbuf, h->d_count,
-                                   h->h_assoc_dev, h->d_count + 2, h->h_flag_dev, h->obs_seq);
+                                   h->h_assoc_dev, h->d_count + 2, h->h_flag_dev, h->obs_seq, sb);
         }
         HIP_TRY(hipGetLastError());
     }
diff --git a/slam.jl_amd/csrc/ekf_update.hip b/slam.jl_amd/csrc/ekf_update.hip
--- a/slam.jl_amd/csrc/ekf_update.hip
+++ b/slam.jl_amd/csrc/ekf_update.hip
@@ -14,12 +14,6 @@
     }
 
 constexpr int PHT_OBS = 16;
-__device__ __forceinline__ double pht_entry(double h0, double h1, double h2, double h3, double h4, double p0, double p1, double p2,
-                                            double q0, double q1) {
-    return __builtin_fma(h4, q1, __builtin_fma(h3, q0, __builtin_fma(h2, p2, __builtin_fma(h1, p1, h0 * p0))));
-}
-constexpr int HB_STRIDE = 10, HB_MAXOBS = 64;
-
 template <typename T>
 __device__ __forceinline__ void pht_body(const T* __restrict__ x, const T* __restrict__ P, int ld, int n,
                                          const int32_t* __restrict__ idf, int m, int k, int kp, double* __restrict__ PHt,
@@ -106,67 +100,7 @@
                                                        double* __restrict__ hblk, unsigned* __restrict__ ready) {
     if (ready && blockIdx.x == 0 && threadIdx.x == 0) ready[0] = 0u;
     SLAM_DEVICE_COUNT(dcount, m, k, kp)
-    const int i = blockIdx.x;
-    if (2 * i >= kp) return;
-    double* row0 = Sg + (size_t)(2 * i) * pitch;
-    double* row1 = row0 + pitch;
-    if (i >= m) {
-        for (int b = threadIdx.x; b < kp; b += blockDim.x) {
-            row0[b] = (b == 2 * i) ? 1.0 : 0.0;
-            row1[b] = (b == 2 * i + 1) ? 1.0 : 0.0;
-        }
-        return;
-    }
-    const double xv = (double)x[0], yv = (double)x[1], phi = (double)x[2];
-    const int fi = 3 + 2 * (idf[i] - 1);
-    const ObsModel oi = obs_model(xv, yv, phi, (double)x[fi], (double)x[fi + 1]);
-    if (hblk && threadIdx.x == 0) {
-#pragma unroll
-        for (int q = 0; q < 6; ++q) hblk[HB_STRIDE * i + q] = oi.Hv[q];
-#pragma unroll
-        for (int q = 0; q < 4; ++q) hblk[HB_STRIDE * i + 6 + q] = oi.Hf[q];
-        reinterpret_cast<int*>(hblk + HB_STRIDE * HB_MAXOBS)[i] = fi;
-    }
-    const int rows[5] = {0, 1, 2, fi, fi + 1};
-    for (int b = threadIdx.x; b < kp; b += blockDim.x) {
-        if (b >= k) {
-            row0[b] = 0.0;
-            row1[b] = 0.0;
-            continue;
-        }
-        const int j = b >> 1, bb = b & 1;
-        const int fj = 3 + 2 * (idf[j] - 1);
-        const ObsModel oj = obs_model(xv, yv, phi, (double)x[fj], (double)x[fj + 1]);
-        double pr[5][5];
-#pragma unroll
-        for (int t = 0; t < 5; ++t) {
-            pr[t][0] = (double)sym_at(P, ld, tile_log2, rows[t], 0);
-            pr[t][1] = (double)sym_at(P, ld, tile_log2, rows[t], 1);
-            pr[t][2] = (double)sym_at(P, ld, tile_log2, rows[t], 2);
-            pr[t][3] = (double)sym_at(P, ld, tile_log2, rows[t], fj);
-            pr[t][4] = (double)sym_at(P, ld, tile_log2, rows[t], fj + 1);
-        }
-        double ph[5];
-#pragma unroll
-        for (int t = 0; t < 5; ++t)
-            ph[t] = bb == 0 ? pht_entry(oj.Hv[0], oj.Hv[1], oj.Hv[2], oj.Hf[0], oj.Hf[1], pr[t][0], pr[t][1], pr[t][2], pr[t][3], pr[t][4])
-                            : pht_entry(oj.Hv[3], oj.Hv[4], oj.Hv[5], oj.Hf[2], oj.Hf[3], pr[t][0], pr[t][1], pr[t][2], pr[t][3], pr[t][4]);
-#pragma unroll
-        for (int ra = 0; ra < 2; ++ra) {
-            double sv = pht_entry(oi.Hv[3 * ra + 0], oi.Hv[3 * ra + 1], oi.Hv[3 * ra + 2], oi.Hf[2 * ra + 0], oi.Hf[2 * ra + 1], ph[0], ph[1], ph[2],
-                                  ph[3], ph[4]);
-            if (j == i) sv += ra ? (bb ? R3 : R1) : (bb ? R2 : R0);
-            double pt[5];
-#pragma unroll
-            for (int t = 0; t < 5; ++t)
-                pt[t] = pht_entry(oi.Hv[3 * ra + 0], oi.Hv[3 * ra + 1], oi.Hv[3 * ra + 2], oi.Hf[2 * ra + 0], oi.Hf[2 * ra + 1], pr[0][t], pr[1][t],
-                                  pr[2][t], pr[3][t], pr[4][t]);
-            double st = pht_entry(bb ? oj.Hv[3] : oj.Hv[0], bb ? oj.Hv[4] : oj.Hv[1], bb ? oj.Hv[5] : oj.Hv[2], bb ? oj.Hf[2] : oj.Hf[0],
-                                  bb ? oj.Hf[3] : oj.Hf[1], pt[0], pt[1], pt[2], pt[3], pt[4]);
-            if (j == i) st += bb ? (ra ? R3 : R1) : (ra ? R2 : R0);
-            (ra ? row1 : row0)[b] = (b == 2 * i + ra) ? sv : (sv + st) * 0.5;
-        }
-    }
+    s_build_rows<T>(x, P, ld, idf, blockIdx.x, m, k, kp, Sg, pitch, tile_log2, R0, R1, R2, R3, hblk);
 }
 
 constexpr int FACTOR_THREADS = 512;
@@ -348,8 +282,6 @@
     int mode;
     unsigned long long* stamps;
 };
-constexpr unsigned PC_DONE = 15u, PC_FAIL = 31u;
-constexpr unsigned long long FW1_TIMEOUT = 200000000ull;
 typedef unsigned pc_u32x4 __attribute__((ext_vector_type(4)));
 typedef unsigned u32x2_pc __attribute__((ext_vector_type(2)));
 __device__ __forceinline__ void emit_c_part(const double* M, int mp, int Jc, const double* dvec, const ProgC& pc, int wave, int lane,
@@ -393,8 +325,13 @@
     }
 }
 
+struct NoLate {
+    __device__ __forceinline__ void operator()() const {}
+};
+template <typename Late = NoLate>
 __device__ __forceinline__ bool eliminate_blocked(double* M, int mp, int k, int kp, double* dvec, double* dinv, double* flag,
-                                                  bool four = true, const ProgC pc = ProgC{nullptr, 0, 0, nullptr, 0, nullptr}) {
+                                                  bool four = true, const ProgC pc = ProgC{nullptr, 0, 0, nullptr, 0, nullptr},
+                                                  const Late late = Late{}) {
     const int tid = threadIdx.x, nt = blockDim.x;
     const int lane = tid & 63, wave = tid >> 6, nwaves = nt >> 6;
     const int li = lane & 15, kk = lane >> 4;
@@ -457,6 +394,7 @@
             if (!okb && lane == 0) flag[0] = 1.0;
             ESTAMP(2);
         } else {
+            if (J == 0) late();
             if (J > 0) trailing(J - 1, wave, nwaves - 1, tp * (tp + 1) / 2);
             if (C < J) {
                 for (int K = C; K < J; ++K) {
@@ -575,6 +513,38 @@
     const int tid = threadIdx.x;
     const int nt = blockDim.x;
     const int mp = kp + 1;
+    bool stream = false;
+    unsigned r0w = 0u;
+    double s0[4], sr[4][4];
+    const int s_nb = kp >> 4, s_nrest = s_nb * (s_nb - 1) / 2;
+    auto rest_at = [&](int u, int& row, int& col) __attribute__((always_inline)) {
+        const int e = (tid >> 6) - 1 + (FACTOR_THREADS / 64 - 1) * u;
+        const bool on = (tid >> 6) >= 1 && e < s_nrest;
+        const int ec = on ? e : 0;
+        int I = 0;
+#pragma unroll
+        for (int t = 1; t <= 6; ++t) I += (t * (t + 1) / 2 <= ec) ? 1 : 0;
+        const int K = ec - I * (I + 1) / 2;
+        row = 16 * (1 + I) + ((tid & 63) >> 2);
+        col = 16 * (1 + K) + 4 * (tid & 3);
+        return on;
+    };
+    if constexpr (INLDS) {
+        stream = ready != nullptr && blocked && !(mode & 64) && nt == FACTOR_THREADS;
+        if (stream) {
+            r0w = __hip_atomic_load(ready, __ATOMIC_RELAXED, __HIP_MEMORY_SCOPE_AGENT);
+            const int a = tid >> 2, c0 = 4 * (tid & 3);
+#pragma unroll
+            for (int q = 0; q < 4; ++q) s0[q] = PHt[(size_t)(a < kp ? a : 0) * pht_pitch + c0 + q];
+#pragma unroll
+            for (int u = 0; u < 4; ++u) {
+                int row = 0, col = 0;
+                (void)rest_at(u, row, col);
+#pragma unroll
+                for (int q = 0; q < 4; ++q) sr[u][q] = PHt[(size_t)row * pht_pitch + col + q];
+            }
+        }
+    }
     double* M;
     double* aux;
     if constexpr (INLDS) {
@@ -607,7 +577,16 @@
     __syncthreads();
     STAMP(1);
 
-    if constexpr (INLDS) {
+    if (stream && r0w == PC_FAIL) {
+        if (tid == 0) { status[0] = 2; status[1] = 2; }
+        return;
+    }
+    if (stream) {
+        const int a = tid >> 2, c0 = 4 * (tid & 3);
+#pragma unroll
+        for (int q = 0; q < 4; ++q)
+            if (a < kp) M[(size_t)a * mp + c0 + q] = s0[q];
+    } else if constexpr (INLDS) {
         const int a0 = tid >> 5, bcol = tid & 31;
         for (int u0 = 0; u0 < kp; u0 += 8 * (nt >> 5)) {
             double v[8][4];
@@ -643,7 +622,7 @@
         M[(size_t)a * mp + b] = s;
     }
     }
-    __syncthreads();
+    if (!stream) __syncthreads();
     STAMP(2);
     if constexpr (!INLDS) {
         for (int idx = tid; idx < k * k; idx += nt) {
@@ -669,7 +648,18 @@
     if constexpr (!INLDS) ok = eliminate_in_memory(M, mp, k, mvec);
     else if (blocked) {
         const ProgC pcs{Cout, c_pitch, k, ready, mode, stamps};
-        ok = eliminate_blocked(M, mp, k, kp, rowbuf, rowbuf + kp, colbuf, blocked != 2, pcs);
+        auto late = [&]() __attribute__((always_inline)) {
+            if (!stream) return;
+#pragma unroll
+            for (int u = 0; u < 4; ++u) {
+                int row = 0, col = 0;
+                if (rest_at(u, row, col)) {
+#pragma unroll
+                    for (int q = 0; q < 4; ++q) M[(size_t)row * mp + col + q] = sr[u][q];
+                }
+            }
+        };
+        ok = eliminate_blocked(M, mp, k, kp, rowbuf, rowbuf + kp, colbuf, blocked != 2, pcs, late);
     }
     else if (kp == 32) ok = eliminate_in_registers<2>(M, mp, k, kp, rowbuf, colbuf);
     else if (kp == 64) ok = eliminate_in_registers<4>(M, mp, k, kp, rowbuf, colbuf);
@@ -1262,7 +1252,9 @@
     const int tlog = h->dtype == SLAM_F32 ? 7 : 6;
     const bool fused = !joseph && kp <= 128 && h->factor_blocked == 1 && !(h->xflags & 128);
     double* hblk = h->Smat;
-    {
+    const bool s_built = dcount && h->s_built && !joseph && kp <= 128;
+    h->s_built = 0;
+    if (!s_built) {
         KTimer t(h, SLAM_K_PHT);
         if (kp <= 128)
             hipLaunchKernelGGL(s_build_kernel<T>, dim3(kp / 2), dim3(128), 0, h->stream, x, P, h->ld, h->idfbuf, m, k, kp, h->PHtS,
@@ -1293,7 +1285,7 @@
                                R[2], R[3], h->Cmat, pitchA, h->gvec, h->d_status, stamps, dcount, h->factor_blocked, (const T*)P, h->ld, n,
                                h->npad, tlog, (const double*)hblk, W1, pitchW, img ? (char*)h->Wimg : (char*)nullptr, h->kcap / 16,
                                img ? h->dd_claim : (unsigned*)nullptr, drift, reinterpret_cast<unsigned*>(h->d_small + 56), wpw,
-                               slam_exp_env("SLAMHIP_FW1", 0));
+                               slam_exp_env("SLAMHIP_FW1", 0) | ((h->xflags & 131072) ? 64 : 0));
         } else if (in_lds)
             hipLaunchKernelGGL((factor_kernel<T, true>), fgrid, dim3(FACTOR_THREADS), shm, h->stream, x, h->PHtS, pitchA,
                                h->obsbuf, h->idfbuf, m, k, kp, R[0], R[1], R[2], R[3], h->Cmat, pitchA, h->gvec,
```
